# pangenome/allwave

Measured on AMD Instinct MI355X. Metric: aligned base-pairs/sec (whole node) + PAF lines/sec, all-pairs 10 kbp, higher is better.
Workload: dtype int16

## Files before the change

### allwave_amd/build.py

```python
import hashlib
import json
import os
import shutil
import subprocess
import tempfile
import time

ROOT = os.path.dirname(os.path.dirname(os.path.abspath(__file__)))
PKG = os.path.join(ROOT, "allwave_amd")
CSRC = os.path.join(PKG, "csrc")
HOST_DIR = os.path.join(CSRC, "host")
HIP_LIB = os.path.join(PKG, "liballwave_hip.so")
HOST_LIB = os.path.join(PKG, "liballwave_host.so")
CLI_BIN = os.path.join(PKG, "allwave_hip")
INFO = os.path.join(PKG, "BUILD_INFO.json")
ABI_HEADER = os.path.join(ROOT, "include", "allwave_hip.h")


def hipcc():
    for c in (os.environ.get("HIPCC"), shutil.which("hipcc"), "/opt/rocm/bin/hipcc"):
        if c and os.path.exists(c):
            return c
    raise RuntimeError("hipcc not found")


HIP_FLAGS = ["-O3", "-std=c++17", "--offload-arch=gfx950"]
HIP_FLAGS_AWV = HIP_FLAGS + ["-mllvm", "-amdgpu-sched-strategy=max-ilp"]
HIP_UNITS = (("engine.hip", HIP_FLAGS), ("kernels_awv.hip", HIP_FLAGS_AWV), ("planner.hip", HIP_FLAGS), ("orient.hip", HIP_FLAGS),
             ("verify.hip", HIP_FLAGS), ("clip.hip", HIP_FLAGS), ("split.hip", HIP_FLAGS), ("normalize.hip", HIP_FLAGS))
HIP_SOURCES = [os.path.join(CSRC, f) for f in ("engine.hip", "kernels_awv.hip", "kernels_awv.hpp", "biwfa_device.hpp", "range_span.hpp", "batch_plan.hpp", "twin_plan.hpp", "twin_base.hpp", "planner.hip",
                                               "planner_device.hpp", "orient.hip", "orient_device.hpp", "verify.hip", "verify_device.hpp", "clip.hip", "clip_device.hpp", "clip_scan.hpp", "split.hip", "split_device.hpp", "normalize.hip", "normalize_device.hpp", "wave_ops.hpp",
                                               "host_errors.hpp", "record_pass.hpp", "record_pieces.hpp")] + [ABI_HEADER]


def _host_sources():
    return [os.path.join(HOST_DIR, f) for f in sorted(os.listdir(HOST_DIR)) if f.endswith((".cpp", ".hpp", ".h"))]


_VERSIONS = {}


def _tool_version(tool):
    if tool not in _VERSIONS:
        try:
            _VERSIONS[tool] = subprocess.run([tool, "--version"], stdout=subprocess.PIPE, stderr=subprocess.STDOUT).stdout.decode(errors="replace")
        except OSError:
            _VERSIONS[tool] = "?"
    return _VERSIONS[tool]


def content_hash(sources, commands, tool):
    h = hashlib.sha256()
    for s in sorted(sources):
        h.update(os.path.relpath(s, ROOT).encode() + b"\0")
        with open(s, "rb") as f:
            h.update(f.read())
        h.update(b"\0")
    for c in commands:
        h.update(" ".join(c).encode() + b"\n")
    h.update(_tool_version(tool).encode())
    return h.hexdigest()


def _load_info():
    try:
        with open(INFO) as f:
            d = json.load(f)
        return d if isinstance(d.get("targets"), dict) else {"targets": {}}
    except (OSError, ValueError):
        return {"targets": {}}


def _record(target, digest, action):
    info = _load_info()
    info["targets"][os.path.basename(target)] = {"sha256": digest, "action": action, "when": time.strftime("%Y-%m-%dT%H:%M:%S")}
    tmp = INFO + ".%d.tmp" % os.getpid()
    with open(tmp, "w") as f:
        json.dump(info, f, indent=1)
    os.replace(tmp, INFO)


def _up_to_date(target, digest):
    return os.path.exists(target) and _load_info()["targets"].get(os.path.basename(target), {}).get("sha256") == digest


def _rel(cmd):
    return [a.replace(ROOT + os.sep, "") for a in cmd]


def build_hip(force=False, verbose=False):
    inc = ["-I" + os.path.join(ROOT, "include"), "-I" + CSRC]
    compile_cmds = [[hipcc()] + flags + ["-fPIC", "-c"] + inc + [os.path.join(CSRC, unit)] for unit, flags in HIP_UNITS]
    link_cmd = [hipcc(), "--offload-arch=gfx950", "-fPIC", "-shared"]
    digest = content_hash(HIP_SOURCES, [_rel(c) for c in compile_cmds] + [_rel(link_cmd)], hipcc())
    if not force and _up_to_date(HIP_LIB, digest):
        _record(HIP_LIB, digest, "reused (content hash of sources + flags + compiler matches)")
        return HIP_LIB
    tmp = tempfile.mkdtemp(prefix="awv_build_%d_" % os.getpid())
    try:
        objs, procs = [], []
        for (unit, _), cmd in zip(HIP_UNITS, compile_cmds):
            obj = os.path.join(tmp, unit.replace(".hip", ".o"))
            full = cmd + ["-o", obj]
            if verbose:
                print(" ".join(full))
            procs.append((full, subprocess.Popen(full)))
            objs.append(obj)
        failed = None
        for full, p in procs:
            if p.wait() != 0 and failed is None:
                failed = (p.returncode, full)
        if failed:
            raise subprocess.CalledProcessError(failed[0], failed[1])
        out = os.path.join(tmp, "liballwave_hip.so")
        full = link_cmd + ["-o", out] + objs
        if verbose:
            print(" ".join(full))
        subprocess.check_call(full)
        staged = HIP_LIB + ".%d.tmp" % os.getpid()
        shutil.copy2(out, staged)
        os.replace(staged, HIP_LIB)
    finally:
        shutil.rmtree(tmp, ignore_errors=True)
    _record(HIP_LIB, digest, "compiled")
    return HIP_LIB


def _build_one(target, sources, cmd, force, verbose, tool="g++"):
    digest = content_hash(sources, [_rel(cmd)], tool)
    if not force and _up_to_date(target, digest):
        _record(target, digest, "reused (content hash of sources + flags + compiler matches)")
        return
    tmp = target + ".%d.tmp" % os.getpid()
    full = cmd[:cmd.index("-o") + 1] + [tmp] + cmd[cmd.index("-o") + 2:]
    if verbose:
        print(" ".join(full))
    try:
        subprocess.check_call(full)
        os.replace(tmp, target)
    finally:
        if os.path.exists(tmp):
            os.remove(tmp)
    _record(target, digest, "compiled")


def build_host(force=False, verbose=False):
    if not os.path.isdir(HOST_DIR):
        return None
    srcs = _host_sources()
    cpps = [s for s in srcs if s.endswith(".cpp") and not s.endswith("main.cpp")]
    if not cpps:
        return None
    cmd = ["g++", "-O2", "-std=c++17", "-fPIC", "-shared", "-pthread", "-I" + os.path.join(ROOT, "include"), "-I" + HOST_DIR,
           "-o", HOST_LIB] + cpps + ["-L" + PKG, "-lallwave_hip", "-ldl", "-Wl,-rpath,$ORIGIN", "-Wl,-rpath-link,/opt/rocm/lib"]
    _build_one(HOST_LIB, srcs + [ABI_HEADER], cmd, force, verbose)
    cli_src = os.path.join(HOST_DIR, "main.cpp")
    if os.path.exists(cli_src):
        cmd = ["g++", "-O2", "-std=c++17", "-pthread", "-I" + os.path.join(ROOT, "include"), "-I" + HOST_DIR, "-o", CLI_BIN, cli_src,
               "-L" + PKG, "-lallwave_host", "-lallwave_hip", "-lz", "-Wl,-rpath,$ORIGIN", "-Wl,-rpath-link,/opt/rocm/lib"]
        _build_one(CLI_BIN, srcs + [ABI_HEADER], cmd, force, verbose)
    return HOST_LIB


def build_all(force=False, verbose=False):
    return build_hip(force, verbose), build_host(force, verbose)


def build_report():
    t = _load_info()["targets"]
    return {k: "%s [sha256 %s]" % (v.get("action", "?"), v.get("sha256", "")[:12]) for k, v in sorted(t.items())}


if __name__ == "__main__":
    print(build_all(force=True, verbose=True))
    print(json.dumps(build_report(), indent=1))
```

### allwave_amd/csrc/biwfa_device.hpp

```cpp


#include <hip/hip_runtime.h>
#include <stdint.h>
#include <limits.h>

#include "range_span.hpp"
#include "twin_base.hpp"

#ifndef AWV_NS
#define AWV_NS awv
#endif
#ifndef AWV_WG
#define AWV_WG 64
#endif
namespace AWV_NS {

constexpr int WG = AWV_WG;
constexpr int MAX_SCOPE = 126;
constexpr int MAX_RING = 256;
constexpr int NCOMP = 5;
constexpr int32_t OFF_NULL = INT32_MIN / 2;
constexpr int32_t NULLISH = INT32_MIN / 4;
constexpr int32_t NULL16 = -16384;
#ifdef AWV_WIDE16
constexpr bool WENC = true;
#else
constexpr bool WENC = false;
#endif
enum { C_M = 0, C_I1 = 1, C_I2 = 2, C_D1 = 3, C_D2 = 4 };
constexpr int FALLBACK_MIN_SCORE = 250;
constexpr int FALLBACK_MIN_LENGTH = 100;
constexpr int STACK_CAP = 48;
constexpr int EV_STACK_WORDS = (STACK_CAP * 32 + 3) / 4 + 16;
constexpr int EV_TWIN_WORDS = MAX_SCOPE * NCOMP;
constexpr int SUB16_MAX_LEN = 32760;
#ifndef AWV_WAVES_PER_SIMD
#define AWV_WAVES_PER_SIMD 4
#endif
constexpr int WAVES_PER_SIMD = AWV_WAVES_PER_SIMD;
constexpr int STATIC_LDS_RESERVE = 1024;
constexpr int COL_PAD = 576;

constexpr int ST_OK = 0, ST_CAPACITY = 1, ST_INTERNAL = 2, ST_MAX_STEPS = 3, ST_ABOVE_BOUND = 4;
constexpr int ST_TWIN_REDO = 64;

struct DevPenalties {
  int x, o1, e1, o2, e2, two_piece, scope;
};

struct DevResult {
  int32_t status, penalty, score;
  uint32_t cigar_len;
  uint64_t cigar_off;
  int32_t num_matches, num_mismatches, num_ins, num_del, q_end, t_end;
};

enum { STAT_CELLS = 0, STAT_EXTEND, STAT_BREAKPOINTS, STAT_BASE, STAT_OVERLAP, STAT_ALIGNED_BP, STAT_PAIRS,
       STAT_T_TOTAL, STAT_T_BI_COMPUTE, STAT_T_BI_BARRIER, STAT_T_BI_FINALIZE, STAT_T_OVERLAP, STAT_T_BASE_STEPS,
       STAT_T_BACKTRACE, STAT_T_EMIT, STAT_N_PASSES,
       STAT_T_CR_LOAD, STAT_T_CR_ALU, STAT_T_CR_EXTEND, STAT_T_CR_STORE, STAT_T_CR_REDUCE, STAT_RESTARTS, STAT_MULTI_CELLS, STAT_WIN_SINGLE, STAT_WIN_MULTI, STAT_WIN_BASE, STAT_WIN_BASE_MULTI,
       STAT_CLK_CYCLES, STAT_CLK_TICKS,
       STAT_DEEP_CELLS,
       STAT_N,
       STAT_TWIN_UNITS = STAT_N, STAT_TWIN_SHARED, STAT_TWIN_SOLO, STAT_TWIN_NONMIRROR,
       STAT_N_DEV };

#ifdef AWV_PROF
#define PROF_DRAIN() __builtin_amdgcn_s_waitcnt(0)
#define PROF_NOW() __builtin_readcyclecounter()
#define PROF_ADD(slot, t0) do { if (threadIdx.x == 0) lstats[slot] += __builtin_readcyclecounter() - (t0); } while (0)
#define PROF_INC(slot) do { if (threadIdx.x == 0) lstats[slot] += 1; } while (0)
#define PROF_ADD_L(slot, t0) do { if (threadIdx.x == 0) sh.prof[(slot) - STAT_T_CR_LOAD] += __builtin_readcyclecounter() - (t0); } while (0)
#else
#define PROF_ADD_L(slot, t0) do { (void)(t0); } while (0)
#define PROF_DRAIN() do { } while (0)
#define PROF_NOW() 0ULL
#define PROF_ADD(slot, t0) do { (void)(t0); } while (0)
#define PROF_INC(slot) do { } while (0)
#endif

struct KParams {
  const uint8_t* seq[4];
  const uint64_t* seq_off;
  const int32_t* seq_len;
  const uint32_t* seq2[2];
  const uint64_t* seq2_off;
  const uint8_t* seq2_ok;
  const int32_t* pair_q;
  const int32_t* pair_t;
  const int32_t* pair_rc;
  long long npairs;
  DevPenalties pen;
  int ring;
  int chain_max;
  int multi_T;
  int deep_passes;
  int sub16;
  int wcap;
  void* ring_mem;
  size_t ring_slot_stride;
  int lds_meta_bytes;
  int lds_seq_bytes;
  int sb_cap;
  int wb_cap;
  void* hist_mem;
  size_t hist_slot_stride;
  size_t hist_meta_offset;
  uint32_t* ev_mem;
  size_t ev_slot_stride;
  uint8_t* cigar;
  const uint64_t* cigar_off;
  DevResult* results;
  unsigned long long* work_counter;
  unsigned long long* stats;
  int score_only;
  int max_penalty;
  const int32_t* pair_max_penalty;
  const int32_t* unit_first;
  const int32_t* unit_twin;
  int twin_levels;
  int twin_base;
};

struct RowMeta { int lo, hi; };
constexpr int K_BIG = 1 << 28;
#define ROW_EMPTY RowMeta{K_BIG, -K_BIG}
struct Acc { int hull_lo[NCOMP]; int hull_hi[NCOMP]; int maxak; int oob; int reach; };
struct Task { int pb, pe, tb, te, cb, ce, score_remaining, known; };
constexpr int TM_A = 0, TM_B = 1, TM_SHARED = 2;
constexpr bool TWIN_BUILD = WG == 64 && !WENC;
constexpr int TWIN_MAGIC = 0x7477696e;
__device__ __forceinline__ int twin_comp(int c) { return c == 0 ? 0 : (c <= 2 ? c + 2 : c - 2); }
struct Breakpoint { int score, sf, sr, kf, kr, off_f, off_r, comp; };
static_assert(sizeof(Task) == 32 && sizeof(Breakpoint) == 32, "stack entry / twin record size");

__device__ __forceinline__ int s_min(int a, int b) { int r; asm("s_min_i32 %0, %1, %2" : "=s"(r) : "s"(a), "s"(b) : "scc"); return r; }
__device__ __forceinline__ int s_max(int a, int b) { int r; asm("s_max_i32 %0, %1, %2" : "=s"(r) : "s"(a), "s"(b) : "scc"); return r; }
__device__ __forceinline__ int s_add(int a, int b) { int r; asm("s_add_i32 %0, %1, %2" : "=s"(r) : "s"(a), "s"(b) : "scc"); return r; }

struct alignas(4) RowMeta16 { int16_t lo, hi; };
template <typename OffT> struct MetaTraits;
#ifdef AWV_WIDE16
template <> struct MetaTraits<int16_t> { typedef RowMeta Stored; };
#else
template <> struct MetaTraits<int16_t> { typedef RowMeta16 Stored; };
#endif
template <> struct MetaTraits<int32_t> { typedef RowMeta Stored; };
__device__ __forceinline__ RowMeta meta_load(const RowMeta16* p) {
  const RowMeta16 m = *p;
  return m.lo > m.hi ? ROW_EMPTY : RowMeta{m.lo, m.hi};
}
__device__ __forceinline__ RowMeta meta_load(const RowMeta* p) { return *p; }
__device__ __forceinline__ void meta_store(RowMeta16* p, const RowMeta& m) {
  *p = m.lo > m.hi ? RowMeta16{1, 0} : RowMeta16{(int16_t)m.lo, (int16_t)m.hi};
}
__device__ __forceinline__ void meta_store_scalar(RowMeta16* p, int lo, int hi) {
  int w;
  asm("s_pack_ll_b32_b16 %0, %1, %2\n\ts_cmp_gt_i32 %1, %2\n\ts_cselect_b32 %0, 1, %0" : "=&s"(w) : "s"(lo), "s"(hi) : "scc");
  *reinterpret_cast<int*>(p) = w;
}
__device__ __forceinline__ void meta_store_scalar(RowMeta* p, int lo, int hi) {
  int l, h;
  asm("s_cmp_gt_i32 %2, %3\n\ts_cselect_b32 %0, %4, %2\n\ts_cselect_b32 %1, %5, %3" : "=&s"(l), "=&s"(h) : "s"(lo), "s"(hi), "s"(K_BIG), "s"(-K_BIG) : "scc");
  *p = RowMeta{l, h};
}
__device__ __forceinline__ void meta_store(RowMeta* p, const RowMeta& m) { *p = m; }

template <typename OffT>
struct Lds {
  typename MetaTraits<OffT>::Stored* ring_meta;
  int* bi_A;
  int* bi_oob;
  int* firstk;
  uint32_t* seq;
  RowMeta* meta_log;
};
struct PassCtx {
  unsigned long long ring_mem;
  unsigned long long ring_bytes;
  unsigned long long P[2], T[2];
  int ring, wcap;
  int x, o1, e1, o2, e2;
  int lds_meta_bytes;
  int chain_max;
  int plen, tlen, kmin[2], wcols;
  int seq_mode, p_w0, t_w0, p_bit, t_bit;
  unsigned long long meta_log;
  int wb_cap, sb_cap, end_comp;
  unsigned long long Pw, Tw;
  int multi_T, lds_seq_bytes, pb_abs, tb_abs;
  int deep_passes;
  int max_penalty, score_cap;
};
struct PhaseResult {
  int why, sc, fmax, rmax, npass;
  int sf, sr, last_fwd;
  int deep_from;
  unsigned long long cells, deep_cells;
};
struct Shared {
  Acc acc[3][2];
  int chain_maxak[2][8];
  PassCtx pctx;
  PhaseResult pres;
  Breakpoint bp_out;
  unsigned long long ext_multi;
  unsigned int win_single, win_multi, win_base, win_base_multi;
  int ext0[2];
#ifdef AWV_PROF
  unsigned long long prof[5];
#endif
  long long cur_pair;
  int error;
  int nev;
  int bt_total;
};

typedef const __attribute__((address_space(1))) uint8_t* gseq_t;
typedef uint64_t u64_unaligned __attribute__((aligned(1)));
typedef const __attribute__((address_space(1))) uint32_t* gwords_t;
__device__ __forceinline__ gseq_t to_global(const uint8_t* p) { return (gseq_t)(uintptr_t)p; }

struct SubCtx {
  int plen, tlen;
  gseq_t P[2];
  gseq_t T[2];
  int kmin[2];
  int wcols;
  int seq_mode;
  int p_w0, t_w0;
  int p_bit, t_bit;
  gwords_t Pw, Tw;
  int pb_abs, tb_abs;
};

__device__ __forceinline__ bool row_empty(const RowMeta& m) { return m.lo > m.hi; }

__device__ __forceinline__ int uni(int x) { return __builtin_amdgcn_readfirstlane(x); }
__device__ __forceinline__ int clamp_from_m1(int x, int hi) {
  int r;
  asm("v_med3_i32 %0, %1, -1, %2" : "=v"(r) : "v"(x), "s"(hi));
  return r;
}
__device__ __forceinline__ int cold_tid() {
  int t = threadIdx.x;
  asm volatile("" : "+v"(t));
  return t;
}
__device__ __forceinline__ RowMeta uni(const RowMeta& m) { return RowMeta{uni(m.lo), uni(m.hi)}; }

__device__ __forceinline__ uint64_t ld64u(gseq_t p) {
  return *(const __attribute__((address_space(1))) u64_unaligned*)p;
}

__device__ __forceinline__ int wave_max_i32(int v) {
  v = max(v, __builtin_amdgcn_update_dpp(INT_MIN, v, 0x111, 0xf, 0xf, false));
  v = max(v, __builtin_amdgcn_update_dpp(INT_MIN, v, 0x112, 0xf, 0xf, false));
  v = max(v, __builtin_amdgcn_update_dpp(INT_MIN, v, 0x114, 0xf, 0xf, false));
  v = max(v, __builtin_amdgcn_update_dpp(INT_MIN, v, 0x118, 0xf, 0xf, false));
  v = max(v, __builtin_amdgcn_update_dpp(INT_MIN, v, 0x142, 0xa, 0xf, false));
  v = max(v, __builtin_amdgcn_update_dpp(INT_MIN, v, 0x143, 0xc, 0xf, false));
  return __builtin_amdgcn_readlane(v, 63);
}

template <typename OffT> struct OffTraits;
template <> struct OffTraits<int32_t> { static constexpr int VEC = 4; };
template <> struct OffTraits<int16_t> { static constexpr int VEC = 4; };

template <typename OffT> constexpr bool wenc_of() { return WENC && sizeof(OffT) == 2; }
template <typename OffT>
__device__ __forceinline__ int32_t off_load1(const OffT* p, int k) {
  const int32_t v = (int32_t)*p;
  if (sizeof(OffT) == 2) return v < 0 ? OFF_NULL : (wenc_of<OffT>() ? v + max(k, 0) : v);
  return v;
}
// ... 1430 lines not shown
        if (lane == 0 && t < Tn) atomicMax(&maxak_out[t], wmax);
      }
    } else {
      const int wmax = wave_max_i32(productive ? lane_maxak : 0);
      if (lane == 0) atomicMax(&maxak_out[0], wmax);
    }
  }
  if (BASE && lane == 0 && reach_mask) atomicOr(&acc.reach, (int)reach_mask);
  return cells;
}

typedef __attribute__((address_space(3))) Shared* lds_shared_ptr;
typedef __attribute__((address_space(3))) unsigned char* lds_bytes_ptr;
constexpr int MP_MARGIN = 0, MP_DISCARD = 1, MP_MET = 2, MP_ERROR = 3, MP_DEEP_MET = 4, MP_BOUND = 5;
template <bool P2, typename OffT, int E1, int E2>
__device__ __attribute__((noinline)) void deep_phase(unsigned sh_addr, unsigned dyn_addr, int s0_v, int fmax_v, int rmax_v, int Tn_v, int pass_v,
                                                     int far_npass_v, unsigned far_cells_lo, unsigned far_cells_hi);
#ifndef AWV_RESTART_ATTEMPTS
#define AWV_RESTART_ATTEMPTS 3
#endif
#ifndef AWV_MARGIN_BASE
#define AWV_MARGIN_BASE 256
#endif
#ifndef AWV_MARGIN_MUL4
#define AWV_MARGIN_MUL4 6
#endif
constexpr int MARGIN_BASE = AWV_MARGIN_BASE, MARGIN_MUL4 = AWV_MARGIN_MUL4;
template <bool P2, typename OffT, int E1, int E2, bool CHAIN>
__device__ __attribute__((noinline)) void multi_phase(unsigned sh_addr, unsigned dyn_addr, int s0_v, int fmax_v, int rmax_v, int Tn_v, int pass_v, int deep_v) {
  Shared& sh = *(Shared*)__builtin_assume_aligned((Shared*)(lds_shared_ptr)(uintptr_t)uni((int)sh_addr), 8);
  unsigned char* dyn_smem = (unsigned char*)__builtin_assume_aligned((unsigned char*)(lds_bytes_ptr)(uintptr_t)uni((int)dyn_addr), 16);
  const int Tn = uni(Tn_v);
  int sc = uni(s0_v);
  int fmax = uni(fmax_v), rmax = uni(rmax_v), pass = uni(pass_v);
  const PassCtx& pc = sh.pctx;
  KParams kp{};
  kp.ring = uni(pc.ring);
  kp.wcap = uni(pc.wcap);
  kp.pen.x = uni(pc.x);
  kp.pen.o1 = uni(pc.o1);
  kp.pen.e1 = uni(pc.e1);
  kp.pen.o2 = uni(pc.o2);
  kp.pen.e2 = uni(pc.e2);
  kp.pen.two_piece = P2 ? 1 : 0;
  kp.pen.scope = max(kp.pen.x, max(kp.pen.o1 + kp.pen.e1, P2 ? kp.pen.o2 + kp.pen.e2 : 0)) + 1;
  kp.lds_meta_bytes = uni(pc.lds_meta_bytes);
  auto uni64 = [](unsigned long long v) { return ((unsigned long long)(unsigned)uni((int)(v >> 32)) << 32) | (unsigned)uni((int)v); };
  SubCtx cx;
  cx.plen = uni(pc.plen);
  cx.tlen = uni(pc.tlen);
  cx.kmin[0] = uni(pc.kmin[0]);
  cx.kmin[1] = uni(pc.kmin[1]);
  cx.wcols = uni(pc.wcols);
  cx.seq_mode = uni(pc.seq_mode);
  cx.p_w0 = uni(pc.p_w0);
  cx.t_w0 = uni(pc.t_w0);
  cx.p_bit = uni(pc.p_bit);
  cx.t_bit = uni(pc.t_bit);
  cx.P[0] = (gseq_t)(uintptr_t)uni64(pc.P[0]);
  cx.P[1] = (gseq_t)(uintptr_t)uni64(pc.P[1]);
  cx.T[0] = (gseq_t)(uintptr_t)uni64(pc.T[0]);
  cx.T[1] = (gseq_t)(uintptr_t)uni64(pc.T[1]);
  cx.Pw = nullptr;
  cx.Tw = nullptr;
  cx.pb_abs = cx.tb_abs = 0;
  Lds<OffT> lds;
  typedef typename MetaTraits<OffT>::Stored MetaStored;
  lds.ring_meta = reinterpret_cast<MetaStored*>(dyn_smem);
  lds.bi_A = reinterpret_cast<int*>(lds.ring_meta + 2 * NCOMP * kp.ring);
  lds.bi_oob = lds.bi_A + 2 * kp.ring;
  lds.firstk = lds.bi_oob + 2 * kp.ring;
  lds.seq = reinterpret_cast<uint32_t*>(dyn_smem + kp.lds_meta_bytes);
  lds.meta_log = nullptr;
  const rsrc_t rs = make_rsrc((void*)(uintptr_t)uni64(pc.ring_mem), (size_t)uni64(pc.ring_bytes));
  const int rmask = kp.ring - 1;
  const int max_antidiagonal = cx.plen + cx.tlen - 1;
  const int arun_start = fmax + rmax;
  int arun0 = fmax, arun1 = rmax;
  int nsteps = 0, npass = 0, why = MP_MARGIN;
  unsigned long long cells = 0;
  unsigned ext_iters = 0;
  const bool lds_chain = CHAIN && sizeof(OffT) == 4 && cx.seq_mode != 1 &&
                         uni(pc.lds_seq_bytes) >= (WG / 64) * TMAX32 * 64 * 16;
  const int margin_shift = (uni(deep_v) >> 8) & 3;
  const bool long_reads = (uni(deep_v) & 0x400) != 0;
  const int chain_cap = CHAIN ? min(max(uni(pc.chain_max), 1), sizeof(OffT) == 2 ? CHAIN_MAX : (lds_chain ? 3 : CHAIN_MAX32)) : 1;
  for (;;) {
    if (sc >= uni(pc.score_cap)) { why = MP_BOUND; break; }
    const int grow = nsteps > 0 ? (arun0 + arun1 - arun_start) / nsteps : 0;
    int nh = 0;
    for (int c = chain_cap; c >= 1; --c) {
      const int T = c > 1 ? TMAX * c : Tn;
      const int mul4 = (sizeof(OffT) == 2 && !long_reads) ? MARGIN_MUL4 : MARGIN_MUL4 + 2;
      if (arun0 + arun1 < max_antidiagonal - ((MARGIN_BASE + mul4 * (kp.pen.scope + T) * max(grow, 8) / 4) << margin_shift)) { nh = c; break; }
    }
    if (nh == 0) { why = MP_MARGIN; break; }
    const int T = nh > 1 ? TMAX * nh : Tn;
    const int aslot = pass % 3;
    int nc0 = 0, nc1 = 0;
#pragma nounroll
    for (int dir = 0; dir < 2; ++dir) {
      MultiPlan mp;
      const unsigned long long tpl = PROF_NOW();
      plan_multi<P2, OffT, E1, E2, false>(kp, lds, cx, dir, sc, T, nh, mp);
      mp.lds_chain = lds_chain ? 1 : 0;
      PROF_ADD_L(STAT_T_CR_REDUCE, tpl);
      Acc& acc = dir ? sh.acc[aslot][1] : sh.acc[aslot][0];
      const int nc = compute_rows_multi<P2, OffT, E1, E2, false, CHAIN>(kp, sh, lds, cx, rs, dir, sc, mp, acc, dir ? sh.chain_maxak[1] : sh.chain_maxak[0], ext_iters);
      if (dir) nc1 = nc; else nc0 = nc;
    }
    __syncthreads();
    if (uni(sh.error)) { why = MP_ERROR; break; }
    if (uni(sh.acc[aslot][0].oob) != 0 || uni(sh.acc[aslot][1].oob) != 0) { why = MP_DISCARD; break; }
    cells += (unsigned long long)(nc0 + nc1);
    const int P0 = uni(sh.chain_maxak[0][0]), P1 = uni(sh.chain_maxak[1][0]);
    arun0 = max(arun0, P0);
    arun1 = max(arun1, P1);
    fmax = max(fmax, P0);
    rmax = max(rmax, P1);
    const bool met = fmax + rmax >= max_antidiagonal;
    __syncthreads();
    if (threadIdx.x < 16) sh.chain_maxak[threadIdx.x >> 3][threadIdx.x & 7] = 0;
    if (threadIdx.x == 0) { acc_reset(sh.acc[(pass + 2) % 3][0]); acc_reset(sh.acc[(pass + 2) % 3][1]); }
    __syncthreads();
    ++pass;
    ++npass;
    nsteps += T;
    sc += T;
    if (met) { why = MP_MET; break; }
  }
  __syncthreads();
  if (threadIdx.x == 0) {
    PhaseResult& pr = sh.pres;
    pr.why = why;
    pr.sc = sc;
    pr.sf = pr.sr = sc;
    pr.last_fwd = 0;
    pr.deep_from = sc;
    pr.fmax = fmax;
    pr.rmax = rmax;
    pr.npass = npass;
    pr.cells = cells;
    pr.deep_cells = 0;
#pragma unroll
    for (int i = 0; i < 3; ++i) { acc_reset(sh.acc[i][0]); acc_reset(sh.acc[i][1]); }
  }
  if (threadIdx.x < 16) sh.chain_maxak[threadIdx.x >> 3][threadIdx.x & 7] = 0;
  atomicAdd(&sh.ext_multi, (unsigned long long)ext_iters);
  __syncthreads();
  if ((uni(deep_v) & 1) != 0 && why == MP_MARGIN)
    deep_phase<P2, OffT, E1, E2>(sh_addr, dyn_addr, sc, fmax, rmax, Tn, pass, npass, (unsigned)cells, (unsigned)(cells >> 32));
}

template <bool P2, typename OffT, int E1, int E2>
__device__ __attribute__((noinline)) void deep_phase(unsigned sh_addr, unsigned dyn_addr, int s0_v, int fmax_v, int rmax_v, int Tn_v, int pass_v,
                                                     int far_npass_v, unsigned far_cells_lo, unsigned far_cells_hi) {
  Shared& sh = *(Shared*)__builtin_assume_aligned((Shared*)(lds_shared_ptr)(uintptr_t)uni((int)sh_addr), 8);
  unsigned char* dyn_smem = (unsigned char*)__builtin_assume_aligned((unsigned char*)(lds_bytes_ptr)(uintptr_t)uni((int)dyn_addr), 16);
  const int Tn = uni(Tn_v);
  int sc = uni(s0_v);
  int fmax = uni(fmax_v), rmax = uni(rmax_v), pass = uni(pass_v);
  const PassCtx& pc = sh.pctx;
  KParams kp{};
  kp.ring = uni(pc.ring);
  kp.wcap = uni(pc.wcap);
  kp.pen.x = uni(pc.x);
  kp.pen.o1 = uni(pc.o1);
  kp.pen.e1 = uni(pc.e1);
  kp.pen.o2 = uni(pc.o2);
  kp.pen.e2 = uni(pc.e2);
  kp.pen.two_piece = P2 ? 1 : 0;
  kp.pen.scope = max(kp.pen.x, max(kp.pen.o1 + kp.pen.e1, P2 ? kp.pen.o2 + kp.pen.e2 : 0)) + 1;
  kp.lds_meta_bytes = uni(pc.lds_meta_bytes);
  auto uni64 = [](unsigned long long v) { return ((unsigned long long)(unsigned)uni((int)(v >> 32)) << 32) | (unsigned)uni((int)v); };
  SubCtx cx;
  cx.plen = uni(pc.plen);
  cx.tlen = uni(pc.tlen);
  cx.kmin[0] = uni(pc.kmin[0]);
  cx.kmin[1] = uni(pc.kmin[1]);
  cx.wcols = uni(pc.wcols);
  cx.seq_mode = uni(pc.seq_mode);
  cx.p_w0 = uni(pc.p_w0);
  cx.t_w0 = uni(pc.t_w0);
  cx.p_bit = uni(pc.p_bit);
  cx.t_bit = uni(pc.t_bit);
  cx.P[0] = (gseq_t)(uintptr_t)uni64(pc.P[0]);
  cx.P[1] = (gseq_t)(uintptr_t)uni64(pc.P[1]);
  cx.T[0] = (gseq_t)(uintptr_t)uni64(pc.T[0]);
  cx.T[1] = (gseq_t)(uintptr_t)uni64(pc.T[1]);
  cx.Pw = nullptr;
  cx.Tw = nullptr;
  cx.pb_abs = cx.tb_abs = 0;
  Lds<OffT> lds;
  typedef typename MetaTraits<OffT>::Stored MetaStored;
  lds.ring_meta = reinterpret_cast<MetaStored*>(dyn_smem);
  lds.bi_A = reinterpret_cast<int*>(lds.ring_meta + 2 * NCOMP * kp.ring);
  lds.bi_oob = lds.bi_A + 2 * kp.ring;
  lds.firstk = lds.bi_oob + 2 * kp.ring;
  lds.seq = reinterpret_cast<uint32_t*>(dyn_smem + kp.lds_meta_bytes);
  lds.meta_log = nullptr;
  const rsrc_t rs = make_rsrc((void*)(uintptr_t)uni64(pc.ring_mem), (size_t)uni64(pc.ring_bytes));
  const int rmask = kp.ring - 1;
  const int max_antidiagonal = cx.plen + cx.tlen - 1;
  int sf = sc, sr = sc, last_fwd = 0;
  const int deep_from = sc, far_npass = uni(far_npass_v);
  const unsigned long long far_cells = ((unsigned long long)(unsigned)uni((int)far_cells_hi) << 32) | (unsigned)uni((int)far_cells_lo);
  int npass = 0, why = MP_DISCARD;
  unsigned long long cells = 0;
  unsigned ext_iters = 0;
  for (;;) {
    if (sc >= uni(pc.score_cap)) { why = MP_BOUND; break; }
    const int aslot = pass % 3;
    int nc0 = 0, nc1 = 0;
#pragma nounroll
    for (int dir = 0; dir < 2; ++dir) {
      MultiPlan mp;
      const unsigned long long tpl = PROF_NOW();
      plan_multi<P2, OffT, E1, E2, false>(kp, lds, cx, dir, sc, Tn, 1, mp);
      PROF_ADD_L(STAT_T_CR_REDUCE, tpl);
      Acc& acc = dir ? sh.acc[aslot][1] : sh.acc[aslot][0];
      const int nc = compute_rows_multi<P2, OffT, E1, E2, false, false, true>(kp, sh, lds, cx, rs, dir, sc, mp, acc, dir ? sh.chain_maxak[1] : sh.chain_maxak[0], ext_iters);
      if (dir) nc1 = nc; else nc0 = nc;
    }
    __syncthreads();
    if (uni(sh.error)) { why = MP_ERROR; break; }
    if (uni(sh.acc[aslot][0].oob) != 0 || uni(sh.acc[aslot][1].oob) != 0) { why = MP_DISCARD; break; }
    cells += (unsigned long long)(nc0 + nc1);
    bool met = false;
    for (int t = 0; t < Tn; ++t) {
      const int slot = (sc + 1 + t) & rmask;
      const int A0 = uni(sh.chain_maxak[0][t]), A1 = uni(sh.chain_maxak[1][t]);
      lds.bi_A[slot] = A0;
      lds.bi_A[kp.ring + slot] = A1;
      lds.bi_oob[slot] = 0;
      lds.bi_oob[kp.ring + slot] = 0;
      if (!met) {
        ++sf;
        fmax = max(fmax, A0);
        last_fwd = 1;
        if (fmax + rmax >= max_antidiagonal) met = true;
        else {
          ++sr;
          rmax = max(rmax, A1);
          last_fwd = 0;
          if (fmax + rmax >= max_antidiagonal) met = true;
        }
      }
    }
    __syncthreads();
    if (threadIdx.x < 16) sh.chain_maxak[threadIdx.x >> 3][threadIdx.x & 7] = 0;
    if (threadIdx.x == 0) { acc_reset(sh.acc[(pass + 2) % 3][0]); acc_reset(sh.acc[(pass + 2) % 3][1]); }
    __syncthreads();
    ++pass;
    ++npass;
    sc += Tn;
    if (met) { why = MP_DEEP_MET; break; }
  }
  __syncthreads();
  if (threadIdx.x == 0) {
    PhaseResult& pr = sh.pres;
    pr.why = why;
    pr.sc = sc;
    pr.sf = sf;
    pr.sr = sr;
    pr.last_fwd = last_fwd;
    pr.deep_from = deep_from;
    pr.fmax = fmax;
    pr.rmax = rmax;
    pr.npass = far_npass + npass;
    pr.cells = far_cells + cells;
    pr.deep_cells = cells;
#pragma unroll
    for (int i = 0; i < 3; ++i) { acc_reset(sh.acc[i][0]); acc_reset(sh.acc[i][1]); }
  }
  if (threadIdx.x < 16) sh.chain_maxak[threadIdx.x >> 3][threadIdx.x & 7] = 0;
  atomicAdd(&sh.ext_multi, (unsigned long long)ext_iters);
  __syncthreads();
}

template <bool P2, typename OffT, int E1, int E2>
__device__ __attribute__((noinline)) void base_phase(unsigned sh_addr, unsigned dyn_addr, int s0_v, int Tn_v, int pass_v) {
  Shared& sh = *(Shared*)__builtin_assume_aligned((Shared*)(lds_shared_ptr)(uintptr_t)uni((int)sh_addr), 8);
  unsigned char* dyn_smem = (unsigned char*)__builtin_assume_aligned((unsigned char*)(lds_bytes_ptr)(uintptr_t)uni((int)dyn_addr), 16);
  const int Tn = uni(Tn_v);
  int sc = uni(s0_v), pass = uni(pass_v);
  const PassCtx& pc = sh.pctx;
  KParams kp{};
  kp.ring = uni(pc.ring);
  kp.wb_cap = uni(pc.wb_cap);
  kp.sb_cap = uni(pc.sb_cap);
  kp.pen.x = uni(pc.x);
  kp.pen.o1 = uni(pc.o1);
  kp.pen.e1 = uni(pc.e1);
  kp.pen.o2 = uni(pc.o2);
  kp.pen.e2 = uni(pc.e2);
  kp.pen.two_piece = P2 ? 1 : 0;
  kp.pen.scope = max(kp.pen.x, max(kp.pen.o1 + kp.pen.e1, P2 ? kp.pen.o2 + kp.pen.e2 : 0)) + 1;
  kp.lds_meta_bytes = uni(pc.lds_meta_bytes);
  auto uni64 = [](unsigned long long v) { return ((unsigned long long)(unsigned)uni((int)(v >> 32)) << 32) | (unsigned)uni((int)v); };
  SubCtx cx;
  cx.plen = uni(pc.plen);
  cx.tlen = uni(pc.tlen);
  cx.kmin[0] = uni(pc.kmin[0]);
  cx.kmin[1] = cx.kmin[0];
  cx.wcols = uni(pc.wcols);
  cx.seq_mode = uni(pc.seq_mode);
// ... 1008 lines not shown
  bp.score = INT_MAX;
  unsigned ext_iters = 0;
  unsigned long long cells = 0, multi_cells = 0, deep_cells = 0;
  int pass = 0;
  const long long max_steps = ((long long)pn.o1 + pn.o2 + 2LL * (pn.e1 + pn.e2) + pn.x) * ((long long)plen + tlen + 4) + 1024;
  long long steps = 0;
  int rc = BP_OK;
  if (kp.max_penalty != INT_MAX) bp.score = kp.max_penalty + 1;
  const int gap_opening = P2 ? max(pn.o1, pn.o2) : pn.o1;
  bool last_fwd = false;
  const bool known_optimum = known_score != INT_MAX;
  bool dirty[2] = {false, false};
  const bool force_single = (attempt & 0xff) >= AWV_RESTART_ATTEMPTS - 1;
  const int deep_arg = kp.deep_passes | ((attempt & 0xff) == 1 && !force_single ? 0x200 : 0) | ((attempt & 0x100) ? 0x400 : 0);
  const int multi_T = (!force_single && plen + tlen > AWV_MIN_PASS_LEN) ? kp.multi_T : 0;
  bool deep_on = multi_T == 0;
  int deep_since[2] = {deep_on ? 0 : INT_MAX, deep_on ? 0 : INT_MAX};
  auto deep_ok = [&](int d0, int s0, int d1, int s1) {
    const int lo_need = max(s1 - (pn.scope - 1), 1);
    return (s0 == 0 || deep_since[d0] <= s0) && (s1 == 0 || deep_since[d1] <= lo_need);
  };
  int phase = 1;
  for (;;) {
    if (phase == 1 && fmax + rmax >= max_antidiagonal) phase = 2;
    {
      Acc* a = sh.acc[pass % 3];
      int plo[2] = {1, 1}, phi[2] = {0, 0};
      bool need[2];
      const unsigned long long tp0 = PROF_NOW();
      if (!deep_on && (dirty[0] || dirty[1])) {
        deep_on = true;
        deep_since[0] = comp[0] + 1;
        deep_since[1] = comp[1] + 1;
      }
      if (!deep_on && phase == 1 && comp[0] == sc[0] && comp[1] == sc[1] && sc[0] == sc[1]) {
        if (P2) multi_phase<P2, OffT, 2, 1, P2>(sh_addr, dyn_addr, sc[0], fmax, rmax, multi_T, pass, deep_arg);
        else if (pn.e1 == 1) multi_phase<P2, OffT, 1, 1, false>(sh_addr, dyn_addr, sc[0], fmax, rmax, multi_T, pass, deep_arg);
        else multi_phase<P2, OffT, 2, 1, false>(sh_addr, dyn_addr, sc[0], fmax, rmax, multi_T, pass, deep_arg);
        PROF_ADD(STAT_T_BI_COMPUTE, tp0);
        const int why = uni(sh.pres.why);
        if (why == MP_ERROR) { rc = uni(sh.error); break; }
        if (why == MP_MET) { rc = BP_RESTART; break; }
        steps += (long long)(uni(sh.pres.sc) - sc[0]);
        comp[0] = comp[1] = uni(sh.pres.sc);
        sc[0] = uni(sh.pres.sf);
        sc[1] = uni(sh.pres.sr);
        last_fwd = uni(sh.pres.last_fwd) != 0;
        fmax = uni(sh.pres.fmax);
        rmax = uni(sh.pres.rmax);
        pass += uni(sh.pres.npass);
        {
          const unsigned long long c = ((unsigned long long)(unsigned)uni((int)(sh.pres.cells >> 32)) << 32) | (unsigned)uni((int)sh.pres.cells);
          const unsigned long long dc = ((unsigned long long)(unsigned)uni((int)(sh.pres.deep_cells >> 32)) << 32) | (unsigned)uni((int)sh.pres.deep_cells);
          cells += c;
          multi_cells += c;
          deep_cells += dc;
        }
        deep_on = true;
        deep_since[0] = deep_since[1] = uni(sh.pres.deep_from) + 1;
        __syncthreads();
        continue;
      } else {
#pragma unroll
      for (int dir = 0; dir < 2; ++dir) {
        need[dir] = comp[dir] == sc[dir];
        if (need[dir]) {
          StepPlan pl;
          plan_step<P2, false, OffT>(kp, lds, dir, sc[dir] + 1, pl);
          cells += compute_row<P2, false, OffT>(kp, sh, lds, cx, ring_rs, dir, sc[dir] + 1, pl, dirty[dir], a[dir], ext_iters);
          plo[dir] = pl.lo;
          phi[dir] = pl.hi;
        }
      }
#ifdef AWV_DIAG
      if (tid == 0) {
        const int zone = (dirty[0] || dirty[1]) ? 4 : multi_T == 0 ? 0 : phase == 2 ? 3 : (sc[0] + 1 - (pn.scope - 1) >= 1) ? 2 : 1;
        unsigned nw = 0;
        if (need[0] && plo[0] <= phi[0]) nw += (unsigned)((phi[0] - plo[0] + 4) / 248 + 1);
        if (need[1] && plo[1] <= phi[1]) nw += (unsigned)((phi[1] - plo[1] + 4) / 248 + 1);
        lstats[STAT_T_CR_LOAD + zone] += nw;
      }
#endif
      if (need[0] || need[1]) {
        PROF_ADD(STAT_T_BI_COMPUTE, tp0);
        PROF_INC(STAT_N_PASSES);
        const unsigned long long tp1 = PROF_NOW();
        __syncthreads();
        PROF_ADD(STAT_T_BI_BARRIER, tp1);
        const unsigned long long tp2 = PROF_NOW();
        if (uni(sh.error)) { rc = uni(sh.error); break; }
        const bool trim0 = need[0] && uni(a[0].oob) != 0, trim1 = need[1] && uni(a[1].oob) != 0;
        dirty[0] = dirty[0] || trim0;
        dirty[1] = dirty[1] || trim1;
        if (trim0 || trim1) {
          if (trim0) trim_pass_fn<P2, false, OffT>(sh_addr, 0, sc[0] + 1, plo[0], phi[0], pass % 3);
          if (trim1) trim_pass_fn<P2, false, OffT>(sh_addr, 1, sc[1] + 1, plo[1], phi[1], pass % 3);
          __syncthreads();
        }
        if (need[0]) { finalize_row<false, OffT>(kp, lds, cx, 0, sc[0] + 1, a[0], trim0); comp[0] = sc[0] + 1; }
        if (need[1]) { finalize_row<false, OffT>(kp, lds, cx, 1, sc[1] + 1, a[1], trim1); comp[1] = sc[1] + 1; }
        if (tid == 0) { acc_reset(sh.acc[(pass + 2) % 3][0]); acc_reset(sh.acc[(pass + 2) % 3][1]); }
        ++pass;
        PROF_ADD(STAT_T_BI_FINALIZE, tp2);
      }
      }
    }
    if (phase == 1) {
      ++sc[0];
      fmax = max(fmax, uni(lds.bi_A[0 * kp.ring + (sc[0] & rmask)]));
      last_fwd = true;
      if (fmax + rmax >= max_antidiagonal) { phase = 2; continue; }
      ++sc[1];
      rmax = max(rmax, uni(lds.bi_A[1 * kp.ring + (sc[1] & rmask)]));
      last_fwd = false;
      if (sc[1] >= uni(sh.pctx.score_cap)) { rc = BP_ABOVE_BOUND; break; }
    } else {
      if (last_fwd) {
        const int min_sr = (sc[1] > pn.scope - 1) ? sc[1] - (pn.scope - 1) : 0;
        if (sc[0] + min_sr - gap_opening >= bp.score) break;
        if (!deep_ok(0, sc[0], 1, sc[1])) { rc = BP_RESTART; break; }
        const unsigned long long to0 = PROF_NOW();
        bialign_overlap<P2, OffT>(kp, sh, lds, cx, ring_mem, ring_rs, 0, sc[0], sc[1], true, bp, lstats);
        PROF_ADD(STAT_T_OVERLAP, to0);
        if (known_optimum && bp.score == known_score) break;
        ++sc[1];
      }
      const int min_sf = (sc[0] > pn.scope - 1) ? sc[0] - (pn.scope - 1) : 0;
      if (min_sf + sc[1] - gap_opening >= bp.score) break;
      if (!deep_ok(1, sc[1], 0, sc[0])) { rc = BP_RESTART; break; }
      const unsigned long long to1 = PROF_NOW();
      bialign_overlap<P2, OffT>(kp, sh, lds, cx, ring_mem, ring_rs, 1, sc[1], sc[0], false, bp, lstats);
      PROF_ADD(STAT_T_OVERLAP, to1);
      if (known_optimum && bp.score == known_score) break;
      ++sc[0];
      last_fwd = true;
    }
    if (++steps > max_steps) { rc = ST_MAX_STEPS; break; }
  }
  if (tid == 0) {
    lstats[STAT_CELLS] += cells;
    lstats[STAT_MULTI_CELLS] += multi_cells;
    lstats[STAT_DEEP_CELLS] += deep_cells;
    lstats[STAT_BREAKPOINTS] += 1;
  }
  atomicAdd(&lstats[STAT_EXTEND], (unsigned long long)ext_iters);
  if (tid == 0) lstats[STAT_EXTEND] += sh.ext_multi;
  if (rc == BP_OK && bp.score > uni(sh.pctx.max_penalty)) rc = BP_ABOVE_BOUND;
  __syncthreads();
  if (rc == BP_OK && bp.score == INT_MAX) rc = ST_INTERNAL;
  return rc;
}

template <bool P2, typename OffT>
__device__ __attribute__((noinline)) int find_breakpoint_fn(unsigned sh_addr, unsigned dyn_addr, unsigned lstats_addr, int cb_v, int ce_v,
                                                            int score_remaining_v, int known_v, int attempt_v) {
  Shared& sh = *(Shared*)__builtin_assume_aligned((Shared*)(__attribute__((address_space(3))) Shared*)(uintptr_t)uni((int)sh_addr), 8);
  unsigned char* dyn_smem = (unsigned char*)__builtin_assume_aligned((unsigned char*)(__attribute__((address_space(3))) unsigned char*)(uintptr_t)uni((int)dyn_addr), 16);
  unsigned long long* lstats = (unsigned long long*)__builtin_assume_aligned((unsigned long long*)(__attribute__((address_space(3))) unsigned long long*)(uintptr_t)uni((int)lstats_addr), 8);
  const int cb = uni(cb_v), ce = uni(ce_v), score_remaining = uni(score_remaining_v), known = uni(known_v);
  const int attempt = uni(attempt_v);
  const PassCtx& pc = sh.pctx;
  auto uni64 = [](unsigned long long v) { return ((unsigned long long)(unsigned)uni((int)(v >> 32)) << 32) | (unsigned)uni((int)v); };
  KParams kp{};
  kp.ring = uni(pc.ring);
  kp.wcap = uni(pc.wcap);
  kp.pen.x = uni(pc.x);
  kp.pen.o1 = uni(pc.o1);
  kp.pen.e1 = uni(pc.e1);
  kp.pen.o2 = uni(pc.o2);
  kp.pen.e2 = uni(pc.e2);
  kp.pen.two_piece = P2 ? 1 : 0;
  kp.pen.scope = max(kp.pen.x, max(kp.pen.o1 + kp.pen.e1, P2 ? kp.pen.o2 + kp.pen.e2 : 0)) + 1;
  kp.lds_meta_bytes = uni(pc.lds_meta_bytes);
  kp.lds_seq_bytes = uni(pc.lds_seq_bytes);
  kp.chain_max = uni(pc.chain_max);
  kp.multi_T = uni(pc.multi_T);
  kp.deep_passes = uni(pc.deep_passes);
  kp.max_penalty = score_remaining == INT_MAX ? uni(pc.max_penalty) : INT_MAX;
  kp.ring_slot_stride = (size_t)uni64(pc.ring_bytes);
  SubCtx cx;
  cx.plen = uni(pc.plen);
  cx.tlen = uni(pc.tlen);
  cx.kmin[0] = cx.kmin[1] = 0;
  cx.wcols = 0;
  cx.seq_mode = uni(pc.seq_mode);
  cx.p_w0 = uni(pc.p_w0);
  cx.t_w0 = uni(pc.t_w0);
  cx.p_bit = uni(pc.p_bit);
  cx.t_bit = uni(pc.t_bit);
  cx.P[0] = (gseq_t)(uintptr_t)uni64(pc.P[0]);
  cx.P[1] = (gseq_t)(uintptr_t)uni64(pc.P[1]);
  cx.T[0] = (gseq_t)(uintptr_t)uni64(pc.T[0]);
  cx.T[1] = (gseq_t)(uintptr_t)uni64(pc.T[1]);
  cx.Pw = (gwords_t)(uintptr_t)uni64(pc.Pw);
  cx.Tw = (gwords_t)(uintptr_t)uni64(pc.Tw);
  cx.pb_abs = uni(pc.pb_abs);
  cx.tb_abs = uni(pc.tb_abs);
  Lds<OffT> lds;
  typedef typename MetaTraits<OffT>::Stored MetaStored;
  lds.ring_meta = reinterpret_cast<MetaStored*>(dyn_smem);
  lds.bi_A = reinterpret_cast<int*>(lds.ring_meta + 2 * NCOMP * kp.ring);
  lds.bi_oob = lds.bi_A + 2 * kp.ring;
  lds.firstk = lds.bi_oob + 2 * kp.ring;
  lds.seq = reinterpret_cast<uint32_t*>(dyn_smem + kp.lds_meta_bytes);
  lds.meta_log = nullptr;
  void* ring_mem = (void*)(__attribute__((address_space(1))) char*)(uintptr_t)uni64(pc.ring_mem);
  const rsrc_t ring_rs = make_rsrc(ring_mem, kp.ring_slot_stride);
  __syncthreads();
  Breakpoint bp;
  const int rc = find_breakpoint<P2, OffT>(kp, sh, lds, cx, ring_mem, ring_rs, cb, ce, score_remaining, known, attempt, bp, lstats);
  if (threadIdx.x == 0) sh.bp_out = bp;
  __syncthreads();
  return rc;
}

template <bool P2, typename OffT, typename... PairSpan>
__global__ __launch_bounds__(WG, WAVES_PER_SIMD) void biwfa_align_kernel(KParams kp, PairSpan... pair_span_arg) {
  constexpr bool RANGES = sizeof...(PairSpan) > 0;
  static_assert(sizeof...(PairSpan) <= 1, "one optional argument: const awvr::Span*");
  __shared__ Shared sh;
  __shared__ unsigned long long lstats[STAT_N];
  static_assert(sizeof(Shared) + sizeof(unsigned long long) * STAT_N <= STATIC_LDS_RESERVE, "static LDS reserve");
  extern __shared__ __attribute__((aligned(16))) unsigned char dyn_smem[];
  Lds<OffT> lds;
  typedef typename MetaTraits<OffT>::Stored MetaStored;
  lds.ring_meta = reinterpret_cast<MetaStored*>(dyn_smem);
  lds.bi_A = reinterpret_cast<int*>(lds.ring_meta + 2 * NCOMP * kp.ring);
  lds.bi_oob = lds.bi_A + 2 * kp.ring;
  lds.firstk = lds.bi_oob + 2 * kp.ring;
  lds.seq = reinterpret_cast<uint32_t*>(dyn_smem + kp.lds_meta_bytes);
  const int tid = cold_tid();
  const DevPenalties& pn = kp.pen;
  void* ring_mem = (char*)kp.ring_mem + (size_t)blockIdx.x * kp.ring_slot_stride;
  void* hist = (char*)kp.hist_mem + (size_t)blockIdx.x * kp.hist_slot_stride;
  uint32_t* events = kp.ev_mem + (size_t)blockIdx.x * kp.ev_slot_stride;
  Task* const stack = reinterpret_cast<Task*>(events + kp.wcap);
  const rsrc_t hist_rs = make_rsrc(hist, kp.hist_slot_stride);
  lds.meta_log = reinterpret_cast<RowMeta*>((char*)hist + kp.hist_meta_offset);
  if (tid < STAT_N) lstats[tid] = 0;
#ifdef AWV_PROF
  if (tid < 5) sh.prof[tid] = 0;
#endif
  const unsigned long long clk_c0 = __builtin_amdgcn_s_memtime(), clk_r0 = __builtin_amdgcn_s_memrealtime();
  if (tid < 16) sh.chain_maxak[tid >> 3][tid & 7] = 0;
  __syncthreads();
  constexpr bool TWINS = TWIN_BUILD && !RANGES && sizeof(OffT) == 2;
  if constexpr (TWINS) {
  for (;;) {
    if (tid == 0) {
      sh.cur_pair = (long long)atomicAdd(kp.work_counter, 1ULL);
      sh.win_single = sh.win_multi = sh.win_base = sh.win_base_multi = 0;
    }
    __syncthreads();
    const long long unit = ((long long)uni((int)(sh.cur_pair >> 32)) << 32) | (unsigned)uni((int)sh.cur_pair);
    if (unit >= kp.npairs) break;
    long long pair = unit, pair_b = -1;
    if constexpr (TWINS) {
      if (kp.unit_first) {
        pair = uni(kp.unit_first[unit]);
        pair_b = uni(kp.unit_twin[unit]);
      }
    }
    const int qi = kp.pair_q[pair], ti = kp.pair_t[pair];
    const int qv = kp.pair_rc[pair] ? 2 : 0;
    const uint64_t qoff = kp.seq_off[qi], toff = kp.seq_off[ti];
    int plenT = kp.seq_len[qi], tlenT = kp.seq_len[ti];
    const uint8_t* Pf = kp.seq[qv] + qoff;
    const uint8_t* Pr = kp.seq[qv + 1] + qoff;
    const uint8_t* Tf = kp.seq[0] + toff;
    const uint8_t* Tr = kp.seq[1] + toff;
    const int qok = (kp.seq2_ok[qi] >> (qv ? 1 : 0)) & 1, tok = kp.seq2_ok[ti] & 1;
    gwords_t Pw = nullptr, Tw = nullptr;
    if (qok && tok && kp.lds_seq_bytes > 0) {
      Pw = (gwords_t)(uintptr_t)(kp.seq2[qv ? 1 : 0] + kp.seq2_off[qi]);
      Tw = (gwords_t)(uintptr_t)(kp.seq2[0] + kp.seq2_off[ti]);
    }
    int tw_shared = 0, tw_solo = 0, tw_nonmirror = 0;
    int run_mode = TWINS && pair_b >= 0 ? TM_SHARED : TM_A;
    int todo = 0;
    for (;;) {
    const unsigned long long tt0 = PROF_NOW();
    int cur = TM_A;
    Emit em, em_o;
    em.cig = kp.score_only ? nullptr : kp.cigar + kp.cigar_off[pair];
    em.n = 0;
    em.cnt[0] = em.cnt[1] = em.cnt[2] = em.cnt[3] = 0;
    em_o = em;
    if (pair_b >= 0 && !kp.score_only) em_o.cig = kp.cigar + kp.cigar_off[pair_b];
    int status = ST_OK;
    int penalty = -1, penalty_o = -1;
    bool top = true, top_o = true;
    auto face = [&](int o) {
      if (cur == o) return;
      cur = o;
      { const uint8_t* x = Pf; Pf = Tf; Tf = x; }
      { const uint8_t* x = Pr; Pr = Tr; Tr = x; }
      { const gwords_t x = Pw; Pw = Tw; Tw = x; }
      { const int x = plenT; plenT = tlenT; tlenT = x; }
      { const Emit x = em; em = em_o; em_o = x; }
      { const int x = penalty; penalty = penalty_o; penalty_o = x; }
      { const bool x = top; top = top_o; top_o = x; }
    };
    if (TWINS && run_mode == TM_B) face(TM_B);
    int sp = 0;
    if constexpr (RANGES) {
      if (tid == 0) {
        const awvr::Span top = (pair_span_arg, ...)[pair];
        const bool min_length = max(top.pe - top.pb, top.te - top.tb) <= FALLBACK_MIN_LENGTH;
        stack[0] = Task{top.pb, top.pe, top.tb, top.te, C_M, C_M, min_length ? 0 : INT_MAX, INT_MAX};
        sh.error = 0;
      }
    } else if (tid == 0) {
      const bool min_length = max(plenT, tlenT) <= FALLBACK_MIN_LENGTH;
      stack[0] = Task{0, plenT, 0, tlenT, C_M | (run_mode << 8), C_M, min_length ? 0 : INT_MAX, INT_MAX};
      sh.error = 0;
    }
    sp = 1;
    __syncthreads();
    while (sp > 0 && status == ST_OK) {
      Task t = stack[sp - 1];
      t.pb = uni(t.pb); t.pe = uni(t.pe); t.tb = uni(t.tb); t.te = uni(t.te);
      t.cb = uni(t.cb); t.ce = uni(t.ce); t.score_remaining = uni(t.score_remaining); t.known = uni(t.known);
      --sp;
      __syncthreads();
      const int mode = TWINS ? (t.cb >> 8) & 3 : TM_A, depth = TWINS ? t.cb >> 16 : 0;
      if (TWINS) {
        t.cb &= 0xff;
        face(mode == TM_B ? TM_B : TM_A);
      }
      const int plen = t.pe - t.pb, tlen = t.te - t.tb;
      bool split = mode == TM_SHARED && (tlen == 0 || plen == 0 || t.score_remaining <= FALLBACK_MIN_SCORE);
      Breakpoint bp, bq;
      bool do_base = false;
      SubCtx cx;
      if (!split) {
      if (tlen == 0) {
        emit_run(em, 'D', plen);
        if (top) penalty = plen > 0 ? min(pn.o1 + plen * pn.e1, P2 ? pn.o2 + plen * pn.e2 : INT_MAX) : 0;
        top = false;
        continue;
      } else if (plen == 0) {
        emit_run(em, 'I', tlen);
        if (top) penalty = min(pn.o1 + tlen * pn.e1, P2 ? pn.o2 + tlen * pn.e2 : INT_MAX);
        top = false;
        continue;
      }
      cx.plen = plen;
      cx.tlen = tlen;
      cx.P[0] = to_global(Pf + t.pb);
      cx.T[0] = to_global(Tf + t.tb);
      cx.P[1] = to_global(Pr + (plenT - t.pe));
      cx.T[1] = to_global(Tr + (tlenT - t.te));
      cx.kmin[0] = cx.kmin[1] = 0;
      cx.wcols = 0;
      cx.Pw = Pw;
      cx.Tw = Tw;
      cx.pb_abs = t.pb;
      cx.tb_abs = t.tb;
      stage_sequences<OffT>(kp, lds, cx);
      do_base = t.score_remaining <= FALLBACK_MIN_SCORE;
      if (!do_base) {
        int rc = BP_OK;
        for (int attempt = 0; attempt < AWV_RESTART_ATTEMPTS; ++attempt) {
          if (tid == 0) {
            PassCtx& pc = sh.pctx;
            pc.ring_mem = (unsigned long long)(uintptr_t)ring_mem;
            pc.ring_bytes = (unsigned long long)kp.ring_slot_stride;
            pc.P[0] = (unsigned long long)(uintptr_t)cx.P[0];
            pc.P[1] = (unsigned long long)(uintptr_t)cx.P[1];
            pc.T[0] = (unsigned long long)(uintptr_t)cx.T[0];
            pc.T[1] = (unsigned long long)(uintptr_t)cx.T[1];
            pc.Pw = (unsigned long long)(uintptr_t)cx.Pw;
            pc.Tw = (unsigned long long)(uintptr_t)cx.Tw;
            pc.ring = kp.ring;
            pc.wcap = kp.wcap;
            pc.x = pn.x; pc.o1 = pn.o1; pc.e1 = pn.e1; pc.o2 = pn.o2; pc.e2 = pn.e2;
            pc.lds_meta_bytes = kp.lds_meta_bytes;
            pc.lds_seq_bytes = kp.lds_seq_bytes;
            pc.chain_max = kp.chain_max;
            pc.multi_T = kp.multi_T;
            pc.deep_passes = kp.deep_passes;
            pc.max_penalty = kp.pair_max_penalty ? kp.pair_max_penalty[pair] : kp.max_penalty;
            pc.plen = plen; pc.tlen = tlen;
            pc.seq_mode = cx.seq_mode; pc.p_w0 = cx.p_w0; pc.t_w0 = cx.t_w0; pc.p_bit = cx.p_bit; pc.t_bit = cx.t_bit;
            pc.pb_abs = cx.pb_abs; pc.tb_abs = cx.tb_abs;
            const unsigned long long tab = (unsigned long long)(uintptr_t)(events + kp.wcap + EV_STACK_WORDS);
            sh.bp_out.comp = mode == TM_SHARED && !kp.score_only ? TWIN_MAGIC : 0;
            sh.bp_out.off_f = (int)(unsigned)tab;
            sh.bp_out.off_r = (int)(unsigned)(tab >> 32);
            if (mode == TM_SHARED)
              reinterpret_cast<Breakpoint*>(dyn_smem + kp.lds_meta_bytes - sizeof(Breakpoint))->score = INT_MAX;
          }
          __syncthreads();
          if constexpr (sizeof(OffT) == 4 && !WENC) {
            if (kp.sub16 != 0 && max(plen, tlen) < SUB16_MAX_LEN)
              rc = uni(find_breakpoint_fn<P2, int16_t>((unsigned)(uintptr_t)&sh, (unsigned)(uintptr_t)lds.ring_meta, (unsigned)(uintptr_t)lstats,
                                                       t.cb, t.ce, t.score_remaining, t.known, attempt | 0x100));
            else
              rc = uni(find_breakpoint_fn<P2, OffT>((unsigned)(uintptr_t)&sh, (unsigned)(uintptr_t)lds.ring_meta, (unsigned)(uintptr_t)lstats,
                                                    t.cb, t.ce, t.score_remaining, t.known, attempt));
          } else {
            rc = uni(find_breakpoint_fn<P2, OffT>((unsigned)(uintptr_t)&sh, (unsigned)(uintptr_t)lds.ring_meta, (unsigned)(uintptr_t)lstats,
                                                  t.cb, t.ce, t.score_remaining, t.known, attempt));
          }
          if (rc == BP_OK) {
            bp.score = uni(sh.bp_out.score); bp.sf = uni(sh.bp_out.sf); bp.sr = uni(sh.bp_out.sr); bp.kf = uni(sh.bp_out.kf);
            bp.kr = uni(sh.bp_out.kr); bp.off_f = uni(sh.bp_out.off_f); bp.off_r = uni(sh.bp_out.off_r); bp.comp = uni(sh.bp_out.comp);
            if (mode == TM_SHARED && !kp.score_only) {
              const Breakpoint* rec = reinterpret_cast<const Breakpoint*>(dyn_smem + kp.lds_meta_bytes - sizeof(Breakpoint));
              bq.score = uni(rec->score); bq.sf = uni(rec->sf); bq.sr = uni(rec->sr); bq.kf = uni(rec->kf);
              bq.off_f = uni(rec->off_f); bq.comp = uni(rec->comp);
            }
          }
          if (rc != BP_RESTART) break;
          if (tid == 0) lstats[STAT_RESTARTS] += 1;
        }
        if (TWINS && pair_b >= 0 && run_mode == TM_SHARED) {
          if (mode == TM_SHARED) ++tw_shared;
          else ++tw_solo;
        }
        if (rc == BP_END_REACHED) {
          if (mode == TM_SHARED) split = true;
          else do_base = true;
        }
        else if (rc == BP_ABOVE_BOUND) { status = ST_ABOVE_BOUND; break; }
        else if (rc != BP_OK) { status = rc; break; }
      }
      }
      bool shared_base = false;
      if (split && kp.twin_base != 0) {
        if (tlen == 0 || plen == 0) {
          const int n = max(plen, tlen);
          const int pen_gap = n > 0 ? min(pn.o1 + n * pn.e1, P2 ? pn.o2 + n * pn.e2 : INT_MAX) : 0;
          emit_run(em, tlen == 0 ? 'D' : 'I', n);
          emit_run(em_o, plen == 0 ? 'D' : 'I', n);
          if (top) penalty = pen_gap;
          if (top_o) penalty_o = pen_gap;
          top = top_o = false;
          continue;
        }
        if (t.score_remaining <= FALLBACK_MIN_SCORE) {
          cx.plen = plen;
          cx.tlen = tlen;
          cx.P[0] = to_global(Pf + t.pb);
          cx.T[0] = to_global(Tf + t.tb);
          cx.P[1] = to_global(Pr + (plenT - t.pe));
          cx.T[1] = to_global(Tr + (tlenT - t.te));
          cx.kmin[0] = cx.kmin[1] = 0;
          cx.wcols = 0;
          cx.Pw = Pw;
          cx.Tw = Tw;
          cx.pb_abs = t.pb;
          cx.tb_abs = t.tb;
          stage_sequences<OffT>(kp, lds, cx);
        }
        split = false;
        do_base = shared_base = true;
      }
      if (split) {
        if (sp + 2 > STACK_CAP) { status = ST_TWIN_REDO; break; }
        if (tid == 0) {
          stack[sp] = Task{t.tb, t.te, t.pb, t.pe, twin_comp(t.cb) | (TM_B << 8), twin_comp(t.ce), t.score_remaining, t.known};
          stack[sp + 1] = Task{t.pb, t.pe, t.tb, t.te, t.cb | (TM_A << 8), t.ce, t.score_remaining, t.known};
        }
        sp += 2;
        __syncthreads();
        continue;
      }
      if (do_base) {
        int pen_b = 0;
        const int rc = base_align_twin<P2, OffT>(kp, sh, lds, cx, hist, hist_rs, events, t.cb, t.ce, em, pen_b, lstats, em_o, shared_base && !kp.score_only);
        if (rc != ST_OK) { status = shared_base ? ST_TWIN_REDO : rc; break; }
        if (top) penalty = pen_b;
        top = false;
        if (shared_base) {
          if (top_o) penalty_o = pen_b;
          top_o = false;
        }
        continue;
      }
      if (kp.score_only) {
        penalty = bp.score;
        if (mode == TM_SHARED) penalty_o = bp.score;
        break;
      }
      const int bh = bp.off_f, bv = bp.off_f - bp.kf;
      if (mode != TM_SHARED) {
        if (bh < 0 || bh > tlen || bv < 0 || bv > plen || sp + 2 > STACK_CAP) { status = ST_INTERNAL; break; }
        if (tid == 0) {
          const int open_c = bp.comp == C_M ? 0 : ((bp.comp == C_I1 || bp.comp == C_D1) ? kp.pen.o1 : kp.pen.o2);
          stack[sp] = Task{t.pb + bv, t.pe, t.tb + bh, t.te, bp.comp | (mode << 8), t.ce, bp.sr, bp.sr - open_c};
          stack[sp + 1] = Task{t.pb, t.pb + bv, t.tb, t.tb + bh, t.cb | (mode << 8), bp.comp, bp.sf, bp.sf - open_c};
        }
        sp += 2;
      } else {
        const int qh = bq.off_f, qv2 = bq.off_f - bq.kf;
        if (bq.score != bp.score || bq.comp < 0 || bq.comp >= NCOMP || (!P2 && (bq.comp == C_I2 || bq.comp == C_D2)) || bh < 0 || bh > tlen || bv < 0 || bv > plen || qh < 0 || qh > plen || qv2 < 0 || qv2 > tlen ||
            sp + 4 > STACK_CAP) { status = ST_TWIN_REDO; break; }
        const bool mirror = bq.kf == -bp.kf && qh == bv && bq.comp == twin_comp(bp.comp) && bq.sf == bp.sf && bq.sr == bp.sr;
        if (!mirror) ++tw_nonmirror;
        const int open_c = bp.comp == C_M ? 0 : ((bp.comp == C_I1 || bp.comp == C_D1) ? kp.pen.o1 : kp.pen.o2);
        if (mirror && depth + 1 < kp.twin_levels) {
          if (tid == 0) {
            const int tag = (TM_SHARED << 8) | ((depth + 1) << 16);
            stack[sp] = Task{t.pb + bv, t.pe, t.tb + bh, t.te, bp.comp | tag, t.ce, bp.sr, bp.sr - open_c};
            stack[sp + 1] = Task{t.pb, t.pb + bv, t.tb, t.tb + bh, t.cb | tag, bp.comp, bp.sf, bp.sf - open_c};
          }
          sp += 2;
        } else {
          if (tid == 0) {
            const int open_q = bq.comp == C_M ? 0 : ((bq.comp == C_I1 || bq.comp == C_D1) ? kp.pen.o1 : kp.pen.o2);
            const int cbq = twin_comp(t.cb), ceq = twin_comp(t.ce);
            stack[sp] = Task{t.pb + bv, t.pe, t.tb + bh, t.te, bp.comp | (TM_A << 8), t.ce, bp.sr, bp.sr - open_c};
            stack[sp + 1] = Task{t.tb + qv2, t.te, t.pb + qh, t.pe, bq.comp | (TM_B << 8), ceq, bq.sr, bq.sr - open_q};
            stack[sp + 2] = Task{t.pb, t.pb + bv, t.tb, t.tb + bh, t.cb | (TM_A << 8), bp.comp, bp.sf, bp.sf - open_c};
            stack[sp + 3] = Task{t.tb, t.tb + qv2, t.pb, t.pb + qh, cbq | (TM_B << 8), bq.comp, bq.sf, bq.sf - open_q};
          }
          sp += 4;
        }
        if (top_o) penalty_o = bp.score;
        top_o = false;
      }
      if (top) penalty = bp.score;
      top = false;
      __syncthreads();
    }
    const int failed_in = cur;
    if (TWINS) face(TM_A);
    bool write_a = run_mode == TM_A, write_b = run_mode == TM_B;
    if (TWINS && run_mode == TM_SHARED) {
      if (status == ST_OK) write_a = write_b = true;
      else if (status == ST_TWIN_REDO) todo = 3;
      else if (failed_in == TM_B) { write_b = true; todo = 1; }
      else { write_a = true; todo = 2; }
    }
    const int pair_bound = kp.pair_max_penalty ? kp.pair_max_penalty[pair] : kp.max_penalty;
    if (status == ST_OK && penalty > pair_bound) {
      status = ST_ABOVE_BOUND;
      em.cnt[0] = em.cnt[1] = em.cnt[2] = em.cnt[3] = 0;
    }
    if (tid == 0) {
      auto record = [&](long long pi, const Emit& e, int pen, int qlen) {
        DevResult r;
        r.status = status;
        r.penalty = status == ST_OK ? pen : status == ST_ABOVE_BOUND ? pair_bound + 1 : 0;
        r.score = -r.penalty;
        r.cigar_len = status == ST_OK && !kp.score_only ? (uint32_t)e.n : 0u;
        r.cigar_off = kp.score_only ? 0 : kp.cigar_off[pi];
        r.num_matches = e.cnt[0];
        r.num_mismatches = e.cnt[1];
        r.num_ins = e.cnt[2];
        r.num_del = e.cnt[3];
        r.q_end = e.cnt[0] + e.cnt[1] + e.cnt[3];
        r.t_end = e.cnt[0] + e.cnt[1] + e.cnt[2];
        kp.results[pi] = r;
        if (status == ST_OK) {
          lstats[STAT_ALIGNED_BP] += (unsigned long long)qlen;
          lstats[STAT_PAIRS] += 1;
        }
      };
      if constexpr (RANGES) {
        record(pair, em, penalty, (pair_span_arg, ...)[pair].pe - (pair_span_arg, ...)[pair].pb);
      } else {
        if (write_a) record(pair, em, penalty, plenT);
        if (TWINS && write_b) record(pair_b, em_o, penalty_o, tlenT);
      }
      PROF_ADD(STAT_T_TOTAL, tt0);
      lstats[STAT_WIN_SINGLE] += sh.win_single; lstats[STAT_WIN_MULTI] += sh.win_multi; lstats[STAT_WIN_BASE] += sh.win_base; lstats[STAT_WIN_BASE_MULTI] += sh.win_base_multi;
      sh.win_single = sh.win_multi = sh.win_base = sh.win_base_multi = 0;
    }
    __syncthreads();
    if (!TWINS || !todo) break;
    run_mode = (todo & 1) ? TM_A : TM_B;
    todo &= ~(1 << run_mode);
    }
    if (TWINS && pair_b >= 0 && tid == 0) {
      atomicAdd(&kp.stats[STAT_TWIN_UNITS], 1ULL);
      atomicAdd(&kp.stats[STAT_TWIN_SHARED], (unsigned long long)tw_shared);
      atomicAdd(&kp.stats[STAT_TWIN_SOLO], (unsigned long long)tw_solo);
      atomicAdd(&kp.stats[STAT_TWIN_NONMIRROR], (unsigned long long)tw_nonmirror);
    }
  }
  } else {
  for (;;) {
    if (tid == 0) {
      sh.cur_pair = (long long)atomicAdd(kp.work_counter, 1ULL);
      sh.error = 0;
      sh.win_single = sh.win_multi = sh.win_base = sh.win_base_multi = 0;
    }
    __syncthreads();
    const long long pair = ((long long)uni((int)(sh.cur_pair >> 32)) << 32) | (unsigned)uni((int)sh.cur_pair);
    if (pair >= kp.npairs) break;
    const int qi = kp.pair_q[pair], ti = kp.pair_t[pair];
    const int qv = kp.pair_rc[pair] ? 2 : 0;
    const uint64_t qoff = kp.seq_off[qi], toff = kp.seq_off[ti];
    const int plenT = kp.seq_len[qi], tlenT = kp.seq_len[ti];
    const uint8_t* Pf = kp.seq[qv] + qoff;
    const uint8_t* Pr = kp.seq[qv + 1] + qoff;
    const uint8_t* Tf = kp.seq[0] + toff;
    const uint8_t* Tr = kp.seq[1] + toff;
    const int qok = (kp.seq2_ok[qi] >> (qv ? 1 : 0)) & 1, tok = kp.seq2_ok[ti] & 1;
    gwords_t Pw = nullptr, Tw = nullptr;
    if (qok && tok && kp.lds_seq_bytes > 0) {
      Pw = (gwords_t)(uintptr_t)(kp.seq2[qv ? 1 : 0] + kp.seq2_off[qi]);
      Tw = (gwords_t)(uintptr_t)(kp.seq2[0] + kp.seq2_off[ti]);
    }
    const unsigned long long tt0 = PROF_NOW();
    Emit em;
    em.cig = kp.score_only ? nullptr : kp.cigar + kp.cigar_off[pair];
    em.n = 0;
    em.cnt[0] = em.cnt[1] = em.cnt[2] = em.cnt[3] = 0;
    int status = ST_OK;
    int penalty = -1;
    int sp = 0;
    if constexpr (RANGES) {
      if (tid == 0) {
        const awvr::Span top = (pair_span_arg, ...)[pair];
        const bool min_length = max(top.pe - top.pb, top.te - top.tb) <= FALLBACK_MIN_LENGTH;
        stack[0] = Task{top.pb, top.pe, top.tb, top.te, C_M, C_M, min_length ? 0 : INT_MAX, INT_MAX};
      }
    } else if (tid == 0) {
      const bool min_length = max(plenT, tlenT) <= FALLBACK_MIN_LENGTH;
      stack[0] = Task{0, plenT, 0, tlenT, C_M, C_M, min_length ? 0 : INT_MAX, INT_MAX};
    }
    sp = 1;
    __syncthreads();
    bool top = true;
    while (sp > 0 && status == ST_OK) {
      Task t = stack[sp - 1];
      t.pb = uni(t.pb); t.pe = uni(t.pe); t.tb = uni(t.tb); t.te = uni(t.te);
      t.cb = uni(t.cb); t.ce = uni(t.ce); t.score_remaining = uni(t.score_remaining); t.known = uni(t.known);
      --sp;
      __syncthreads();
      const int plen = t.pe - t.pb, tlen = t.te - t.tb;
      if (tlen == 0) {
        emit_run(em, 'D', plen);
        if (top) penalty = plen > 0 ? min(pn.o1 + plen * pn.e1, P2 ? pn.o2 + plen * pn.e2 : INT_MAX) : 0;
        top = false;
        continue;
      } else if (plen == 0) {
        emit_run(em, 'I', tlen);
        if (top) penalty = min(pn.o1 + tlen * pn.e1, P2 ? pn.o2 + tlen * pn.e2 : INT_MAX);
        top = false;
        continue;
      }
      SubCtx cx;
      cx.plen = plen;
      cx.tlen = tlen;
      cx.P[0] = to_global(Pf + t.pb);
      cx.T[0] = to_global(Tf + t.tb);
      cx.P[1] = to_global(Pr + (plenT - t.pe));
      cx.T[1] = to_global(Tr + (tlenT - t.te));
      cx.kmin[0] = cx.kmin[1] = 0;
      cx.wcols = 0;
      cx.Pw = Pw;
      cx.Tw = Tw;
      cx.pb_abs = t.pb;
      cx.tb_abs = t.tb;
      stage_sequences<OffT>(kp, lds, cx);
      bool do_base = t.score_remaining <= FALLBACK_MIN_SCORE;
      Breakpoint bp;
      if (!do_base) {
        int rc = BP_OK;
        for (int attempt = 0; attempt < AWV_RESTART_ATTEMPTS; ++attempt) {
          if (tid == 0) {
            PassCtx& pc = sh.pctx;
            pc.ring_mem = (unsigned long long)(uintptr_t)ring_mem;
            pc.ring_bytes = (unsigned long long)kp.ring_slot_stride;
            pc.P[0] = (unsigned long long)(uintptr_t)cx.P[0];
            pc.P[1] = (unsigned long long)(uintptr_t)cx.P[1];
            pc.T[0] = (unsigned long long)(uintptr_t)cx.T[0];
            pc.T[1] = (unsigned long long)(uintptr_t)cx.T[1];
            pc.Pw = (unsigned long long)(uintptr_t)cx.Pw;
            pc.Tw = (unsigned long long)(uintptr_t)cx.Tw;
            pc.ring = kp.ring;
            pc.wcap = kp.wcap;
            pc.x = pn.x; pc.o1 = pn.o1; pc.e1 = pn.e1; pc.o2 = pn.o2; pc.e2 = pn.e2;
            pc.lds_meta_bytes = kp.lds_meta_bytes;
            pc.lds_seq_bytes = kp.lds_seq_bytes;
            pc.chain_max = kp.chain_max;
            pc.multi_T = kp.multi_T;
            pc.deep_passes = kp.deep_passes;
            pc.max_penalty = kp.pair_max_penalty ? kp.pair_max_penalty[pair] : kp.max_penalty;
            pc.plen = plen; pc.tlen = tlen;
            pc.seq_mode = cx.seq_mode; pc.p_w0 = cx.p_w0; pc.t_w0 = cx.t_w0; pc.p_bit = cx.p_bit; pc.t_bit = cx.t_bit;
            pc.pb_abs = cx.pb_abs; pc.tb_abs = cx.tb_abs;
          }
          __syncthreads();
          if constexpr (sizeof(OffT) == 4 && !WENC) {
            if (kp.sub16 != 0 && max(plen, tlen) < SUB16_MAX_LEN)
              rc = uni(find_breakpoint_fn<P2, int16_t>((unsigned)(uintptr_t)&sh, (unsigned)(uintptr_t)lds.ring_meta, (unsigned)(uintptr_t)lstats,
                                                       t.cb, t.ce, t.score_remaining, t.known, attempt | 0x100));
            else
              rc = uni(find_breakpoint_fn<P2, OffT>((unsigned)(uintptr_t)&sh, (unsigned)(uintptr_t)lds.ring_meta, (unsigned)(uintptr_t)lstats,
                                                    t.cb, t.ce, t.score_remaining, t.known, attempt));
          } else {
            rc = uni(find_breakpoint_fn<P2, OffT>((unsigned)(uintptr_t)&sh, (unsigned)(uintptr_t)lds.ring_meta, (unsigned)(uintptr_t)lstats,
                                                  t.cb, t.ce, t.score_remaining, t.known, attempt));
          }
          if (rc == BP_OK) {
            bp.score = uni(sh.bp_out.score); bp.sf = uni(sh.bp_out.sf); bp.sr = uni(sh.bp_out.sr); bp.kf = uni(sh.bp_out.kf);
            bp.kr = uni(sh.bp_out.kr); bp.off_f = uni(sh.bp_out.off_f); bp.off_r = uni(sh.bp_out.off_r); bp.comp = uni(sh.bp_out.comp);
          }
          if (rc != BP_RESTART) break;
          if (tid == 0) lstats[STAT_RESTARTS] += 1;
        }
        if (rc == BP_END_REACHED) do_base = true;
        else if (rc == BP_ABOVE_BOUND) { status = ST_ABOVE_BOUND; break; }
        else if (rc != BP_OK) { status = rc; break; }
      }
      if (do_base) {
        int pen_b = 0;
        const int rc = base_align<P2, OffT>(kp, sh, lds, cx, hist, hist_rs, events, t.cb, t.ce, em, pen_b, lstats);
        if (rc != ST_OK) { status = rc; break; }
        if (top) penalty = pen_b;
        top = false;
        continue;
      }
      if (kp.score_only) {
        penalty = bp.score;
        break;
      }
      const int bh = bp.off_f, bv = bp.off_f - bp.kf;
      if (bh < 0 || bh > tlen || bv < 0 || bv > plen || sp + 2 > STACK_CAP) { status = ST_INTERNAL; break; }
      if (tid == 0) {
        const int open_c = bp.comp == C_M ? 0 : ((bp.comp == C_I1 || bp.comp == C_D1) ? kp.pen.o1 : kp.pen.o2);
        stack[sp] = Task{t.pb + bv, t.pe, t.tb + bh, t.te, bp.comp, t.ce, bp.sr, bp.sr - open_c};
        stack[sp + 1] = Task{t.pb, t.pb + bv, t.tb, t.tb + bh, t.cb, bp.comp, bp.sf, bp.sf - open_c};
      }
      sp += 2;
      if (top) penalty = bp.score;
      top = false;
      __syncthreads();
    }
// ... 45 lines not shown
```

### allwave_amd/csrc/engine.hip

```cpp
#include "allwave_hip.h"
#include "host_errors.hpp"
#include "planner_device.hpp"
#include "verify_device.hpp"
#include "clip_device.hpp"
#include "split_device.hpp"
#include "normalize_device.hpp"
#include "kernels_awv.hpp"
#define AWV_NS awv
#define AWV_WG 64
#include "biwfa_device.hpp"
#undef AWV_NS
#undef AWV_WG
#define AWV_NS awvw
#define AWV_WG 256
#include "biwfa_device.hpp"
#undef AWV_NS
#undef AWV_WG
#define AWV_NS awvx
#define AWV_WG 1024
#include "biwfa_device.hpp"
#undef AWV_NS
#undef AWV_WG
#define AWV_WIDE16 1
#define AWV_NS awvw_m
#define AWV_WG 256
#include "biwfa_device.hpp"
#undef AWV_NS
#undef AWV_WG
#define AWV_NS awvx_m
#define AWV_WG 1024
#include "biwfa_device.hpp"
#undef AWV_NS
#undef AWV_WG
#undef AWV_WIDE16

#include <algorithm>
#include <chrono>
#include <climits>
#include <cmath>
#include <cstdio>
#include <cstdlib>
#include <cstring>
#include <exception>
#include <string>
#include <thread>
#include <vector>

#include "batch_plan.hpp"
#include "twin_plan.hpp"

namespace {
const awvb::Limits LIMITS = {awv::TMAX, awv::TMAX32, awv::CHAIN_MAX, awv::MAX_RING, awv::MAX_SCOPE, awv::NCOMP, awv::COL_PAD,
                             awv::FALLBACK_MIN_SCORE, awv::FALLBACK_MIN_LENGTH, awv::WAVES_PER_SIMD, awv::STATIC_LDS_RESERVE,
                             (size_t)awv::EV_STACK_WORDS, (size_t)awv::EV_TWIN_WORDS, sizeof(awv::RowMeta), sizeof(awv::RowMeta16),
                             sizeof(awv::Breakpoint)};
static_assert(awv::EV_STACK_WORDS == (awv::STACK_CAP * sizeof(awv::Task) + 3) / 4 + 16, "DFS stack words");

thread_local std::string g_last_error;

int fail(int code, const std::string& msg) {
  g_last_error = msg;
  return code;
}

template <typename T>
struct DevBuf {
  T* p = nullptr;
  size_t cap = 0;
  int reserve(size_t n) {
    if (n <= cap) return AWV_OK;
    if (p) (void)hipFree(p);
    p = nullptr;
    cap = 0;
    size_t want = n + std::min<size_t>(n / 8, (size_t)64 << 20) + 64;
    hipError_t e = hipMalloc((void**)&p, want * sizeof(T));
    if (e != hipSuccess) {
      want = n;
      e = hipMalloc((void**)&p, want * sizeof(T));
    }
    if (e != hipSuccess) {
      p = nullptr;
      return fail(AWV_ERR_OOM, std::string("hipMalloc ") + std::to_string(want * sizeof(T)) + " bytes: " + hipGetErrorString(e));
    }
    cap = want;
    return AWV_OK;
  }
  void release() {
    if (p) (void)hipFree(p);
    p = nullptr;
    cap = 0;
  }
  void adopt(T* q, size_t n) {
    release();
    p = q;
    cap = n;
  }
  size_t bytes() const { return cap * sizeof(T); }
};

struct SeqSet {
  int32_t n = 0;
  std::vector<uint64_t> off;
  std::vector<int32_t> len;
  DevBuf<uint8_t> d_seq[4];
  DevBuf<uint64_t> d_off;
  DevBuf<int32_t> d_len;
  DevBuf<uint32_t> d_seq2[2];
  DevBuf<uint64_t> d_off2;
  DevBuf<uint8_t> d_ok2;
  size_t total = 0;
  void release() {
    for (auto& b : d_seq) b.release();
    for (auto& b : d_seq2) b.release();
    d_off2.release();
    d_ok2.release();
    d_off.release();
    d_len.release();
    n = 0;
  }
};

inline uint8_t rc_base(uint8_t b) {
  switch (b) {
    case 'A': case 'a': return 'T';
    case 'T': case 't': return 'A';
    case 'C': case 'c': return 'G';
    case 'G': case 'g': return 'C';
    default: return 'N';
  }
}

}

struct awv_engine {
  awv_engine_config cfg{};
  int device = 0;
  int num_cus = 0;
  int wall_clock_khz = 100000;
  hipStream_t stream = nullptr;
  hipEvent_t ev0 = nullptr, ev1 = nullptr;
  SeqSet seqs;
  DevBuf<uint8_t> ring_mem, hist_mem;
  DevBuf<uint32_t> ev_mem;
  DevBuf<int32_t> d_pair_q, d_pair_t, d_pair_rc;
  DevBuf<int32_t> d_pair_bound;
  DevBuf<int32_t> d_unit_first, d_unit_twin;
  uint64_t twin_stats[4] = {0, 0, 0, 0};
  DevBuf<awvr::Span> d_pair_span;
  DevBuf<uint64_t> d_cigar_off;
  DevBuf<awv::DevResult> d_results;
  DevBuf<uint8_t> d_cigar;
  DevBuf<unsigned long long> d_counters;
  std::vector<uint8_t> h_cigar;
  struct HostStage {
    std::vector<int32_t> hq, ht, hrc, hbound, hufirst, hutwin;
    std::vector<uint64_t> hoff;
    std::vector<awvr::Span> hspan;
    std::vector<awv_result> tres;
  } stage;
  awv_stats stats{};
  awp::PlanState* plan = nullptr;
  awvf::State* verify = nullptr;
  awvc::State* clip = nullptr;
  awvs::State* split = nullptr;
  awvn::State* normalize = nullptr;
  int32_t norm_mode = AWV_NORM_OFF;
};

namespace {

int upload_seqset(awv_engine* e, SeqSet& s, int32_t n, const uint8_t* bytes, const uint64_t* offsets) {
  if (n < 0 || (n > 0 && (!bytes || !offsets))) return fail(AWV_ERR_ARG, "set_sequences: null input");
  s.n = 0;
  s.off.assign((size_t)n + 1, 0);
  s.len.assign((size_t)n, 0);
  uint64_t run = 0;
  for (int i = 0; i < n; ++i) {
    if (offsets[i + 1] < offsets[i]) return fail(AWV_ERR_ARG, "set_sequences: offsets not monotone");
    const uint64_t l = offsets[i + 1] - offsets[i];
    if (l > (uint64_t)(INT32_MAX / 4)) return fail(AWV_ERR_ARG, "set_sequences: sequence too long");
    s.off[i] = run;
    s.len[i] = (int32_t)l;
    run += l + awp::SEQ_PAD_BYTES;
  }
  s.off[n] = run;
  s.total = run + 64;
  std::vector<uint8_t> h[4];
  for (auto& v : h) v.assign(s.total, 0);
  for (int i = 0; i < n; ++i) {
    const uint8_t* src = bytes + offsets[i];
    const size_t l = (size_t)s.len[i];
    uint8_t* f = h[0].data() + s.off[i];
    uint8_t* r = h[1].data() + s.off[i];
    uint8_t* c = h[2].data() + s.off[i];
    uint8_t* cr = h[3].data() + s.off[i];
    for (size_t j = 0; j < l; ++j) {
      const uint8_t b = src[j];
      f[j] = b;
      r[l - 1 - j] = b;
      const uint8_t cb = rc_base(b);
      c[l - 1 - j] = cb;
      cr[j] = cb;
    }
  }
  std::vector<uint64_t> off2((size_t)n + 1, 2);
  std::vector<uint8_t> ok2((size_t)std::max(n, 1), 0);
  for (int i = 0; i < n; ++i) off2[i + 1] = off2[i] + ((size_t)s.len[i] + 15) / 16 + 1;
  std::vector<uint32_t> h2[2];
  for (auto& v : h2) v.assign(off2[n] + 4, 0u);
  auto code = [](uint8_t b) -> int { return b == 'A' ? 0 : b == 'C' ? 1 : b == 'G' ? 2 : b == 'T' ? 3 : -1; };
  for (int i = 0; i < n; ++i) {
    for (int v = 0; v < 2; ++v) {
      const uint8_t* src = h[v ? 2 : 0].data() + s.off[i];
      uint32_t* dst = h2[v].data() + off2[i];
      bool ok = true;
      for (size_t j = 0; j < (size_t)s.len[i]; ++j) {
        const int c = code(src[j]);
        if (c < 0) { ok = false; break; }
        dst[j >> 4] |= (uint32_t)c << (2 * (j & 15));
      }
      if (ok) ok2[i] |= (uint8_t)(1 << v);
    }
  }
  AWV_TRY(hipSetDevice(e->device));
  for (int v = 0; v < 2; ++v) {
    if (int rc = s.d_seq2[v].reserve(h2[v].size())) return rc;
    AWV_TRY(hipMemcpyAsync(s.d_seq2[v].p, h2[v].data(), h2[v].size() * sizeof(uint32_t), hipMemcpyHostToDevice, e->stream));
  }
  if (int rc = s.d_off2.reserve((size_t)n + 1)) return rc;
  if (int rc = s.d_ok2.reserve(ok2.size())) return rc;
  AWV_TRY(hipMemcpyAsync(s.d_off2.p, off2.data(), ((size_t)n + 1) * sizeof(uint64_t), hipMemcpyHostToDevice, e->stream));
  AWV_TRY(hipMemcpyAsync(s.d_ok2.p, ok2.data(), ok2.size(), hipMemcpyHostToDevice, e->stream));
  for (int v = 0; v < 4; ++v) {
    if (int rc = s.d_seq[v].reserve(s.total)) return rc;
    AWV_TRY(hipMemcpyAsync(s.d_seq[v].p, h[v].data(), s.total, hipMemcpyHostToDevice, e->stream));
  }
  if (int rc = s.d_off.reserve((size_t)n + 1)) return rc;
  if (int rc = s.d_len.reserve((size_t)std::max(n, 1))) return rc;
  AWV_TRY(hipMemcpyAsync(s.d_off.p, s.off.data(), ((size_t)n + 1) * sizeof(uint64_t), hipMemcpyHostToDevice, e->stream));
  if (n > 0) AWV_TRY(hipMemcpyAsync(s.d_len.p, s.len.data(), (size_t)n * sizeof(int32_t), hipMemcpyHostToDevice, e->stream));
  AWV_TRY(hipStreamSynchronize(e->stream));
  s.n = n;
  return AWV_OK;
}

int check_penalty_signs(const awv_penalties* p) {
  std::string msg;
  const int rc = awvb::check_signs(p, msg);
  return rc == AWV_OK ? rc : fail(rc, msg);
}

__global__ __launch_bounds__(64, 4) void arena_probe_kernel(unsigned char* arena, size_t slot_stride, int row_bytes, int steps, int width_cols,
                                                             unsigned long long* sink) {
  const int lane = threadIdx.x;
  awv::rsrc_t rs = __builtin_amdgcn_make_buffer_rsrc(arena + (size_t)blockIdx.x * slot_stride, 0, (int)std::min<size_t>(slot_stride, 0x7FFFFFFF), 0x00020000);
  auto off = [&](int dir, int comp, int score) { return ((dir * 5 + comp) * 32 + (score & 31)) * row_bytes; };
  typedef unsigned int u32x2 __attribute__((ext_vector_type(2)));
  unsigned acc = 0;
  for (int s = 32; s < 32 + steps; ++s) {
    for (int dir = 0; dir < 2; ++dir) {
      const int lo = 1024 + (s & 7) * 4;
      for (int cb = lo; cb < lo + width_cols; cb += 248) {
        const int voff = (cb + lane * 4) * 2;
        const u32x2 a = __builtin_amdgcn_raw_buffer_load_b64(rs, voff, off(dir, 0, s - 5), 0);
        const u32x2 b = __builtin_amdgcn_raw_buffer_load_b64(rs, voff, off(dir, 0, s - 10), 0);
        const u32x2 c = __builtin_amdgcn_raw_buffer_load_b64(rs, voff, off(dir, 0, s - 25), 0);
        const u32x2 d = __builtin_amdgcn_raw_buffer_load_b64(rs, voff, off(dir, 1, s - 2), 2);
        const u32x2 f = __builtin_amdgcn_raw_buffer_load_b64(rs, voff, off(dir, 3, s - 2), 2);
        const u32x2 g = __builtin_amdgcn_raw_buffer_load_b64(rs, voff, off(dir, 2, s - 1), 2);
        const u32x2 h = __builtin_amdgcn_raw_buffer_load_b64(rs, voff, off(dir, 4, s - 1), 2);
        const u32x2 m = a + b + c;
        acc += m[0] ^ m[1];
        __builtin_amdgcn_raw_buffer_store_b64(b + d, rs, voff, off(dir, 1, s), 0);
        __builtin_amdgcn_raw_buffer_store_b64(b + f, rs, voff, off(dir, 3, s), 0);
        __builtin_amdgcn_raw_buffer_store_b64(c + g, rs, voff, off(dir, 2, s), 0);
        __builtin_amdgcn_raw_buffer_store_b64(c + h, rs, voff, off(dir, 4, s), 0);
        __builtin_amdgcn_raw_buffer_store_b64(m, rs, voff, off(dir, 0, s), 0);
      }
    }
  }
  if (acc == 0x12345678u) sink[0] = acc;
}

struct SplitOut {
  int64_t min_score;
  const uint64_t* seg_first;
  awv_split_index* iout;
  awv_clip_result* sout;
};
struct AlignRequest {
  const awv_pair* pairs = nullptr;
  int64_t npairs = 0;
  awv_result* out = nullptr;
  awv_sink sink = nullptr;
  void* user = nullptr;
  bool score_only = false;
  int max_penalty = INT_MAX;
  const int32_t* pair_bound = nullptr;
  awv_verify_result* vout = nullptr;
  const awvr::Span* spans = nullptr;
  awv_clip_result* cout = nullptr;
  int32_t match_bonus = 0;
  const SplitOut* split = nullptr;
};

struct SinkRunner {
  std::thread th;
  int rc = 0;
  std::vector<awv_result> res;
  std::vector<uint8_t> cig;
  int wait() {
    if (th.joinable()) th.join();
    const int r = rc;
    rc = 0;
    return r;
  }
  ~SinkRunner() { if (th.joinable()) th.join(); }
};

struct AlignCall {
  awv_engine* e;
  SeqSet& s;
  const awv_penalties* pen;
  const AlignRequest& rq;
  awvb::PenaltyPlan pp;
  awvb::Config cfg;
  int32_t norm = AWV_NORM_OFF;
  bool twin_ok = false;
  int64_t max_batch = 0;
  uint64_t max_arena = 0;
  bool inline_sink = false, timing = false;
  int force_sixteen_len = INT_MAX;
  std::chrono::steady_clock::time_point t0 = std::chrono::steady_clock::now();
  int64_t first = 0, n = 0;
  uint64_t arena = 0;
  std::vector<awvb::Entry> entries;
  std::vector<awv_result> hres;
  double kernel_ms = 0, h2d_ms = 0, d2h_ms = 0;
  unsigned long long stat_tot[awv::STAT_N_DEV] = {0};
  uint64_t launches = 0;
  SinkRunner runner;
  bool want_cigar() const { return rq.sink && !rq.score_only && !(e->cfg.flags & AWV_F_KEEP_ON_DEVICE); }
  void lap(const char* what) const {
    if (timing) fprintf(stderr, "[awv] %-22s %.3f s\n", what, std::chrono::duration<double>(std::chrono::steady_clock::now() - t0).count());
  }
};

void read_knobs(AlignCall& c) {
#ifdef AWV_DEBUG_KNOBS
  if (const char* env = getenv("AWV_MAX_ARENA_MB")) c.max_arena = std::max<uint64_t>(1, (uint64_t)atoll(env)) << 20;
  c.inline_sink = getenv("AWV_INLINE_SINK") != nullptr;
  c.timing = getenv("AWV_TIMING") != nullptr;
  if (const char* env = getenv("AWV_FORCE_SIXTEEN")) c.force_sixteen_len = atoi(env);
#else
  (void)c;
#endif
}

int timer_wait(AlignCall& c, double& acc) {
  float ms = 0;
  AWV_TRY(hipEventSynchronize(c.e->ev1));
  AWV_TRY(hipEventElapsedTime(&ms, c.e->ev0, c.e->ev1));
  acc += ms;
  return AWV_OK;
}
int timer_stop(AlignCall& c, double& acc) {
  AWV_TRY(hipEventRecord(c.e->ev1, c.e->stream));
  return timer_wait(c, acc);
}

bool carve_and_order(AlignCall& c) {
  const AlignRequest& rq = c.rq;
  const awvb::Carve cv = awvb::carve_batch(
      [&](int64_t gi, int32_t& ql, int32_t& tl) {
        if (rq.spans) {
          ql = rq.spans[gi].pe - rq.spans[gi].pb;
          tl = rq.spans[gi].te - rq.spans[gi].tb;
        } else {
          ql = c.s.len[rq.pairs[gi].q_idx];
          tl = c.s.len[rq.pairs[gi].t_idx];
        }
      },
      c.first, rq.npairs, c.max_batch, c.max_arena, rq.score_only, c.entries);
  c.n = cv.n;
  c.arena = cv.arena;
  for (awvb::Entry& en : c.entries) {
    const awv_pair& p = rq.pairs[c.first + en.batch_index];
    en.q = p.q_idx;
    en.t = p.t_idx;
    en.rc = p.q_revcomp ? 1 : 0;
  }
  return awvb::order_by_cost(c.entries);
}

int reserve_batch_buffers(AlignCall& c) {
  awv_engine* e = c.e;
  const size_t n = (size_t)c.n;
  if (int rc = e->d_pair_q.reserve(n)) return rc;
  if (int rc = e->d_pair_t.reserve(n)) return rc;
  if (int rc = e->d_pair_rc.reserve(n)) return rc;
  if (int rc = e->d_cigar_off.reserve(n)) return rc;
  if (int rc = e->d_results.reserve(n)) return rc;
  if (int rc = e->d_cigar.reserve((size_t)c.arena + 64)) return rc;
  if (int rc = e->d_counters.reserve(1 + awv::STAT_N_DEV)) return rc;
  static_assert(sizeof(awv_result) == sizeof(awv::DevResult), "result layout");
  c.hres.assign(n, awv_result{});
  return AWV_OK;
}

void drop_beyond_span(AlignCall& c, std::vector<awvb::Entry>& ge, int width) {
  const long long span = awvb::capacity_span(LIMITS, awvb::wc_2g(LIMITS, c.pp.ring, width));
  size_t k = 0;
  for (size_t i = 0; i < ge.size(); ++i) {
    const awvb::Entry en = ge[i];
    if (awvb::beyond_span(en.ql, en.tl, span)) {
      awv_result r{};
      r.status = AWV_ST_CAPACITY;
      r.cigar_off = en.off;
      c.hres[(size_t)en.batch_index] = r;
      continue;
    }
    ge[k++] = en;
  }
  ge.resize(k);
}

int choose_ring_arena(AlignCall& c, const awvb::RowPlan& rp, int wc, int nslots) {
  awv_engine* e = c.e;
  const size_t ring_stride = rp.ring_stride(wc);
  const size_t want = ring_stride * (size_t)nslots + ((size_t)64 << 20);
  size_t free_b = 0, total_b = 0;
  e->ring_mem.release();
  (void)hipMemGetInfo(&free_b, &total_b);
  int ncand = (e->cfg.flags & AWV_F_NO_ARENA_PROBE) ? 1 : 4;
  while (ncand > 1 && (size_t)ncand * want > free_b / 10 * 8) --ncand;
  const bool probe_ok = ncand > 1 && want >= ((size_t)1 << 30) && rp.esz == 2 && ring_stride >= (size_t)2 * 5 * 32 * 4096 &&
                        (size_t)wc * rp.esz >= 4096;
  if (!probe_ok) ncand = 1;
  uint8_t* cand[4] = {nullptr, nullptr, nullptr, nullptr};
  float cms[4] = {0, 0, 0, 0};
  int best = -1;
  for (int k = 0; k < ncand; ++k) {
    if (hipMalloc((void**)&cand[k], want) != hipSuccess) { cand[k] = nullptr; (void)hipGetLastError(); break; }
    if (ncand == 1) { best = 0; break; }
    float tbest = 1e30f;
    hipError_t perr = hipSuccess;
    for (int rep = 0; rep < 2 && perr == hipSuccess; ++rep) {
      float pms = 0;
      if ((perr = hipEventRecord(e->ev0, e->stream)) != hipSuccess) break;
      hipLaunchKernelGGL(arena_probe_kernel, dim3(nslots), dim3(64), 0, e->stream, cand[k], ring_stride, (int)((size_t)wc * rp.esz), 24,
                         std::min(1400, wc - 2048), e->d_counters.p);
      if ((perr = hipEventRecord(e->ev1, e->stream)) != hipSuccess) break;
      if ((perr = hipEventSynchronize(e->ev1)) != hipSuccess) break;
      if ((perr = hipEventElapsedTime(&pms, e->ev0, e->ev1)) != hipSuccess) break;
      tbest = std::min(tbest, pms);
    }
    if (perr != hipSuccess) {
      for (int j = 0; j < 4; ++j)
        if (cand[j]) (void)hipFree(cand[j]);
      return fail(AWV_ERR_HIP, std::string("ring arena probe: ") + hipGetErrorString(perr));
    }
    cms[k] = tbest;
    if (best < 0 || tbest < cms[best]) best = k;
    if (c.timing) fprintf(stderr, "[awv] ring arena candidate %d at %p: %.2f ms\n", k, (void*)cand[k], tbest);
  }
  if (best < 0) return fail(AWV_ERR_OOM, "hipMalloc " + std::to_string(want) + " bytes for the ring arena failed");
  for (int k = 0; k < 4; ++k)
    if (k != best && cand[k]) (void)hipFree(cand[k]);
  e->ring_mem.adopt(cand[best], want);
  return AWV_OK;
}

int ensure_arenas(AlignCall& c, const awvb::RowPlan& rp, int wc, int nslots) {
  awv_engine* e = c.e;
  if (rp.ring_stride(wc) * nslots > e->ring_mem.cap)
    if (int rc = choose_ring_arena(c, rp, wc, nslots)) return rc;
  if (int rc = e->hist_mem.reserve(rp.hist_stride * nslots)) return rc;
  if (int rc = e->ev_mem.reserve(rp.ev_stride(wc) * nslots)) return rc;
  return AWV_OK;
}

int upload_twin_units(AlignCall& c, const std::vector<awvb::Entry>& ge, int64_t& nunits) {
  awv_engine* e = c.e;
  awv_engine::HostStage& st = e->stage;
  const awvt::TwinPlan tp = awvt::plan_twins(st.hq.data(), st.ht.data(), st.hrc.data(), ge.size());
  std::vector<size_t> uo(tp.first.size());
  for (size_t u = 0; u < uo.size(); ++u) uo[u] = u;
  auto ucost = [&](size_t u) {
    const awvb::Entry& en = ge[(size_t)tp.first[u]];
    const uint64_t cost = awvb::pair_cost(en.ql, en.tl);
    return tp.twin[u] >= 0 ? 2 * cost : cost;
  };
  std::stable_sort(uo.begin(), uo.end(), [&](size_t a, size_t b) { return ucost(a) > ucost(b); });
  st.hufirst.resize(uo.size());
  st.hutwin.resize(uo.size());
  for (size_t u = 0; u < uo.size(); ++u) {
    st.hufirst[u] = tp.first[uo[u]];
    st.hutwin[u] = tp.twin[uo[u]];
  }
  nunits = (int64_t)uo.size();
  if (int rc = e->d_unit_first.reserve((size_t)nunits)) return rc;
  if (int rc = e->d_unit_twin.reserve((size_t)nunits)) return rc;
  AWV_TRY(hipMemcpyAsync(e->d_unit_first.p, st.hufirst.data(), (size_t)nunits * 4, hipMemcpyHostToDevice, e->stream));
  AWV_TRY(hipMemcpyAsync(e->d_unit_twin.p, st.hutwin.data(), (size_t)nunits * 4, hipMemcpyHostToDevice, e->stream));
  return AWV_OK;
}

int upload_group(AlignCall& c, const std::vector<awvb::Entry>& ge, const awvb::RowPlan& rp, int64_t& nunits) {
  awv_engine* e = c.e;
  awv_engine::HostStage& st = e->stage;
  const AlignRequest& rq = c.rq;
  const size_t m = ge.size();
  st.hq.resize(m); st.ht.resize(m); st.hrc.resize(m); st.hoff.resize(m);
  for (size_t i = 0; i < m; ++i) {
    st.hq[i] = ge[i].q; st.ht[i] = ge[i].t; st.hrc[i] = ge[i].rc; st.hoff[i] = ge[i].off;
  }
  AWV_TRY(hipEventRecord(e->ev0, e->stream));
  AWV_TRY(hipMemcpyAsync(e->d_pair_q.p, st.hq.data(), m * 4, hipMemcpyHostToDevice, e->stream));
  AWV_TRY(hipMemcpyAsync(e->d_pair_t.p, st.ht.data(), m * 4, hipMemcpyHostToDevice, e->stream));
  AWV_TRY(hipMemcpyAsync(e->d_pair_rc.p, st.hrc.data(), m * 4, hipMemcpyHostToDevice, e->stream));
  AWV_TRY(hipMemcpyAsync(e->d_cigar_off.p, st.hoff.data(), m * 8, hipMemcpyHostToDevice, e->stream));
  if (rq.pair_bound) {
    st.hbound.resize(m);
    for (size_t i = 0; i < m; ++i) st.hbound[i] = rq.pair_bound[c.first + ge[i].batch_index];
    if (int rc = e->d_pair_bound.reserve(m)) return rc;
    AWV_TRY(hipMemcpyAsync(e->d_pair_bound.p, st.hbound.data(), m * 4, hipMemcpyHostToDevice, e->stream));
  }
  if (rq.spans) {
    st.hspan.resize(m);
    for (size_t i = 0; i < m; ++i) st.hspan[i] = rq.spans[c.first + ge[i].batch_index];
    if (int rc = e->d_pair_span.reserve(m)) return rc;
    AWV_TRY(hipMemcpyAsync(e->d_pair_span.p, st.hspan.data(), m * sizeof(awvr::Span), hipMemcpyHostToDevice, e->stream));
  }
  nunits = (int64_t)m;
  if (rp.twin_here)
    if (int rc = upload_twin_units(c, ge, nunits)) return rc;
  AWV_TRY(hipMemsetAsync(e->d_counters.p, 0, (1 + awv::STAT_N_DEV) * sizeof(unsigned long long), e->stream));
  return timer_stop(c, c.h2d_ms);
}

awv::KParams fill_kparams(const AlignCall& c, const awvb::RowPlan& rp, int wc, int64_t nunits) {
  const awv_engine* e = c.e;
  const SeqSet& s = c.s;
  const bool narrow = rp.width != 1;
  awv::KParams kp{};
  for (int v = 0; v < 4; ++v) kp.seq[v] = s.d_seq[v].p;
  kp.seq_off = s.d_off.p;
  kp.seq_len = s.d_len.p;
  kp.seq2[0] = s.d_seq2[0].p;
  kp.seq2[1] = s.d_seq2[1].p;
  kp.seq2_off = s.d_off2.p;
  kp.seq2_ok = s.d_ok2.p;
  kp.pair_q = e->d_pair_q.p;
  kp.pair_t = e->d_pair_t.p;
  kp.pair_rc = e->d_pair_rc.p;
  kp.npairs = nunits;
  kp.unit_first = rp.twin_here ? e->d_unit_first.p : nullptr;
  kp.unit_twin = rp.twin_here ? e->d_unit_twin.p : nullptr;
  kp.twin_levels = (e->cfg.flags & AWV_F_TWIN_TOP_ONLY) ? 1 : INT_MAX;
  kp.twin_base = (e->cfg.flags & AWV_F_NO_TWIN_BASE) ? 0 : 1;
  kp.pen = awv::DevPenalties{c.pp.x, c.pp.o1, c.pp.e1, c.pp.o2, c.pp.e2, c.pp.two_piece, c.pp.scope};
  kp.ring = c.pp.ring;
  kp.multi_T = narrow ? c.pp.multi_T : (std::min(c.pp.multi_T, awv::TMAX32) >= 2 ? std::min(c.pp.multi_T, awv::TMAX32) : 0);
  kp.deep_passes = (kp.multi_T > 0 && !(e->cfg.flags & AWV_F_NO_DEEP)) ? 1 : 0;
  kp.sub16 = (e->cfg.flags & AWV_F_FORCE_INT32) ? 0 : 1;
  kp.chain_max = narrow ? c.pp.chain_max : (awv::TMAX32 == awv::TMAX ? std::min(c.pp.chain_max, 3) : 1);
  kp.wcap = wc;
  kp.ring_mem = e->ring_mem.p;
  kp.ring_slot_stride = rp.ring_stride(wc);
  kp.lds_meta_bytes = (int)rp.lds_meta;
  kp.lds_seq_bytes = (int)rp.lds_seq;
  kp.sb_cap = c.pp.sb_cap;
  kp.wb_cap = c.pp.wb_cap;
  kp.hist_mem = e->hist_mem.p;
  kp.hist_slot_stride = rp.hist_stride;
  kp.hist_meta_offset = rp.hist_rows;
  kp.ev_mem = e->ev_mem.p;
  kp.ev_slot_stride = rp.ev_stride(wc);
  kp.cigar = e->d_cigar.p;
  kp.cigar_off = e->d_cigar_off.p;
  kp.results = e->d_results.p;
  kp.work_counter = e->d_counters.p;
  kp.stats = e->d_counters.p + 1;
  kp.score_only = c.rq.score_only ? 1 : 0;
  kp.max_penalty = c.rq.max_penalty;
  kp.pair_max_penalty = c.rq.pair_bound ? e->d_pair_bound.p : nullptr;
  return kp;
}

struct LaunchShape {
  unsigned grid;
  int wg;
  size_t dyn_lds;
  hipStream_t stream;
  bool two_piece, narrow;
  const awvr::Span* d_span;
};
#define AWV_KERNELS_OF(NS)                                                                   \
  struct NS##_kernels {                                                                      \
    typedef NS::KParams KParams;                                                             \
    static constexpr bool only16 = NS::WENC;                                                 \
    template <bool P2, typename OffT, typename... S>                                         \
    static auto kernel() { return &NS::biwfa_align_kernel<P2, OffT, S...>; }                \
  }
AWV_KERNELS_OF(awvw);
AWV_KERNELS_OF(awvx);
AWV_KERNELS_OF(awvw_m);
AWV_KERNELS_OF(awvx_m);
#undef AWV_KERNELS_OF
template <typename K, typename KP, typename... PairSpan>
int launch_kernel(K kern, const LaunchShape& l, const KP& kparams, PairSpan... pair_span) {
  AWV_TRY(hipFuncSetAttribute((const void*)kern, hipFuncAttributeMaxDynamicSharedMemorySize, (int)l.dyn_lds));
  hipLaunchKernelGGL(kern, dim3(l.grid), dim3(l.wg), l.dyn_lds, l.stream, kparams, pair_span...);
  return AWV_OK;
}
template <typename NS, bool P2, typename OffT>
int launch_ranged(const LaunchShape& l, const typename NS::KParams& k) {
  if (l.d_span) return launch_kernel(NS::template kernel<P2, OffT, const awvr::Span*>(), l, k, l.d_span);
  return launch_kernel(NS::template kernel<P2, OffT>(), l, k);
}
template <typename NS, bool P2>
int launch_rows(const LaunchShape& l, const typename NS::KParams& k) {
  if constexpr (NS::only16) return launch_ranged<NS, P2, int16_t>(l, k);
  else return l.narrow ? launch_ranged<NS, P2, int16_t>(l, k) : launch_ranged<NS, P2, int32_t>(l, k);
}
template <typename NS>
int launch_flavour(const LaunchShape& l, const awv::KParams& kp) {
  static_assert(sizeof(typename NS::KParams) == sizeof(awv::KParams), "same parameter block for every workgroup size");
  typename NS::KParams k;
  std::memcpy(&k, &kp, sizeof(k));
  return l.two_piece ? launch_rows<NS, true>(l, k) : launch_rows<NS, false>(l, k);
}

int launch_group(AlignCall& c, const awvb::RowPlan& rp, const awv::KParams& kp, int nslots) {
  awv_engine* e = c.e;
  const LaunchShape l{(unsigned)nslots, rp.wg, rp.dyn_lds, e->stream, kp.pen.two_piece != 0, rp.width != 1, c.rq.spans ? e->d_pair_span.p : nullptr};
  AWV_TRY(hipEventRecord(e->ev0, e->stream));
  if (rp.waves == 1) AWV_TRY((hipError_t)awv_launch_one_wave(l.two_piece, l.narrow ? 1 : 0, l.d_span, l.grid, l.dyn_lds, l.stream, &kp));
  else if (int rc = rp.width == 2 ? (rp.waves == 4 ? launch_flavour<awvw_m_kernels>(l, kp) : launch_flavour<awvx_m_kernels>(l, kp))
                                  : (rp.waves == 4 ? launch_flavour<awvw_kernels>(l, kp) : launch_flavour<awvx_kernels>(l, kp)))
    return rc;
  AWV_TRY(hipGetLastError());
  AWV_TRY(hipEventRecord(e->ev1, e->stream));
  if (c.want_cigar() && e->h_cigar.size() < (size_t)c.arena + 64) e->h_cigar.resize((size_t)c.arena + 64);
  if (int rc = timer_wait(c, c.kernel_ms)) return rc;
  ++c.launches;
  c.lap("kernel done");
  return AWV_OK;
}

int read_back(AlignCall& c, const std::vector<awvb::Entry>& ge) {
  awv_engine* e = c.e;
  awv_engine::HostStage& st = e->stage;
  const size_t m = ge.size();
  st.tres.resize(m);
  AWV_TRY(hipEventRecord(e->ev0, e->stream));
  AWV_TRY(hipMemcpyAsync(st.tres.data(), e->d_results.p, m * sizeof(awv_result), hipMemcpyDeviceToHost, e->stream));
  unsigned long long hstat[1 + awv::STAT_N_DEV];
  AWV_TRY(hipMemcpyAsync(hstat, e->d_counters.p, sizeof(hstat), hipMemcpyDeviceToHost, e->stream));
  if (int rc = timer_stop(c, c.d2h_ms)) return rc;
  for (int i = 0; i < awv::STAT_N_DEV; ++i) c.stat_tot[i] += hstat[1 + i];
  for (size_t i = 0; i < m; ++i) c.hres[(size_t)ge[i].batch_index] = st.tres[i];
  return AWV_OK;
}

void select_reruns(const AlignCall& c, std::vector<awvb::Entry>& ge, bool wider_rows_left) {
  const awv_engine::HostStage& st = c.e->stage;
  size_t k = 0;
  if (wider_rows_left && !(c.e->cfg.flags & AWV_F_NO_RERUN))
    for (size_t i = 0; i < ge.size(); ++i)
      if (st.tres[i].status == AWV_ST_CAPACITY) ge[k++] = ge[i];
  ge.resize(k);
}

int run_group(AlignCall& c, std::vector<awvb::Entry>& ge, const awvb::RowPlan& rp) {
  for (int wc = rp.wcap; !ge.empty(); wc = rp.next_wc(wc)) {
    const int nslots = rp.slots(wc, (int64_t)ge.size());
    if (int rc = ensure_arenas(c, rp, wc, nslots)) return rc;
    c.lap("arenas reserved");
    if (c.timing) fprintf(stderr, "[awv] ring arena %p (%zu MiB), hist %p, cigar %p\n", (void*)c.e->ring_mem.p, c.e->ring_mem.bytes() >> 20, (void*)c.e->hist_mem.p, (void*)c.e->d_cigar.p);
    int64_t nunits = 0;
    if (int rc = upload_group(c, ge, rp, nunits)) return rc;
    if (int rc = launch_group(c, rp, fill_kparams(c, rp, wc, nunits), nslots)) return rc;
    if (int rc = read_back(c, ge)) return rc;
    select_reruns(c, ge, wc < rp.wc_last);
  }
  return AWV_OK;
}

int run_groups(AlignCall& c, bool skewed) {
  const awvb::GroupPlan gp = awvb::assign_groups(LIMITS, c.cfg, c.entries, skewed, c.force_sixteen_len);
  std::vector<awvb::Entry> ge[awvb::NG];
  for (int g = 0; g < awvb::NG; ++g) ge[g].reserve(gp.count[g]);
  for (size_t i = 0; i < c.entries.size(); ++i) ge[gp.group[i]].push_back(c.entries[i]);
  awvb::RowPlan rp[awvb::NG];
  for (int k = 0; k < awvb::NG; ++k) {
    const int g = gp.demand_order[k];
    drop_beyond_span(c, ge[g], awvb::width_of(g));
    if (ge[g].empty()) continue;
    rp[g] = awvb::plan_rows(LIMITS, c.cfg, c.pp, ge[g], awvb::waves_of(g), awvb::width_of(g), c.twin_ok);
    if (int rc = ensure_arenas(c, rp[g], rp[g].wcap, rp[g].slots(rp[g].wcap, (int64_t)ge[g].size()))) return rc;
  }
  for (int g = awvb::NG - 1; g >= 0; --g)
    if (int rc = run_group(c, ge[g], rp[g])) return rc;
  return AWV_OK;
}

int run_record_steps(AlignCall& c) {
  awv_engine* e = c.e;
  const AlignRequest& rq = c.rq;
  const SeqSet& s = c.s;
  const int64_t first = c.first, n = c.n;
  const uint64_t arena = c.arena;
  std::vector<awv_result>& hres = c.hres;
  if (c.norm != AWV_NORM_OFF) {
    const awvn::SeqView sv{s.n, s.d_seq[0].p, s.d_seq[2].p, s.d_off.p, s.d_len.p};
    if (int rc = awvn::normalize_batch(e, sv, c.norm, rq.pairs + first, n, hres.data(), e->d_cigar.p, arena, rq.spans ? rq.spans + first : nullptr)) return rc;
    c.lap("batch normalized");
  }
  if (rq.vout) {
    if (int rc = awvf::verify_batch(e, c.pen, rq.pairs + first, n, hres.data(), e->d_cigar.p, arena, rq.vout + first, rq.spans ? rq.spans + first : nullptr)) return rc;
    c.lap("batch verified");
  }
  if (rq.cout) {
    if (int rc = awvc::clip_batch(e, c.pen, rq.match_bonus, n, hres.data(), e->d_cigar.p, arena, rq.cout + first)) return rc;
    c.lap("batch clipped");
  }
  if (rq.split) {
    if (int rc = awvs::split_batch(e, c.pen, rq.match_bonus, rq.split->min_score, n, hres.data(), e->d_cigar.p, arena, rq.split->seg_first + first,
                                   rq.split->iout + first, rq.split->sout)) return rc;
    c.lap("batch split");
  }
  return AWV_OK;
}

int copy_cigars_back(AlignCall& c) {
  awv_engine* e = c.e;
  if (c.want_cigar()) {
    e->h_cigar.resize((size_t)c.arena + 64);
    c.lap("host cigar buffer");
    AWV_TRY(hipEventRecord(e->ev0, e->stream));
    AWV_TRY(hipMemcpyAsync(e->h_cigar.data(), e->d_cigar.p, (size_t)c.arena, hipMemcpyDeviceToHost, e->stream));
    if (int rc = timer_stop(c, c.d2h_ms)) return rc;
  }
  c.lap("cigars on host");
  return AWV_OK;
}

int deliver(AlignCall& c) {
  const AlignRequest& rq = c.rq;
  if (rq.out) std::memcpy(rq.out + c.first, c.hres.data(), (size_t)c.n * sizeof(awv_result));
  if (!rq.sink) return AWV_OK;
  const bool want_cigar = c.want_cigar();
  const awv_sink sink = rq.sink;
  void* const user = rq.user;
  if (const int prc = c.runner.wait()) return fail(AWV_ERR_SINK, "sink callback returned " + std::to_string(prc));
  if (c.first + c.n >= rq.npairs || c.inline_sink) {
    const int rc = sink(user, c.first, c.n, c.hres.data(), want_cigar ? c.e->h_cigar.data() : nullptr);
    if (rc != 0) return fail(AWV_ERR_SINK, "sink callback returned " + std::to_string(rc));
    c.lap("sink returned");
    return AWV_OK;
  }
  c.runner.res.swap(c.hres);
  c.runner.cig.swap(c.e->h_cigar);
  const awv_result* rp = c.runner.res.data();
  const uint8_t* cp = want_cigar ? c.runner.cig.data() : nullptr;
  const int64_t f0 = c.first, n0 = c.n;
  SinkRunner* rn = &c.runner;
  try {
    c.runner.th = std::thread([rn, sink, user, f0, n0, rp, cp]() { rn->rc = sink(user, f0, n0, rp, cp); });
    c.lap("sink handed off");
  } catch (const std::exception&) {
    const int rc = sink(user, f0, n0, rp, cp);
    if (rc != 0) return fail(AWV_ERR_SINK, "sink callback returned " + std::to_string(rc));
  }
  return AWV_OK;
}

void publish_stats(AlignCall& c) {
  using namespace awv;
  awv_engine* e = c.e;
  const unsigned long long* stat_tot = c.stat_tot;
  e->stats.kernel_ms = c.kernel_ms;
  e->stats.h2d_ms = c.h2d_ms;
  e->stats.d2h_ms = c.d2h_ms;
  e->stats.launches = c.launches;
  e->stats.cell_steps = stat_tot[STAT_CELLS];
  e->stats.extend_steps = stat_tot[STAT_EXTEND];
  e->stats.n_breakpoints = stat_tot[STAT_BREAKPOINTS];
  e->stats.n_base = stat_tot[STAT_BASE];
  e->stats.overlap_scans = stat_tot[STAT_OVERLAP];
  e->stats.aligned_bp = stat_tot[STAT_ALIGNED_BP];
  e->stats.pairs_completed = stat_tot[STAT_PAIRS];
  e->stats.scratch_bytes = e->ring_mem.bytes() + e->hist_mem.bytes() + e->ev_mem.bytes();
  for (int i = 0; i < 14; ++i) e->stats.prof[i] = stat_tot[STAT_T_TOTAL + i];
  e->stats.restarts = stat_tot[STAT_RESTARTS];
  e->stats.multi_cell_steps = stat_tot[STAT_MULTI_CELLS];
  e->stats.windows[0] = stat_tot[STAT_WIN_SINGLE];
  e->stats.windows[1] = stat_tot[STAT_WIN_MULTI];
  e->stats.windows[2] = stat_tot[STAT_WIN_BASE];
  e->stats.windows[3] = stat_tot[STAT_WIN_BASE_MULTI];
  e->stats.clock_cycles = stat_tot[STAT_CLK_CYCLES];
  e->stats.clock_ticks = stat_tot[STAT_CLK_TICKS];
  e->stats.clock_tick_khz = (uint64_t)e->wall_clock_khz;
  e->stats.deep_cell_steps = stat_tot[STAT_DEEP_CELLS];
  for (int i = 0; i < 4; ++i) e->twin_stats[i] = stat_tot[STAT_TWIN_UNITS + i];
}

int align_core(awv_engine* e, SeqSet& s, const awv_penalties* pen, const AlignRequest& rq) {
  if (rq.npairs < 0 || (rq.npairs > 0 && !rq.pairs)) return fail(AWV_ERR_ARG, "align_pairs: null pairs");
  AlignCall c{e, s, pen, rq};
  c.pp = awvb::plan_penalties(LIMITS, pen, e->cfg.flags);
  if (c.pp.code != AWV_OK && !c.pp.late) return fail(c.pp.code, c.pp.message);
  AWV_TRY(hipSetDevice(e->device));
  e->stats = awv_stats{};
  for (uint64_t& v : e->twin_stats) v = 0;
  c.norm = rq.score_only ? AWV_NORM_OFF : e->norm_mode;
  if (c.norm != AWV_NORM_OFF) awvn::stats_reset(e->normalize);
  if (rq.npairs == 0) return AWV_OK;
  for (int64_t i = 0; i < rq.npairs; ++i) {
    if (rq.pairs[i].q_idx < 0 || rq.pairs[i].q_idx >= s.n || rq.pairs[i].t_idx < 0 || rq.pairs[i].t_idx >= s.n)
      return fail(AWV_ERR_ARG, "align_pairs: sequence index out of range");
  }
  if (c.pp.code != AWV_OK) return fail(c.pp.code, c.pp.message);
  c.cfg = awvb::Config{e->cfg.flags, e->num_cus, e->cfg.workgroups, (int64_t)e->cfg.max_scratch_bytes, e->cfg.first_row_cols};
  c.max_batch = e->cfg.max_batch_pairs > 0 ? e->cfg.max_batch_pairs : (int64_t)1 << 20;
  c.max_arena = e->cfg.max_arena_bytes > 0 ? (uint64_t)e->cfg.max_arena_bytes : (uint64_t)8 << 30;
  c.twin_ok = rq.max_penalty == INT_MAX && !rq.pair_bound && !rq.spans && !rq.cout && !(e->cfg.flags & (AWV_F_NO_TWIN | AWV_F_NO_RERUN));
  read_knobs(c);
  for (; c.first < rq.npairs; c.first += c.n) {
    const bool skewed = carve_and_order(c);
    if (int rc = reserve_batch_buffers(c)) return rc;
    if (int rc = run_groups(c, skewed)) return rc;
    c.lap("results on host");
    if (int rc = run_record_steps(c)) return rc;
    if (int rc = copy_cigars_back(c)) return rc;
    if (int rc = deliver(c)) return rc;
  }
  publish_stats(c);
  return AWV_OK;
}

int require_sequences(const awv_engine* e, int64_t n, const char* who) {
  if (e->seqs.n == 0 && n > 0) return fail(AWV_ERR_STATE, std::string(who) + " before set_sequences");
  return AWV_OK;
}
int32_t norm_bound(int32_t b) { return b < 0 || b >= (1 << 30) ? INT_MAX : b; }
const int32_t* normalized_bounds(const int32_t* bounds, int64_t n, std::vector<int32_t>& store) {
  if (!bounds || n <= 0) return nullptr;
  store.resize((size_t)n);
  for (int64_t i = 0; i < n; ++i) store[(size_t)i] = norm_bound(bounds[i]);
  return store.data();
}
AlignRequest full_request(const awv_pair* pairs, int64_t npairs, awv_result* out, awv_sink sink, void* user) {
  AlignRequest rq;
  rq.pairs = pairs;
  rq.npairs = npairs;
  rq.out = out;
  rq.sink = sink;
  rq.user = user;
  return rq;
}

}

extern "C" {

int awv_abi_version(void) { return AWV_ABI_VERSION; }

const char* awv_last_error(void) { return g_last_error.c_str(); }

int awv_engine_create(const awv_engine_config* cfg, awv_engine** out) {
  if (!out) return fail(AWV_ERR_ARG, "engine_create: null out");
  *out = nullptr;
  int ndev = 0;
  hipError_t err = hipGetDeviceCount(&ndev);
  if (err != hipSuccess || ndev <= 0)
    return fail(AWV_ERR_NO_DEVICE, std::string("no HIP device available (") + hipGetErrorString(err) +
                                       "): liballwave_hip has no CPU fallback");
  awv_engine* e = new awv_engine();
  if (cfg) e->cfg = *cfg;
  e->device = e->cfg.device;
  if (e->device < 0 || e->device >= ndev) {
    delete e;
    return fail(AWV_ERR_ARG, "engine_create: device ordinal out of range");
  }
  auto bail = [&](hipError_t he, const char* what) {
    std::string m = std::string(what) + ": " + hipGetErrorString(he);
    awv_engine_destroy(e);
    return fail(AWV_ERR_HIP, m);
  };
  hipError_t he;
  if ((he = hipSetDevice(e->device)) != hipSuccess) return bail(he, "hipSetDevice");
  hipDeviceProp_t prop;
  if ((he = hipGetDeviceProperties(&prop, e->device)) != hipSuccess) return bail(he, "hipGetDeviceProperties");
  e->num_cus = prop.multiProcessorCount;
  {
    int khz = 0;
    if (hipDeviceGetAttribute(&khz, hipDeviceAttributeWallClockRate, e->device) == hipSuccess && khz > 0) e->wall_clock_khz = khz;
    else (void)hipGetLastError();
  }
  if ((he = hipStreamCreateWithFlags(&e->stream, hipStreamNonBlocking)) != hipSuccess) return bail(he, "hipStreamCreate");
  if ((he = hipEventCreate(&e->ev0)) != hipSuccess) return bail(he, "hipEventCreate");
  if ((he = hipEventCreate(&e->ev1)) != hipSuccess) return bail(he, "hipEventCreate");
  *out = e;
  return AWV_OK;
}

void awv_engine_destroy(awv_engine* e) {
  if (!e) return;
  (void)hipSetDevice(e->device);
  awp::plan_state_release(e->plan);
  e->plan = nullptr;
  awvf::state_release(e->verify);
  e->verify = nullptr;
  awvc::state_release(e->clip);
  e->clip = nullptr;
  awvs::state_release(e->split);
  e->split = nullptr;
  awvn::state_release(e->normalize);
  e->normalize = nullptr;
  e->seqs.release();
  e->ring_mem.release();
  e->hist_mem.release();
  e->ev_mem.release();
  e->d_pair_q.release();
  e->d_pair_t.release();
  e->d_pair_rc.release();
  e->d_pair_bound.release();
  e->d_pair_span.release();
  e->d_cigar_off.release();
  e->d_results.release();
  e->d_cigar.release();
  e->d_counters.release();
  if (e->ev0) (void)hipEventDestroy(e->ev0);
  if (e->ev1) (void)hipEventDestroy(e->ev1);
  if (e->stream) (void)hipStreamDestroy(e->stream);
  delete e;
}

int awv_engine_set_sequences(awv_engine* e, int32_t n, const uint8_t* concat_bytes, const uint64_t* offsets) {
  if (!e) return fail(AWV_ERR_ARG, "null engine");
  awp::plan_state_release(e->plan);
  e->plan = nullptr;
  AWV_GUARDED(return upload_seqset(e, e->seqs, n, concat_bytes, offsets);)
}

int awv_align_pairs(awv_engine* e, const awv_penalties* pen, const awv_pair* pairs, int64_t npairs, awv_result* out,
                    awv_sink sink, void* user) {
  if (!e) return fail(AWV_ERR_ARG, "null engine");
  if (int rc = require_sequences(e, npairs, "align_pairs")) return rc;
  AWV_GUARDED(return align_core(e, e->seqs, pen, full_request(pairs, npairs, out, sink, user));)
}

int awv_align_pairs_verified(awv_engine* e, const awv_penalties* pen, const awv_pair* pairs, int64_t npairs, awv_result* out,
                             awv_verify_result* vout, awv_sink sink, void* user) {
  if (!e) return fail(AWV_ERR_ARG, "null engine");
  if (!vout) return fail(AWV_ERR_ARG, "align_pairs_verified: null vout");
  if (int rc = require_sequences(e, npairs, "align_pairs")) return rc;
  awvf::stats_reset(e->verify);
  AlignRequest rq = full_request(pairs, npairs, out, sink, user);
  rq.vout = vout;
  AWV_GUARDED(return align_core(e, e->seqs, pen, rq);)
}

namespace {
int score_core(awv_engine* e, const awv_penalties* pen, AlignRequest rq, awv_score_result* out) {
  if (!e) return awv_internal_null_engine();
  if (!out) return fail(AWV_ERR_ARG, "score_pairs: null out");
  if (rq.npairs < 0) return fail(AWV_ERR_ARG, "score_pairs: npairs < 0");
  if (int rc = require_sequences(e, rq.npairs, "score_pairs")) return rc;
  AWV_GUARDED(
    std::vector<awv_result> res((size_t)rq.npairs);
    std::vector<int32_t> pb;
    rq.out = res.data();
    rq.score_only = true;
    rq.max_penalty = norm_bound(rq.max_penalty);
    rq.pair_bound = normalized_bounds(rq.pair_bound, rq.npairs, pb);
    const int rc = align_core(e, e->seqs, pen, rq);
    if (rc != AWV_OK) return rc;
    for (int64_t i = 0; i < rq.npairs; ++i) {
      out[i].status = res[(size_t)i].status;
      out[i].penalty = res[(size_t)i].penalty;
    }
    return AWV_OK;
  )
}
}

int awv_score_pairs(awv_engine* e, const awv_penalties* pen, const awv_pair* pairs, int64_t npairs, int32_t max_penalty,
                    awv_score_result* out) {
  AlignRequest rq = full_request(pairs, npairs, nullptr, nullptr, nullptr);
  rq.max_penalty = max_penalty;
  return score_core(e, pen, rq, out);
}

int awv_score_pairs_bounded(awv_engine* e, const awv_penalties* pen, const awv_pair* pairs, int64_t npairs,
                            const int32_t* max_penalty, awv_score_result* out) {
  if (e && npairs > 0 && !max_penalty) return fail(AWV_ERR_ARG, "score_pairs_bounded: null max_penalty");
  AlignRequest rq = full_request(pairs, npairs, nullptr, nullptr, nullptr);
  rq.max_penalty = -1;
  rq.pair_bound = max_penalty;
  return score_core(e, pen, rq, out);
}

namespace {
int split_ranges(const SeqSet& s, const awv_range_pair* ranges, int64_t n, std::vector<awv_pair>& pairs, std::vector<awvr::Span>& spans,
                 const char* who) {
  pairs.resize((size_t)n);
  spans.resize((size_t)n);
  for (int64_t i = 0; i < n; ++i)
    if (!awvr::split_range(s.len.data(), s.n, ranges[i], pairs[(size_t)i], spans[(size_t)i]))
      return fail(AWV_ERR_ARG, std::string(who) + ": range " + std::to_string(i) + " names a sequence index or an interval out of range");
  return AWV_OK;
}
int check_split_args(int32_t match_bonus, const SplitOut& sp, int64_t n) {
  if (match_bonus < 1 || match_bonus > AWV_CLIP_MAX_BONUS) return fail(AWV_ERR_ARG, "align_split: match_bonus must be in [1, 32767]");
  if (sp.min_score < 1) return fail(AWV_ERR_ARG, "align_split: min_score must be >= 1");
  if (!sp.seg_first || (n > 0 && !sp.iout)) return fail(AWV_ERR_ARG, "align_split: null seg_first or iout");
  for (int64_t i = 0; i < n; ++i)
    if (sp.seg_first[i + 1] < sp.seg_first[i]) return fail(AWV_ERR_ARG, "align_split: seg_first must ascend");
  if (n > 0 && sp.seg_first[n] > sp.seg_first[0] && !sp.sout) return fail(AWV_ERR_ARG, "align_split: null sout");
  return AWV_OK;
}
int check_split_slots(const SplitOut& sp, int64_t i, int32_t match_bonus, int64_t shorter) {
  if (sp.seg_first[i + 1] - sp.seg_first[i] < (uint64_t)awvs::slots(match_bonus, sp.min_score, shorter))
    return fail(AWV_ERR_ARG, "align_split: entry " + std::to_string(i) + " owns fewer slots than awv_split_slots(a, min_score, min(plen, tlen))");
  return AWV_OK;
}
int align_ranges_core(awv_engine* e, const awv_penalties* pen, const awv_range_pair* ranges, int64_t n, AlignRequest rq) {
  if (n < 0 || (n > 0 && !ranges)) return fail(AWV_ERR_ARG, "align_ranges: null ranges");
  if (int rc = require_sequences(e, n, "align_ranges")) return rc;
  std::vector<awv_pair> pairs;
  std::vector<awvr::Span> spans;
  if (int rc = split_ranges(e->seqs, ranges, n, pairs, spans, "align_ranges")) return rc;
  if (rq.vout) awvf::stats_reset(e->verify);
  if (n == 0) return align_core(e, e->seqs, pen, full_request(nullptr, 0, rq.out, rq.sink, rq.user));
  if (rq.split)
    for (int64_t i = 0; i < n; ++i) {
      const awvr::Span& sp = spans[(size_t)i];
      if (int rc = check_split_slots(*rq.split, i, rq.match_bonus, std::min(sp.pe - sp.pb, sp.te - sp.tb))) return rc;
    }
  std::vector<int32_t> pb;
  rq.pairs = pairs.data();
  rq.npairs = n;
  rq.spans = spans.data();
  rq.pair_bound = normalized_bounds(rq.pair_bound, n, pb);
  return align_core(e, e->seqs, pen, rq);
}
int check_clip_args(const awv_clip_result* cout, int32_t match_bonus) {
  if (!cout) return fail(AWV_ERR_ARG, "align_clipped: null cout");
  if (match_bonus < 1 || match_bonus > AWV_CLIP_MAX_BONUS) return fail(AWV_ERR_ARG, "align_clipped: match_bonus must be in [1, 32767]");
  return AWV_OK;
}
}

int awv_align_pairs_clipped(awv_engine* e, const awv_penalties* pen, const awv_pair* pairs, int64_t npairs, const int32_t* max_penalty,
                            int32_t match_bonus, awv_result* out, awv_verify_result* vout, awv_clip_result* cout, awv_sink sink, void* user) {
  if (!e) return fail(AWV_ERR_ARG, "null engine");
  if (int rc = check_clip_args(cout, match_bonus)) return rc;
  if (int rc = require_sequences(e, npairs, "align_pairs")) return rc;
  if (vout) awvf::stats_reset(e->verify);
  awvc::stats_reset(e->clip);
  AWV_GUARDED(
    std::vector<int32_t> pb;
    AlignRequest rq = full_request(pairs, npairs, out, sink, user);
    rq.pair_bound = normalized_bounds(max_penalty, npairs, pb);
    rq.vout = vout;
    rq.cout = cout;
    rq.match_bonus = match_bonus;
    return align_core(e, e->seqs, pen, rq);
  )
}

int awv_align_ranges_clipped(awv_engine* e, const awv_penalties* pen, const awv_range_pair* ranges, int64_t n, const int32_t* max_penalty,
                             int32_t match_bonus, awv_result* out, awv_verify_result* vout, awv_clip_result* cout, awv_sink sink, void* user) {
  if (!e) return fail(AWV_ERR_ARG, "null engine");
  if (int rc = check_clip_args(cout, match_bonus)) return rc;
// ... 223 lines not shown
```

### allwave_amd/ffi.py

```python
import ctypes as C
import os

import numpy as np

_HERE = os.path.dirname(os.path.abspath(__file__))
LIB_PATH = os.environ.get("AWV_HIP_LIB") or os.path.join(_HERE, "liballwave_hip.so")

AWV_OK = 0
AWV_ERR_NO_DEVICE = -1
AWV_ERR_ARG = -3
AWV_ERR_STATE = -6
AWV_ERR_SINK = -7
AWV_ST_COMPLETED = 0
AWV_ST_CAPACITY = 1
AWV_ST_ABOVE_BOUND = 4
AWV_F_KEEP_ON_DEVICE = 1
AWV_F_FORCE_INT32 = 2
AWV_F_NO_PACKED_SEQ = 4
AWV_F_ONE_WAVE = 8
AWV_F_FOUR_WAVES = 16
AWV_F_NO_ARENA_PROBE = 32
AWV_F_SINGLE_STEP = 64
AWV_F_NO_CHAIN = 128
AWV_F_NO_WIDE16 = 256
AWV_F_NO_DEEP = 512
AWV_F_NO_RERUN = 1024
AWV_F_NO_TWIN = 2048
AWV_F_TWIN_TOP_ONLY = 4096
AWV_F_NO_TWIN_BASE = 8192
AWV_ORIENT_FORWARD = 0
AWV_ORIENT_REVERSE = 1
AWV_ORIENT_UNDECIDED = 2
AWV_ORIENT_BY_BOUND = 0
AWV_ORIENT_BY_EDITS = 1
AWV_ORIENT_FULL = 1
AWV_ORIENT_SKIP_RATIO = 8
AWV_ORIENT_NO_EDITS = 2 ** 64 - 1
AWV_ORIENT_HI_NONE = 2 ** 31 - 1
AWV_VF_OK = 0
AWV_VF_SKIPPED = 1
AWV_VF_BAD_OP = 2
AWV_VF_OVERRUN = 3
AWV_VF_M_DIFFERS = 4
AWV_VF_X_EQUAL = 5
AWV_VF_SHORT = 6
AWV_VF_COUNTS = 7
AWV_VF_PENALTY = 8
AWV_CL_OK = 0
AWV_CL_SKIPPED = 1
AWV_CL_EMPTY = 2
AWV_CL_BAD_OP = 3
AWV_CLIP_MAX_BONUS = 32767
AWV_NORM_OFF = 0
AWV_NORM_LEFT = 1
AWV_NORM_RIGHT = 2
AWV_NM_OK = 0
AWV_NM_SKIPPED = 1
AWV_NM_BAD_OP = 2
AWV_NM_LENGTHS = 3
AWV_SK_CANONICAL = 0
AWV_SK_FORWARD = 1
AWV_SK_REVCOMP = 2

EXPORTS = ("awv_abi_version", "awv_last_error", "awv_engine_create", "awv_engine_destroy",
           "awv_engine_set_sequences", "awv_align_pairs", "awv_align_one", "awv_score_pairs", "awv_engine_stats",
           "awv_score_pairs_bounded", "awv_orient_pairs", "awv_orient_decide", "awv_orient_settling_bound",
           "awv_sketch", "awv_sketch_copy", "awv_sketch_pair_counts", "awv_sketch_rows", "awv_sketch_knn", "awv_keep_pairs",
           "awv_align_pairs_verified", "awv_verify_cigars", "awv_verify_one_host", "awv_engine_verify_stats",
           "awv_align_ranges", "awv_align_ranges_verified", "awv_score_ranges", "awv_verify_ranges",
           "awv_align_pairs_bounded", "awv_align_ranges_bounded", "awv_divergence_bound",
           "awv_clip_one_host", "awv_clip_cigars", "awv_align_pairs_clipped", "awv_align_ranges_clipped", "awv_engine_clip_stats",
           "awv_twin_stats",
           "awv_split_slots", "awv_split_layout_pairs", "awv_split_layout_ranges", "awv_split_one_host", "awv_split_cigars",
           "awv_align_pairs_split", "awv_align_ranges_split", "awv_engine_split_stats",
           "awv_normalize_one_host", "awv_normalize_cigars", "awv_normalize_ranges", "awv_engine_set_normalize",
           "awv_engine_normalize_stats")


class EngineConfig(C.Structure):
    _fields_ = [("device", C.c_int32), ("workgroups", C.c_int32), ("max_batch_pairs", C.c_int64),
                ("max_arena_bytes", C.c_int64), ("flags", C.c_int32), ("first_row_cols", C.c_int32),
                ("max_scratch_bytes", C.c_int64)]


class Penalties(C.Structure):
    _fields_ = [(n, C.c_int32) for n in
                ("match", "mismatch", "gap_open1", "gap_ext1", "gap_open2", "gap_ext2", "two_piece")]

    @classmethod
    def from_scores(cls, scores):
        s = [int(v) for v in scores]
        if len(s) == 6:
            return cls(s[0], s[1], s[2], s[3], s[4], s[5], 1)
        if len(s) == 4:
            return cls(s[0], s[1], s[2], s[3], 0, 0, 0)
        raise ValueError("Invalid number of scores: %d. Expected 4 or 6 values." % len(s))


class Stats(C.Structure):
    _fields_ = [("kernel_ms", C.c_double), ("h2d_ms", C.c_double), ("d2h_ms", C.c_double),
                ("launches", C.c_uint64), ("cell_steps", C.c_uint64), ("extend_steps", C.c_uint64),
                ("n_breakpoints", C.c_uint64), ("n_base", C.c_uint64), ("overlap_scans", C.c_uint64),
                ("aligned_bp", C.c_uint64), ("pairs_completed", C.c_uint64), ("scratch_bytes", C.c_uint64),
                ("prof", C.c_uint64 * 14), ("restarts", C.c_uint64), ("multi_cell_steps", C.c_uint64), ("windows", C.c_uint64 * 4),
                ("clock_cycles", C.c_uint64), ("clock_ticks", C.c_uint64), ("clock_tick_khz", C.c_uint64),
                ("deep_cell_steps", C.c_uint64)]


class VerifyStats(C.Structure):
    _fields_ = [("kernel_ms", C.c_double), ("pairs", C.c_uint64), ("failed", C.c_uint64), ("columns", C.c_uint64)]


class ClipStats(C.Structure):
    _fields_ = [("kernel_ms", C.c_double), ("pairs", C.c_uint64), ("empty", C.c_uint64), ("columns", C.c_uint64)]


class SplitStats(C.Structure):
    _fields_ = [("kernel_ms", C.c_double), ("pairs", C.c_uint64), ("segments", C.c_uint64), ("empty", C.c_uint64), ("columns", C.c_uint64),
                ("columns_scanned", C.c_uint64)]


class NormStats(C.Structure):
    _fields_ = [("kernel_ms", C.c_double), ("pairs", C.c_uint64), ("records_moved", C.c_uint64), ("runs", C.c_uint64),
                ("runs_moved", C.c_uint64), ("columns_moved", C.c_uint64), ("columns", C.c_uint64)]


PAIR_DTYPE = np.dtype([("q_idx", "<i4"), ("t_idx", "<i4"), ("q_revcomp", "<i4")])
RANGE_DTYPE = np.dtype([("q_idx", "<i4"), ("t_idx", "<i4"), ("q_revcomp", "<i4"), ("q_beg", "<i4"), ("q_end", "<i4"),
                        ("t_beg", "<i4"), ("t_end", "<i4")])
RESULT_DTYPE = np.dtype([("status", "<i4"), ("penalty", "<i4"), ("score", "<i4"), ("cigar_len", "<u4"),
                         ("cigar_off", "<u8"), ("num_matches", "<i4"), ("num_mismatches", "<i4"),
                         ("num_ins", "<i4"), ("num_del", "<i4"), ("q_end", "<i4"), ("t_end", "<i4")])
VERIFY_DTYPE = np.dtype([("code", "<i4"), ("reserved", "<i4"), ("column", "<i8"), ("penalty", "<i8")])
CLIP_DTYPE = np.dtype([("code", "<i4"), ("reserved", "<i4"), ("score", "<i8"), ("col_beg", "<u4"), ("col_end", "<u4"),
                       ("q_skip", "<i4"), ("t_skip", "<i4"), ("num_matches", "<i4"), ("num_mismatches", "<i4"),
                       ("num_ins", "<i4"), ("num_del", "<i4"), ("penalty", "<i4"), ("reserved2", "<i4")])
SPLIT_INDEX_DTYPE = np.dtype([("code", "<i4"), ("count", "<i4"), ("column", "<i8")])
NORM_DTYPE = np.dtype([("code", "<i4"), ("runs_moved", "<i4"), ("columns_moved", "<i8"), ("max_shift", "<i4"), ("reserved", "<i4")])
SCORE_DTYPE = np.dtype([("status", "<i4"), ("penalty", "<i4")])

ORIENT_DTYPE = np.dtype([("is_reverse", "<i4"), ("how", "<i4"), ("lo_f", "<i4"), ("hi_f", "<i4"), ("lo_r", "<i4"), ("hi_r", "<i4"),
                         ("edits_f", "<u8"), ("edits_r", "<u8"), ("rounds", "<i4"), ("reserved", "<i4")])

SINK_FN = C.CFUNCTYPE(C.c_int, C.c_void_p, C.c_int64, C.c_int64, C.c_void_p, C.c_void_p)

_LIB = None


def load():
    global _LIB
    if _LIB is None:
        if not os.path.exists(LIB_PATH):
            raise RuntimeError("%s is missing: run `python -c 'import __graft_entry__ as g; g.build()'`" % LIB_PATH)
        L = C.CDLL(LIB_PATH)
        L.awv_abi_version.restype = C.c_int
        L.awv_last_error.restype = C.c_char_p
        L.awv_engine_create.argtypes = [C.POINTER(EngineConfig), C.POINTER(C.c_void_p)]
        L.awv_engine_destroy.argtypes = [C.c_void_p]
        L.awv_engine_destroy.restype = None
        L.awv_engine_set_sequences.argtypes = [C.c_void_p, C.c_int32, C.c_void_p, C.c_void_p]
        L.awv_align_pairs.argtypes = [C.c_void_p, C.POINTER(Penalties), C.c_void_p, C.c_int64, C.c_void_p,
                                      SINK_FN, C.c_void_p]
        L.awv_align_one.argtypes = [C.c_void_p, C.POINTER(Penalties), C.c_char_p, C.c_int32, C.c_char_p, C.c_int32,
                                    C.c_void_p, C.c_void_p, C.c_size_t]
        L.awv_score_pairs.argtypes = [C.c_void_p, C.POINTER(Penalties), C.c_void_p, C.c_int64, C.c_int32, C.c_void_p]
        L.awv_engine_stats.argtypes = [C.c_void_p, C.POINTER(Stats)]
        L.awv_twin_stats.argtypes = [C.c_void_p, C.POINTER(C.c_uint64 * 4)]
        L.awv_score_pairs_bounded.argtypes = [C.c_void_p, C.POINTER(Penalties), C.c_void_p, C.c_int64, C.c_void_p, C.c_void_p]
        L.awv_orient_pairs.argtypes = [C.c_void_p, C.POINTER(Penalties), C.c_void_p, C.c_int64, C.c_int32, C.c_void_p]
        L.awv_orient_decide.argtypes = [C.POINTER(Penalties), C.c_int32, C.c_int32, C.c_int32, C.c_int32]
        L.awv_orient_settling_bound.argtypes = [C.POINTER(Penalties), C.c_int32, C.c_int32]
        L.awv_orient_settling_bound.restype = C.c_int32
        L.awv_align_pairs_verified.argtypes = [C.c_void_p, C.POINTER(Penalties), C.c_void_p, C.c_int64, C.c_void_p, C.c_void_p,
                                               SINK_FN, C.c_void_p]
        L.awv_verify_cigars.argtypes = [C.c_void_p, C.POINTER(Penalties), C.c_void_p, C.c_int64, C.c_void_p, C.c_void_p, C.c_uint64,
                                        C.c_void_p]
        L.awv_verify_one_host.argtypes = [C.POINTER(Penalties), C.c_char_p, C.c_int32, C.c_char_p, C.c_int32, C.c_char_p, C.c_int64,
                                          C.c_void_p, C.c_void_p]
        L.awv_engine_verify_stats.argtypes = [C.c_void_p, C.POINTER(VerifyStats)]
        L.awv_align_ranges.argtypes = L.awv_align_pairs.argtypes
        L.awv_align_ranges_verified.argtypes = L.awv_align_pairs_verified.argtypes
        L.awv_score_ranges.argtypes = L.awv_score_pairs_bounded.argtypes
# ... 481 lines not shown
```

### include/allwave_hip.h

```cpp
#ifndef ALLWAVE_HIP_H
#define ALLWAVE_HIP_H

#include <stddef.h>
#include <stdint.h>

#ifdef __cplusplus
extern "C" {
#endif

#define AWV_ABI_VERSION 3

#define AWV_OK 0
#define AWV_ERR_NO_DEVICE (-1)
#define AWV_ERR_HIP (-2)
#define AWV_ERR_ARG (-3)
#define AWV_ERR_PENALTIES (-4)
#define AWV_ERR_OOM (-5)
#define AWV_ERR_STATE (-6)
#define AWV_ERR_SINK (-7)

#define AWV_ST_COMPLETED 0
#define AWV_ST_CAPACITY 1
#define AWV_ST_INTERNAL 2
#define AWV_ST_MAX_STEPS 3
#define AWV_ST_ABOVE_BOUND 4

typedef struct awv_engine awv_engine;

typedef struct {
  int32_t device;
  int32_t workgroups;
  int64_t max_batch_pairs;
  int64_t max_arena_bytes;
  int32_t flags;
  int32_t first_row_cols;
  int64_t max_scratch_bytes;
} awv_engine_config;

#define AWV_F_KEEP_ON_DEVICE 1
#define AWV_F_NO_ARENA_PROBE 32
#define AWV_F_NO_RERUN 1024
#define AWV_F_FORCE_INT32 2
#define AWV_F_NO_WIDE16 256
#define AWV_F_NO_PACKED_SEQ 4
#define AWV_F_ONE_WAVE 8
#define AWV_F_FOUR_WAVES 16
#define AWV_F_NO_CHAIN 128
#define AWV_F_NO_DEEP 512
#define AWV_F_SINGLE_STEP 64
#define AWV_F_NO_TWIN 2048
#define AWV_F_TWIN_TOP_ONLY 4096
#define AWV_F_NO_TWIN_BASE 8192

typedef struct {
  int32_t match;
  int32_t mismatch;
  int32_t gap_open1;
  int32_t gap_ext1;
  int32_t gap_open2;
  int32_t gap_ext2;
  int32_t two_piece;
} awv_penalties;

typedef struct {
  int32_t q_idx;
  int32_t t_idx;
  int32_t q_revcomp;
} awv_pair;

typedef struct {
  int32_t status;
  int32_t penalty;
  int32_t score;
  uint32_t cigar_len;
  uint64_t cigar_off;
  int32_t num_matches;
  int32_t num_mismatches;
  int32_t num_ins;
  int32_t num_del;
  int32_t q_end;
  int32_t t_end;
} awv_result;

typedef int (*awv_sink)(void* user, int64_t first, int64_t n, const awv_result* results,
                        const uint8_t* cigar_arena);

typedef struct {
  double kernel_ms;
  double h2d_ms, d2h_ms;
  uint64_t launches;
  uint64_t cell_steps;
  uint64_t extend_steps;
  uint64_t n_breakpoints;
  uint64_t n_base;
  uint64_t overlap_scans;
  uint64_t aligned_bp;
  uint64_t pairs_completed;
  uint64_t scratch_bytes;
  uint64_t prof[14];
  uint64_t restarts;
  uint64_t multi_cell_steps;
  uint64_t windows[4];
  uint64_t clock_cycles, clock_ticks;
  uint64_t clock_tick_khz;
  uint64_t deep_cell_steps;
} awv_stats;

int awv_abi_version(void);
const char* awv_last_error(void);

int awv_engine_create(const awv_engine_config* cfg, awv_engine** out);
void awv_engine_destroy(awv_engine* e);

int awv_engine_set_sequences(awv_engine* e, int32_t n, const uint8_t* concat_bytes,
                             const uint64_t* offsets);

int awv_align_pairs(awv_engine* e, const awv_penalties* pen, const awv_pair* pairs, int64_t npairs,
                    awv_result* out, awv_sink sink, void* user);

int awv_align_one(awv_engine* e, const awv_penalties* pen, const uint8_t* pattern, int32_t plen,
                  const uint8_t* text, int32_t tlen, awv_result* result, uint8_t* cigar_buf,
                  size_t cigar_cap);

typedef struct {
  int32_t status;
  int32_t penalty;
} awv_score_result;
int awv_score_pairs(awv_engine* e, const awv_penalties* pen, const awv_pair* pairs, int64_t npairs,
                    int32_t max_penalty , awv_score_result* out );

int awv_score_pairs_bounded(awv_engine* e, const awv_penalties* pen, const awv_pair* pairs, int64_t npairs,
                            const int32_t* max_penalty , awv_score_result* out );

#define AWV_ORIENT_FORWARD 0
#define AWV_ORIENT_REVERSE 1
#define AWV_ORIENT_UNDECIDED 2
#define AWV_ORIENT_SKIP_RATIO 8
#define AWV_ORIENT_BY_BOUND 0
#define AWV_ORIENT_BY_EDITS 1
#define AWV_ORIENT_FULL 1
#define AWV_ORIENT_NO_EDITS UINT64_MAX

typedef struct {
  int32_t is_reverse;
  int32_t how;
  int32_t lo_f, hi_f;
  int32_t lo_r, hi_r;
  uint64_t edits_f;
  uint64_t edits_r;
  int32_t rounds;
  int32_t reserved;
} awv_orient_result;

int awv_orient_pairs(awv_engine* e, const awv_penalties* pen, const awv_pair* pairs, int64_t npairs, int32_t flags,
                     awv_orient_result* out );
int awv_orient_decide(const awv_penalties* pen, int32_t lo_f, int32_t hi_f, int32_t lo_r, int32_t hi_r);
int32_t awv_orient_settling_bound(const awv_penalties* pen, int32_t known_is_reverse, int32_t penalty);

int awv_engine_stats(const awv_engine* e, awv_stats* out);
int awv_twin_stats(const awv_engine* e, uint64_t out[4]);

#define AWV_VF_OK 0
#define AWV_VF_SKIPPED 1
#define AWV_VF_BAD_OP 2
#define AWV_VF_OVERRUN 3
#define AWV_VF_M_DIFFERS 4
#define AWV_VF_X_EQUAL 5
#define AWV_VF_SHORT 6
#define AWV_VF_COUNTS 7
#define AWV_VF_PENALTY 8

typedef struct {
  int32_t code;
  int32_t reserved;
  int64_t column;
  int64_t penalty;
} awv_verify_result;

typedef struct {
  double kernel_ms;
  uint64_t pairs;
  uint64_t failed;
  uint64_t columns;
} awv_verify_stats;

int awv_align_pairs_verified(awv_engine* e, const awv_penalties* pen, const awv_pair* pairs, int64_t npairs, awv_result* out,
                             awv_verify_result* vout , awv_sink sink, void* user);
int awv_verify_cigars(awv_engine* e, const awv_penalties* pen, const awv_pair* pairs, int64_t npairs, const awv_result* results,
                      const uint8_t* cigar_arena, uint64_t arena_bytes, awv_verify_result* vout );
int awv_verify_one_host(const awv_penalties* pen, const uint8_t* pattern, int32_t plen, const uint8_t* text, int32_t tlen,
                        const uint8_t* cigar, int64_t n, const awv_result* claimed, awv_verify_result* out);
int awv_engine_verify_stats(const awv_engine* e, awv_verify_stats* out);

typedef struct {
  int32_t q_idx, t_idx, q_revcomp;
  int32_t q_beg, q_end;
  int32_t t_beg, t_end;
} awv_range_pair;

int awv_align_ranges(awv_engine* e, const awv_penalties* pen, const awv_range_pair* ranges, int64_t n, awv_result* out,
                     awv_sink sink, void* user);
int awv_align_ranges_verified(awv_engine* e, const awv_penalties* pen, const awv_range_pair* ranges, int64_t n, awv_result* out,
                              awv_verify_result* vout , awv_sink sink, void* user);
int awv_score_ranges(awv_engine* e, const awv_penalties* pen, const awv_range_pair* ranges, int64_t n,
                     const int32_t* max_penalty , awv_score_result* out );
// ... 137 lines not shown
```

Baseline: 759.4 million.

## Archive wavefront rows across passes and reuse them for repeated alignments

Adds per-workgroup row archives in global memory that record ring rows, metadata and per-pass bounding boxes during a recording pass. Later coverage passes over the same pair (forward or reverse) can skip recomputing archived score passes and hand archived rows back into the ring. The goal is to avoid redundant wavefront extension work between repeated BiWFA passes, at the cost of extra device memory, extra global copies and added branching in the multi-phase loop.

Measured after the change: 782.1 million, median of 6. +3.0%, better.

```diff
diff --git a/allwave_amd/build.py b/allwave_amd/build.py
--- a/allwave_amd/build.py
+++ b/allwave_amd/build.py
@@ -28,7 +28,7 @@
 HIP_FLAGS_AWV = HIP_FLAGS + ["-mllvm", "-amdgpu-sched-strategy=max-ilp"]
 HIP_UNITS = (("engine.hip", HIP_FLAGS), ("kernels_awv.hip", HIP_FLAGS_AWV), ("planner.hip", HIP_FLAGS), ("orient.hip", HIP_FLAGS),
              ("verify.hip", HIP_FLAGS), ("clip.hip", HIP_FLAGS), ("split.hip", HIP_FLAGS), ("normalize.hip", HIP_FLAGS))
-HIP_SOURCES = [os.path.join(CSRC, f) for f in ("engine.hip", "kernels_awv.hip", "kernels_awv.hpp", "biwfa_device.hpp", "range_span.hpp", "batch_plan.hpp", "twin_plan.hpp", "twin_base.hpp", "planner.hip",
+HIP_SOURCES = [os.path.join(CSRC, f) for f in ("engine.hip", "kernels_awv.hip", "kernels_awv.hpp", "biwfa_device.hpp", "range_span.hpp", "batch_plan.hpp", "twin_plan.hpp", "twin_base.hpp", "row_reuse.hpp", "planner.hip",
                                                "planner_device.hpp", "orient.hip", "orient_device.hpp", "verify.hip", "verify_device.hpp", "clip.hip", "clip_device.hpp", "clip_scan.hpp", "split.hip", "split_device.hpp", "normalize.hip", "normalize_device.hpp", "wave_ops.hpp",
                                                "host_errors.hpp", "record_pass.hpp", "record_pieces.hpp")] + [ABI_HEADER]
 
diff --git a/allwave_amd/csrc/biwfa_device.hpp b/allwave_amd/csrc/biwfa_device.hpp
--- a/allwave_amd/csrc/biwfa_device.hpp
+++ b/allwave_amd/csrc/biwfa_device.hpp
@@ -6,6 +6,7 @@
 
 #include "range_span.hpp"
 #include "twin_base.hpp"
+#include "row_reuse.hpp"
 
 #ifndef AWV_NS
 #define AWV_NS awv
@@ -63,6 +64,7 @@
        STAT_DEEP_CELLS,
        STAT_N,
        STAT_TWIN_UNITS = STAT_N, STAT_TWIN_SHARED, STAT_TWIN_SOLO, STAT_TWIN_NONMIRROR,
+       STAT_REUSE_CELLS, STAT_REUSE_SEARCHES,
        STAT_N_DEV };
 
 #ifdef AWV_PROF
@@ -121,6 +123,7 @@
   int twin_levels;
   int twin_base;
 };
+constexpr int RR_DESC_WORDS = 4;
 
 struct RowMeta { int lo, hi; };
 constexpr int K_BIG = 1 << 28;
@@ -1857,6 +1860,383 @@
     deep_phase<P2, OffT, E1, E2>(sh_addr, dyn_addr, sc, fmax, rmax, Tn, pass, npass, (unsigned)cells, (unsigned)(cells >> 32));
 }
 
+constexpr int RR_RECORD = 0x1000, RR_FWD = 0x2000, RR_REV = 0x4000;
+enum { RRS_ARCH_LO = 0, RRS_ARCH_HI, RRS_PASSES, RRS_T, RRS_NID,
+       RRS_PART,
+       RRS_COV,
+       RRS_N,
+       RRS_KMIN,
+       RRS_BOX,
+       RRS_SKIP = RRS_BOX + 4,
+       RRS_MAXAK,
+       RRS_CELLS,
+       RRS_WORDS };
+static_assert(RRS_WORDS == 16, "the kernel asks for scope * NCOMP >= RRS_WORDS words of Lds::firstk");
+typedef __attribute__((address_space(1))) unsigned char* garch_t;
+
+template <typename OffT>
+struct RrEnv {
+  typedef typename MetaTraits<OffT>::Stored MetaStored;
+  Shared* sh;
+  KParams kp;
+  int plen, tlen, kmin[2], wcols;
+  MetaStored* ring_meta;
+  int* st;
+  garch_t ring, arch;
+  awvrr::Layout al;
+  __device__ __forceinline__ __attribute__((address_space(1))) int* word(size_t byte_off) const { return (__attribute__((address_space(1))) int*)(arch + byte_off); }
+  __device__ __forceinline__ int load(size_t byte_off) const { return uni(__hip_atomic_load((int*)word(byte_off), __ATOMIC_RELAXED, __HIP_MEMORY_SCOPE_AGENT)); }
+  __device__ __forceinline__ garch_t ring_row(int dir, int comp, int score) const { return ring + (unsigned)row_off<false, OffT>(kp, dir, comp, score); }
+};
+template <bool P2, typename OffT>
+__device__ __forceinline__ RrEnv<OffT> rr_env(unsigned sh_addr, unsigned dyn_addr) {
+  static_assert(WG == 64 && sizeof(OffT) == 2 && !wenc_of<OffT>(), "row archives: one wave per workgroup, 16-bit text offsets");
+  RrEnv<OffT> e;
+  e.sh = (Shared*)__builtin_assume_aligned((Shared*)(lds_shared_ptr)(uintptr_t)uni((int)sh_addr), 8);
+  unsigned char* dyn_smem = (unsigned char*)__builtin_assume_aligned((unsigned char*)(lds_bytes_ptr)(uintptr_t)uni((int)dyn_addr), 16);
+  const PassCtx& pc = e.sh->pctx;
+  auto uni64 = [](unsigned long long v) { return ((unsigned long long)(unsigned)uni((int)(v >> 32)) << 32) | (unsigned)uni((int)v); };
+  e.kp = KParams{};
+  e.kp.ring = uni(pc.ring);
+  e.kp.wcap = uni(pc.wcap);
+  e.kp.pen.x = uni(pc.x);
+  e.kp.pen.o1 = uni(pc.o1);
+  e.kp.pen.e1 = uni(pc.e1);
+  e.kp.pen.o2 = uni(pc.o2);
+  e.kp.pen.e2 = uni(pc.e2);
+  e.kp.pen.two_piece = P2 ? 1 : 0;
+  e.kp.pen.scope = max(e.kp.pen.x, max(e.kp.pen.o1 + e.kp.pen.e1, P2 ? e.kp.pen.o2 + e.kp.pen.e2 : 0)) + 1;
+  e.plen = uni(pc.plen);
+  e.tlen = uni(pc.tlen);
+  e.kmin[0] = uni(pc.kmin[0]);
+  e.kmin[1] = uni(pc.kmin[1]);
+  e.wcols = uni(pc.wcols);
+  e.ring_meta = reinterpret_cast<typename RrEnv<OffT>::MetaStored*>(dyn_smem);
+  e.st = reinterpret_cast<int*>(e.ring_meta + 2 * NCOMP * e.kp.ring) + 4 * e.kp.ring;
+  e.ring = (garch_t)(uintptr_t)uni64(pc.ring_mem);
+  e.arch = (garch_t)(uintptr_t)(((unsigned long long)(unsigned)uni(e.st[RRS_ARCH_HI]) << 32) | (unsigned)uni(e.st[RRS_ARCH_LO]));
+  e.al = awvrr::make_layout(uni(e.st[RRS_PASSES]), uni(e.st[RRS_T]), uni(e.st[RRS_NID]));
+  return e;
+}
+
+template <bool P2, typename OffT, int E1, int E2>
+__device__ __attribute__((noinline)) void rr_begin(unsigned sh_addr, unsigned dyn_addr, int s0_v, int t_full_v) {
+  constexpr int NID = 2 * E1 + (P2 ? 2 * E2 : 0);
+  const RrEnv<OffT> e = rr_env<P2, OffT>(sh_addr, dyn_addr);
+  const int part = uni(e.st[RRS_PART]);
+  const bool usable = e.arch != nullptr && uni(s0_v) == 0 && e.al.passes > 0 && e.al.nid == NID && e.al.T == uni(t_full_v);
+  const bool rec = usable && (part & RR_RECORD) != 0;
+  int cov = !usable || rec ? -1 : (part & RR_FWD) ? 0 : (part & RR_REV) ? 1 : -1;
+  int n = 0, kmin = 0;
+  if (rec && threadIdx.x == 0) {
+    *e.word(awvrr::H_KMIN0 * 4) = e.kmin[0];
+    *e.word(awvrr::H_KMIN1 * 4) = e.kmin[1];
+  }
+  if (cov >= 0) {
+    n = e.load(awvrr::H_NPASS * 4);
+    kmin = e.load((cov ? awvrr::H_KMIN1 : awvrr::H_KMIN0) * 4);
+    if (n <= 0) cov = -1;
+  }
+  if (threadIdx.x == 0) {
+    e.st[RRS_PART] = rec ? 1 : 0;
+    e.st[RRS_COV] = cov;
+    e.st[RRS_N] = n;
+    e.st[RRS_KMIN] = kmin;
+    e.st[RRS_BOX] = e.st[RRS_BOX + 1] = e.st[RRS_BOX + 2] = e.st[RRS_BOX + 3] = 0;
+    e.st[RRS_SKIP] = -1;
+    e.st[RRS_MAXAK] = e.st[RRS_CELLS] = 0;
+  }
+  __syncthreads();
+}
+
+template <bool P2, typename OffT, int E1, int E2>
+__device__ __forceinline__ void rr_hand_over(const RrEnv<OffT>& e, int dirc, int sc) {
+  constexpr int NID = 2 * E1 + (P2 ? 2 * E2 : 0);
+  const awvrr::Layout& al = e.al;
+  const int kminC = dirc ? e.kmin[1] : e.kmin[0], kminA = uni(e.st[RRS_KMIN]);
+  const int fc = awvrr::first_col(al, kminA);
+  const int lane = threadIdx.x & 63, rmask = e.kp.ring - 1;
+  typename RrEnv<OffT>::MetaStored* const meta = e.ring_meta + (size_t)dirc * NCOMP * e.kp.ring;
+  auto put_row = [&](int comp, int score, int apass, int arow) {
+    const int w = e.load(al.meta_off() + al.meta_index(dirc, score, C_M) * 4);
+    const RowMeta m{(int)(short)(w & 0xffff), (int)(short)(w >> 16)};
+    if (m.lo > m.hi) return;
+    if (m.lo - kminC < 256 + 1 || m.hi - kminC + 256 + 4 + 2 > e.wcols) {
+      e.sh->error = ST_CAPACITY;
+      return;
+    }
+    const __attribute__((address_space(1))) short* src = (const __attribute__((address_space(1))) short*)(e.arch + al.row_off(dirc, apass, arow));
+    garch_t dst = e.ring_row(dirc, comp, score);
+    const int c_hi = (m.hi - kminC) | 3;
+    for (int c = ((m.lo - kminC) & ~3) + 4 * lane; c <= c_hi; c += 256) {
+      unsigned short v[4];
+#pragma unroll
+      for (int j = 0; j < 4; ++j) {
+        const int k = c + j + kminC;
+        v[j] = (k >= m.lo && k <= m.hi) ? (unsigned short)src[k - kminA - fc] : (unsigned short)NULL16;
+      }
+      typedef unsigned int u32x2r __attribute__((ext_vector_type(2)));
+      u32x2r w2;
+      w2[0] = (unsigned)v[0] | ((unsigned)v[1] << 16);
+      w2[1] = (unsigned)v[2] | ((unsigned)v[3] << 16);
+      *(__attribute__((address_space(1))) u32x2r*)(dst + (size_t)c * 2) = w2;
+    }
+  };
+  if (sc > 0) {
+    const int lastp = sc / al.T - 1;
+    for (int s = max(1, sc + 1 - (e.kp.pen.scope - 1)); s <= sc; ++s) {
+      if (lane < NCOMP)
+        *reinterpret_cast<int*>(&meta[lane * e.kp.ring + (s & rmask)]) = __hip_atomic_load((int*)e.word(al.meta_off() + al.meta_index(dirc, s, lane) * 4), __ATOMIC_RELAXED, __HIP_MEMORY_SCOPE_AGENT);
+      put_row(C_M, s, awvrr::pass_of(al, s), awvrr::row_of(al, s));
+    }
+    for (int q = 0; q < NID; ++q) {
+      int qc, qs;
+      multi_source<P2, E1, E2>(e.kp.pen, sc, q, qc, qs);
+      if (qs >= 1) put_row(qc, qs, lastp, awvrr::id_row(al, E1, E2, qc, sc - qs));
+    }
+  }
+  if (threadIdx.x == 0) {
+    e.st[RRS_COV] = -1;
+    e.st[RRS_SKIP] = -1;
+  }
+  __syncthreads();
+}
+
+template <bool P2, typename OffT, int E1, int E2>
+__device__ __attribute__((noinline)) void rr_before_pass(unsigned sh_addr, unsigned dyn_addr, int sc_v, int T_v) {
+  const RrEnv<OffT> e = rr_env<P2, OffT>(sh_addr, dyn_addr);
+  const int sc = uni(sc_v), T = uni(T_v), cov = uni(e.st[RRS_COV]);
+  if (cov < 0) return;
+  int take = awvrr::pass_for(e.al, uni(e.st[RRS_N]), sc, T);
+  if (take >= 0) {
+    const size_t tb = e.al.table_off() + e.al.table_index(cov, take) * 4;
+    if (!awvrr::box_ok(e.load(tb + awvrr::P_BOXH * 4), e.load(tb + awvrr::P_BOXV * 4), e.plen, e.tlen)) take = -1;
+    else {
+      const int maxak = e.load(tb + awvrr::P_MAXAK * 4), nc = e.load(tb + awvrr::P_CELLS * 4);
+      if (threadIdx.x == 0) {
+        e.st[RRS_SKIP] = cov;
+        e.st[RRS_MAXAK] = maxak;
+        e.st[RRS_CELLS] = nc;
+        __attribute__((address_space(1))) unsigned long long* const rc = (__attribute__((address_space(1))) unsigned long long*)(e.arch + awvrr::H_RCELLS * 4);
+        *rc = __hip_atomic_load((unsigned long long*)rc, __ATOMIC_RELAXED, __HIP_MEMORY_SCOPE_AGENT) + (unsigned long long)nc;
+        if (take == 0) *e.word(awvrr::H_RSEARCH * 4) = __hip_atomic_load((int*)e.word(awvrr::H_RSEARCH * 4), __ATOMIC_RELAXED, __HIP_MEMORY_SCOPE_AGENT) + 1;
+      }
+      __syncthreads();
+    }
+  }
+  if (take < 0) rr_hand_over<P2, OffT, E1, E2>(e, cov, sc);
+}
+
+template <bool P2, typename OffT, int E1, int E2>
+__device__ __attribute__((noinline)) void rr_end(unsigned sh_addr, unsigned dyn_addr, int sc_v) {
+  const RrEnv<OffT> e = rr_env<P2, OffT>(sh_addr, dyn_addr);
+  const int cov = uni(e.st[RRS_COV]);
+  if (cov >= 0) rr_hand_over<P2, OffT, E1, E2>(e, cov, uni(sc_v));
+}
+
+template <bool P2, typename OffT, int E1, int E2>
+__device__ __attribute__((noinline)) void rr_after_pass(unsigned sh_addr, unsigned dyn_addr, int sc_v, int T_v, int P0_v, int P1_v, int nc0_v, int nc1_v,
+                                                        int arun0_v, int arun1_v) {
+  constexpr int NID = 2 * E1 + (P2 ? 2 * E2 : 0);
+  const RrEnv<OffT> e = rr_env<P2, OffT>(sh_addr, dyn_addr);
+  if (uni(e.st[RRS_PART]) == 0) return;
+  const awvrr::Layout& al = e.al;
+  const int sc = uni(sc_v), T = uni(T_v), n = uni(e.st[RRS_N]);
+  const int lane = threadIdx.x & 63, rmask = e.kp.ring - 1;
+  bool ok = n < al.passes && T == al.T && sc == n * al.T;
+  int hmax[2] = {-K_BIG, -K_BIG}, lmin[2] = {K_BIG, K_BIG};
+#pragma unroll
+  for (int d = 0; d < 2; ++d) {
+    typename RrEnv<OffT>::MetaStored* const meta = e.ring_meta + (size_t)d * NCOMP * e.kp.ring;
+    for (int t = 0; t < T && ok; ++t) {
+      const RowMeta m = uni(meta_load(&meta[C_M * e.kp.ring + ((sc + 1 + t) & rmask)]));
+      if (!awvrr::hull_fits(al, m.lo, m.hi)) ok = false;
+      if (m.lo <= m.hi) { hmax[d] = max(hmax[d], m.hi); lmin[d] = min(lmin[d], m.lo); }
+    }
+  }
+  if (!ok) {
+    if (threadIdx.x == 0) e.st[RRS_PART] = 0;
+    __syncthreads();
+    return;
+  }
+#pragma unroll
+  for (int d = 0; d < 2; ++d) {
+    typename RrEnv<OffT>::MetaStored* const meta = e.ring_meta + (size_t)d * NCOMP * e.kp.ring;
+    const int kminD = d ? e.kmin[1] : e.kmin[0];
+    const int fc = awvrr::first_col(al, kminD);
+    for (int r = 0; r < T + NID; ++r) {
+      int comp = C_M, score = sc + 1 + r;
+      if (r >= T) multi_source<P2, E1, E2>(e.kp.pen, sc + T, r - T, comp, score);
+      if (score < 1) continue;
+      if (r < T && lane < NCOMP)
+        *e.word(al.meta_off() + al.meta_index(d, score, lane) * 4) = *reinterpret_cast<const int*>(&meta[lane * e.kp.ring + (score & rmask)]);
+      const RowMeta m = uni(meta_load(&meta[C_M * e.kp.ring + (score & rmask)]));
+      if (m.lo > m.hi) continue;
+      typedef unsigned int u32x2r __attribute__((ext_vector_type(2)));
+      const garch_t src = e.ring_row(d, comp, score);
+      garch_t dst = e.arch + al.row_off(d, n, r);
+      const int c_hi = (m.hi - kminD) | 3;
+      for (int c = ((m.lo - kminD) & ~3) + 4 * lane; c <= c_hi; c += 256)
+        *(__attribute__((address_space(1))) u32x2r*)(dst + (size_t)(c - fc) * 2) = *(const __attribute__((address_space(1))) u32x2r*)(src + (size_t)c * 2);
+    }
+    const int ar = uni(d ? arun1_v : arun0_v);
+    int boxh = uni(e.st[RRS_BOX + 2 * d]), boxv = uni(e.st[RRS_BOX + 2 * d + 1]);
+    if (hmax[d] >= lmin[d]) {
+      boxh = max(boxh, ar + hmax[d]);
+      boxv = max(boxv, ar - lmin[d]);
+    }
+    if (lane == 0) {
+      e.st[RRS_BOX + 2 * d] = boxh;
+      e.st[RRS_BOX + 2 * d + 1] = boxv;
+      const size_t tb = al.table_off() + al.table_index(d, n) * 4;
+      *e.word(tb + awvrr::P_MAXAK * 4) = uni(d ? P1_v : P0_v);
+      *e.word(tb + awvrr::P_CELLS * 4) = uni(d ? nc1_v : nc0_v);
+      *e.word(tb + awvrr::P_BOXH * 4) = boxh;
+      *e.word(tb + awvrr::P_BOXV * 4) = boxv;
+    }
+  }
+  if (lane == 0) {
+    e.st[RRS_N] = n + 1;
+    *e.word(awvrr::H_NPASS * 4) = n + 1;
+  }
+  __syncthreads();
+}
+
+template <bool P2, typename OffT, int E1, int E2, bool CHAIN>
+__device__ __attribute__((noinline)) void multi_phase_reuse(unsigned sh_addr, unsigned dyn_addr, int s0_v, int fmax_v, int rmax_v, int Tn_v, int pass_v, int deep_v) {
+  Shared& sh = *(Shared*)__builtin_assume_aligned((Shared*)(lds_shared_ptr)(uintptr_t)uni((int)sh_addr), 8);
+  unsigned char* dyn_smem = (unsigned char*)__builtin_assume_aligned((unsigned char*)(lds_bytes_ptr)(uintptr_t)uni((int)dyn_addr), 16);
+  const int Tn = uni(Tn_v);
+  int sc = uni(s0_v);
+  int fmax = uni(fmax_v), rmax = uni(rmax_v), pass = uni(pass_v);
+  const PassCtx& pc = sh.pctx;
+  KParams kp{};
+  kp.ring = uni(pc.ring);
+  kp.wcap = uni(pc.wcap);
+  kp.pen.x = uni(pc.x);
+  kp.pen.o1 = uni(pc.o1);
+  kp.pen.e1 = uni(pc.e1);
+  kp.pen.o2 = uni(pc.o2);
+  kp.pen.e2 = uni(pc.e2);
+  kp.pen.two_piece = P2 ? 1 : 0;
+  kp.pen.scope = max(kp.pen.x, max(kp.pen.o1 + kp.pen.e1, P2 ? kp.pen.o2 + kp.pen.e2 : 0)) + 1;
+  kp.lds_meta_bytes = uni(pc.lds_meta_bytes);
+  auto uni64 = [](unsigned long long v) { return ((unsigned long long)(unsigned)uni((int)(v >> 32)) << 32) | (unsigned)uni((int)v); };
+  SubCtx cx;
+  cx.plen = uni(pc.plen);
+  cx.tlen = uni(pc.tlen);
+  cx.kmin[0] = uni(pc.kmin[0]);
+  cx.kmin[1] = uni(pc.kmin[1]);
+  cx.wcols = uni(pc.wcols);
+  cx.seq_mode = uni(pc.seq_mode);
+  cx.p_w0 = uni(pc.p_w0);
+  cx.t_w0 = uni(pc.t_w0);
+  cx.p_bit = uni(pc.p_bit);
+  cx.t_bit = uni(pc.t_bit);
+  cx.P[0] = (gseq_t)(uintptr_t)uni64(pc.P[0]);
+  cx.P[1] = (gseq_t)(uintptr_t)uni64(pc.P[1]);
+  cx.T[0] = (gseq_t)(uintptr_t)uni64(pc.T[0]);
+  cx.T[1] = (gseq_t)(uintptr_t)uni64(pc.T[1]);
+  cx.Pw = nullptr;
+  cx.Tw = nullptr;
+  cx.pb_abs = cx.tb_abs = 0;
+  Lds<OffT> lds;
+  typedef typename MetaTraits<OffT>::Stored MetaStored;
+  lds.ring_meta = reinterpret_cast<MetaStored*>(dyn_smem);
+  lds.bi_A = reinterpret_cast<int*>(lds.ring_meta + 2 * NCOMP * kp.ring);
+  lds.bi_oob = lds.bi_A + 2 * kp.ring;
+  lds.firstk = lds.bi_oob + 2 * kp.ring;
+  lds.seq = reinterpret_cast<uint32_t*>(dyn_smem + kp.lds_meta_bytes);
+  lds.meta_log = nullptr;
+  const rsrc_t rs = make_rsrc((void*)(uintptr_t)uni64(pc.ring_mem), (size_t)uni64(pc.ring_bytes));
+  const int rmask = kp.ring - 1;
+  const int max_antidiagonal = cx.plen + cx.tlen - 1;
+  const int arun_start = fmax + rmax;
+  int arun0 = fmax, arun1 = rmax;
+  int nsteps = 0, npass = 0, why = MP_MARGIN;
+  unsigned long long cells = 0;
+  unsigned ext_iters = 0;
+  const bool lds_chain = CHAIN && sizeof(OffT) == 4 && cx.seq_mode != 1 &&
+                         uni(pc.lds_seq_bytes) >= (WG / 64) * TMAX32 * 64 * 16;
+  const int margin_shift = (uni(deep_v) >> 8) & 3;
+  const bool long_reads = (uni(deep_v) & 0x400) != 0;
+  const int chain_cap = CHAIN ? min(max(uni(pc.chain_max), 1), sizeof(OffT) == 2 ? CHAIN_MAX : (lds_chain ? 3 : CHAIN_MAX32)) : 1;
+  int* const rrs = lds.firstk;
+  rr_begin<P2, OffT, E1, E2>(sh_addr, dyn_addr, sc, chain_cap > 1 ? TMAX * chain_cap : Tn);
+  for (;;) {
+    if (sc >= uni(pc.score_cap)) { why = MP_BOUND; break; }
+    const int grow = nsteps > 0 ? (arun0 + arun1 - arun_start) / nsteps : 0;
+    int nh = 0;
+    for (int c = chain_cap; c >= 1; --c) {
+      const int T = c > 1 ? TMAX * c : Tn;
+      const int mul4 = (sizeof(OffT) == 2 && !long_reads) ? MARGIN_MUL4 : MARGIN_MUL4 + 2;
+      if (arun0 + arun1 < max_antidiagonal - ((MARGIN_BASE + mul4 * (kp.pen.scope + T) * max(grow, 8) / 4) << margin_shift)) { nh = c; break; }
+    }
+    if (nh == 0) { why = MP_MARGIN; break; }
+    const int T = nh > 1 ? TMAX * nh : Tn;
+    const int aslot = pass % 3;
+    int nc0 = 0, nc1 = 0;
+    if (uni(rrs[RRS_COV]) >= 0) rr_before_pass<P2, OffT, E1, E2>(sh_addr, dyn_addr, sc, T);
+#pragma nounroll
+    for (int dir = 0; dir < 2; ++dir) {
+      if (uni(rrs[RRS_SKIP]) == dir) continue;
+      MultiPlan mp;
+      const unsigned long long tpl = PROF_NOW();
+      plan_multi<P2, OffT, E1, E2, false>(kp, lds, cx, dir, sc, T, nh, mp);
+      mp.lds_chain = lds_chain ? 1 : 0;
+      PROF_ADD_L(STAT_T_CR_REDUCE, tpl);
+      Acc& acc = dir ? sh.acc[aslot][1] : sh.acc[aslot][0];
+      const int nc = compute_rows_multi<P2, OffT, E1, E2, false, CHAIN>(kp, sh, lds, cx, rs, dir, sc, mp, acc, dir ? sh.chain_maxak[1] : sh.chain_maxak[0], ext_iters);
+      if (dir) nc1 = nc; else nc0 = nc;
+    }
+    __syncthreads();
+    if (uni(sh.error)) { why = MP_ERROR; break; }
+    if (uni(sh.acc[aslot][0].oob) != 0 || uni(sh.acc[aslot][1].oob) != 0) { why = MP_DISCARD; break; }
+    const int rr_skip = uni(rrs[RRS_SKIP]);
+    if (rr_skip == 0) nc0 = uni(rrs[RRS_CELLS]);
+    if (rr_skip == 1) nc1 = uni(rrs[RRS_CELLS]);
+    cells += (unsigned long long)(nc0 + nc1);
+    const int P0 = rr_skip == 0 ? uni(rrs[RRS_MAXAK]) : uni(sh.chain_maxak[0][0]), P1 = rr_skip == 1 ? uni(rrs[RRS_MAXAK]) : uni(sh.chain_maxak[1][0]);
+    arun0 = max(arun0, P0);
+    arun1 = max(arun1, P1);
+    fmax = max(fmax, P0);
+    rmax = max(rmax, P1);
+    const bool met = fmax + rmax >= max_antidiagonal;
+    if (uni(rrs[RRS_PART]) != 0) rr_after_pass<P2, OffT, E1, E2>(sh_addr, dyn_addr, sc, T, P0, P1, nc0, nc1, arun0, arun1);
+    __syncthreads();
+    if (threadIdx.x < 16) sh.chain_maxak[threadIdx.x >> 3][threadIdx.x & 7] = 0;
+    if (threadIdx.x == 0) { acc_reset(sh.acc[(pass + 2) % 3][0]); acc_reset(sh.acc[(pass + 2) % 3][1]); }
+    __syncthreads();
+    ++pass;
+    ++npass;
+    nsteps += T;
+    sc += T;
+    if (met) { why = MP_MET; break; }
+  }
+  if (uni(rrs[RRS_COV]) >= 0) rr_end<P2, OffT, E1, E2>(sh_addr, dyn_addr, sc);
+  __syncthreads();
+  if (threadIdx.x == 0) {
+    PhaseResult& pr = sh.pres;
+    pr.why = why;
+    pr.sc = sc;
+    pr.sf = pr.sr = sc;
+    pr.last_fwd = 0;
+    pr.deep_from = sc;
+    pr.fmax = fmax;
+    pr.rmax = rmax;
+    pr.npass = npass;
+    pr.cells = cells;
+    pr.deep_cells = 0;
+#pragma unroll
+    for (int i = 0; i < 3; ++i) { acc_reset(sh.acc[i][0]); acc_reset(sh.acc[i][1]); }
+  }
+  if (threadIdx.x < 16) sh.chain_maxak[threadIdx.x >> 3][threadIdx.x & 7] = 0;
+  atomicAdd(&sh.ext_multi, (unsigned long long)ext_iters);
+  __syncthreads();
+  if ((uni(deep_v) & 1) != 0 && why == MP_MARGIN)
+    deep_phase<P2, OffT, E1, E2>(sh_addr, dyn_addr, sc, fmax, rmax, Tn, pass, npass, (unsigned)cells, (unsigned)(cells >> 32));
+}
+
 template <bool P2, typename OffT, int E1, int E2>
 __device__ __attribute__((noinline)) void deep_phase(unsigned sh_addr, unsigned dyn_addr, int s0_v, int fmax_v, int rmax_v, int Tn_v, int pass_v,
                                                      int far_npass_v, unsigned far_cells_lo, unsigned far_cells_hi) {
@@ -3171,6 +3551,233 @@
 }
 
 template <bool P2, typename OffT>
+__device__ __forceinline__ int find_breakpoint_reuse(const KParams& kp, Shared& sh, const Lds<OffT>& lds, SubCtx cx, void* ring_mem, rsrc_t ring_rs, int cb, int ce,
+                               int score_remaining, int known_score, int attempt, Breakpoint& bp, unsigned long long* lstats) {
+  const DevPenalties& pn = kp.pen;
+  const int tid = cold_tid();
+  const int plen = cx.plen, tlen = cx.tlen;
+  const int rmask = kp.ring - 1;
+  {
+    long long bound = (long long)score_remaining + 2LL * pn.scope + 16;
+    const long long half = (kp.wcap - 2 * COL_PAD - 9 - 256) / 2;
+    bound = min(bound, half);
+    const int blo = (int)min((long long)plen, bound), bhi = (int)min((long long)tlen, bound);
+    const int need = -blo - 4 - COL_PAD;
+    cx.kmin[0] = need;
+    const int D = tlen - plen;
+    const int c0 = D - need - need;
+    const int adj = ((255 - c0) % 256 + 256) % 256;
+    cx.kmin[1] = need - adj;
+    cx.wcols = blo + bhi + 9 + adj + 2 * COL_PAD;
+    if (cx.wcols > kp.wcap) return ST_CAPACITY;
+  }
+  const unsigned sh_addr = (unsigned)(uintptr_t)&sh, dyn_addr = (unsigned)(uintptr_t)lds.ring_meta;
+  if (tid == 0) {
+    PassCtx& pc = sh.pctx;
+    pc.ring_mem = (unsigned long long)(uintptr_t)ring_mem;
+    pc.ring_bytes = (unsigned long long)kp.ring_slot_stride;
+    pc.P[0] = (unsigned long long)(uintptr_t)cx.P[0];
+    pc.P[1] = (unsigned long long)(uintptr_t)cx.P[1];
+    pc.T[0] = (unsigned long long)(uintptr_t)cx.T[0];
+    pc.T[1] = (unsigned long long)(uintptr_t)cx.T[1];
+    pc.ring = kp.ring;
+    pc.wcap = kp.wcap;
+    pc.x = pn.x; pc.o1 = pn.o1; pc.e1 = pn.e1; pc.o2 = pn.o2; pc.e2 = pn.e2;
+    pc.lds_meta_bytes = kp.lds_meta_bytes;
+    pc.chain_max = kp.chain_max;
+    pc.plen = plen; pc.tlen = tlen;
+    pc.kmin[0] = cx.kmin[0]; pc.kmin[1] = cx.kmin[1];
+    pc.wcols = cx.wcols;
+    pc.seq_mode = cx.seq_mode; pc.p_w0 = cx.p_w0; pc.t_w0 = cx.t_w0; pc.p_bit = cx.p_bit; pc.t_bit = cx.t_bit;
+    const long long gap_open_max = P2 ? max(pn.o1, pn.o2) : pn.o1;
+    pc.score_cap = kp.max_penalty == INT_MAX ? INT_MAX : (int)min((long long)INT_MAX, ((long long)kp.max_penalty + pn.scope - 1 + gap_open_max) / 2 + 1);
+    sh.ext_multi = 0;
+  }
+  for (int i = tid; i < 2 * NCOMP; i += WG) {
+    const int dir = i / NCOMP, c = i % NCOMP;
+    const int begin = dir == 0 ? cb : ce;
+    meta_store(&lds.ring_meta[(dir * NCOMP + c) * kp.ring + 0], (c == begin) ? RowMeta{0, 0} : ROW_EMPTY);
+  }
+  if (tid == 0 || tid == (WG > 64 ? 64 : 1)) {
+    const int dir = tid ? 1 : 0;
+    const int begin = dir == 0 ? cb : ce;
+    unsigned it = 0;
+    int v0 = 0;
+    if (begin == C_M)
+      v0 = cx.seq_mode == 2 ? (dir ? extend_lcp_gw<1>(cx, 0, 0, it) : extend_lcp_gw<0>(cx, 0, 0, it))
+                            : extend_lcp(dir ? cx.P[1] : cx.P[0], dir ? cx.T[1] : cx.T[0], 0, 0, plen, tlen, it);
+    {
+      const int col = 0 - (dir ? cx.kmin[1] : cx.kmin[0]);
+      OffT* row = row_ptr<false, OffT>(kp, ring_mem, dir, begin, 0);
+      for (int j = 0; j < 4; ++j) row[(col & ~3) + j] = (OffT)(sizeof(OffT) == 2 ? NULL16 : OFF_NULL);
+      row[col] = (OffT)v0;
+    }
+    sh.ext0[dir] = v0;
+    lds.bi_A[(dir) * kp.ring + (0)] = (begin == C_M) ? 2 * v0 : 0;
+    lds.bi_oob[(dir) * kp.ring + (0)] = 0;
+    acc_reset(sh.acc[0][dir]);
+    acc_reset(sh.acc[1][dir]);
+    acc_reset(sh.acc[2][dir]);
+  }
+  __syncthreads();
+  if (cb == C_M && ce == C_M && plen == tlen && (uni(sh.ext0[0]) >= tlen || uni(sh.ext0[1]) >= tlen)) return BP_END_REACHED;
+  const int max_antidiagonal = plen + tlen - 1;
+  int sc[2] = {0, 0};
+  int comp[2] = {0, 0};
+  int fmax = uni(lds.bi_A[(0) * kp.ring + (0)]), rmax = uni(lds.bi_A[(1) * kp.ring + (0)]);
+  bp.score = INT_MAX;
+  unsigned ext_iters = 0;
+  unsigned long long cells = 0, multi_cells = 0, deep_cells = 0;
+  int pass = 0;
+  const long long max_steps = ((long long)pn.o1 + pn.o2 + 2LL * (pn.e1 + pn.e2) + pn.x) * ((long long)plen + tlen + 4) + 1024;
+  long long steps = 0;
+  int rc = BP_OK;
+  if (kp.max_penalty != INT_MAX) bp.score = kp.max_penalty + 1;
+  const int gap_opening = P2 ? max(pn.o1, pn.o2) : pn.o1;
+  bool last_fwd = false;
+  const bool known_optimum = known_score != INT_MAX;
+  bool dirty[2] = {false, false};
+  const bool force_single = (attempt & 0xff) >= AWV_RESTART_ATTEMPTS - 1;
+  const int deep_arg = kp.deep_passes | ((attempt & 0xff) == 1 && !force_single ? 0x200 : 0) | ((attempt & 0x100) ? 0x400 : 0);
+  const int multi_T = (!force_single && plen + tlen > AWV_MIN_PASS_LEN) ? kp.multi_T : 0;
+  bool deep_on = multi_T == 0;
+  int deep_since[2] = {deep_on ? 0 : INT_MAX, deep_on ? 0 : INT_MAX};
+  auto deep_ok = [&](int d0, int s0, int d1, int s1) {
+    const int lo_need = max(s1 - (pn.scope - 1), 1);
+    return (s0 == 0 || deep_since[d0] <= s0) && (s1 == 0 || deep_since[d1] <= lo_need);
+  };
+  int phase = 1;
+  for (;;) {
+    if (phase == 1 && fmax + rmax >= max_antidiagonal) phase = 2;
+    {
+      Acc* a = sh.acc[pass % 3];
+      int plo[2] = {1, 1}, phi[2] = {0, 0};
+      bool need[2];
+      const unsigned long long tp0 = PROF_NOW();
+      if (!deep_on && (dirty[0] || dirty[1])) {
+        deep_on = true;
+        deep_since[0] = comp[0] + 1;
+        deep_since[1] = comp[1] + 1;
+      }
+      if (!deep_on && phase == 1 && comp[0] == sc[0] && comp[1] == sc[1] && sc[0] == sc[1]) {
+        if (P2) multi_phase_reuse<P2, OffT, 2, 1, P2>(sh_addr, dyn_addr, sc[0], fmax, rmax, multi_T, pass, deep_arg);
+        else if (pn.e1 == 1) multi_phase_reuse<P2, OffT, 1, 1, false>(sh_addr, dyn_addr, sc[0], fmax, rmax, multi_T, pass, deep_arg);
+        else multi_phase_reuse<P2, OffT, 2, 1, false>(sh_addr, dyn_addr, sc[0], fmax, rmax, multi_T, pass, deep_arg);
+        PROF_ADD(STAT_T_BI_COMPUTE, tp0);
+        const int why = uni(sh.pres.why);
+        if (why == MP_ERROR) { rc = uni(sh.error); break; }
+        if (why == MP_MET) { rc = BP_RESTART; break; }
+        steps += (long long)(uni(sh.pres.sc) - sc[0]);
+        comp[0] = comp[1] = uni(sh.pres.sc);
+        sc[0] = uni(sh.pres.sf);
+        sc[1] = uni(sh.pres.sr);
+        last_fwd = uni(sh.pres.last_fwd) != 0;
+        fmax = uni(sh.pres.fmax);
+        rmax = uni(sh.pres.rmax);
+        pass += uni(sh.pres.npass);
+        {
+          const unsigned long long c = ((unsigned long long)(unsigned)uni((int)(sh.pres.cells >> 32)) << 32) | (unsigned)uni((int)sh.pres.cells);
+          const unsigned long long dc = ((unsigned long long)(unsigned)uni((int)(sh.pres.deep_cells >> 32)) << 32) | (unsigned)uni((int)sh.pres.deep_cells);
+          cells += c;
+          multi_cells += c;
+          deep_cells += dc;
+        }
+        deep_on = true;
+        deep_since[0] = deep_since[1] = uni(sh.pres.deep_from) + 1;
+        __syncthreads();
+        continue;
+      } else {
+#pragma unroll
+      for (int dir = 0; dir < 2; ++dir) {
+        need[dir] = comp[dir] == sc[dir];
+        if (need[dir]) {
+          StepPlan pl;
+          plan_step<P2, false, OffT>(kp, lds, dir, sc[dir] + 1, pl);
+          cells += compute_row<P2, false, OffT>(kp, sh, lds, cx, ring_rs, dir, sc[dir] + 1, pl, dirty[dir], a[dir], ext_iters);
+          plo[dir] = pl.lo;
+          phi[dir] = pl.hi;
+        }
+      }
+#ifdef AWV_DIAG
+      if (tid == 0) {
+        const int zone = (dirty[0] || dirty[1]) ? 4 : multi_T == 0 ? 0 : phase == 2 ? 3 : (sc[0] + 1 - (pn.scope - 1) >= 1) ? 2 : 1;
+        unsigned nw = 0;
+        if (need[0] && plo[0] <= phi[0]) nw += (unsigned)((phi[0] - plo[0] + 4) / 248 + 1);
+        if (need[1] && plo[1] <= phi[1]) nw += (unsigned)((phi[1] - plo[1] + 4) / 248 + 1);
+        lstats[STAT_T_CR_LOAD + zone] += nw;
+      }
+#endif
+      if (need[0] || need[1]) {
+        PROF_ADD(STAT_T_BI_COMPUTE, tp0);
+        PROF_INC(STAT_N_PASSES);
+        const unsigned long long tp1 = PROF_NOW();
+        __syncthreads();
+        PROF_ADD(STAT_T_BI_BARRIER, tp1);
+        const unsigned long long tp2 = PROF_NOW();
+        if (uni(sh.error)) { rc = uni(sh.error); break; }
+        const bool trim0 = need[0] && uni(a[0].oob) != 0, trim1 = need[1] && uni(a[1].oob) != 0;
+        dirty[0] = dirty[0] || trim0;
+        dirty[1] = dirty[1] || trim1;
+        if (trim0 || trim1) {
+          if (trim0) trim_pass_fn<P2, false, OffT>(sh_addr, 0, sc[0] + 1, plo[0], phi[0], pass % 3);
+          if (trim1) trim_pass_fn<P2, false, OffT>(sh_addr, 1, sc[1] + 1, plo[1], phi[1], pass % 3);
+          __syncthreads();
+        }
+        if (need[0]) { finalize_row<false, OffT>(kp, lds, cx, 0, sc[0] + 1, a[0], trim0); comp[0] = sc[0] + 1; }
+        if (need[1]) { finalize_row<false, OffT>(kp, lds, cx, 1, sc[1] + 1, a[1], trim1); comp[1] = sc[1] + 1; }
+        if (tid == 0) { acc_reset(sh.acc[(pass + 2) % 3][0]); acc_reset(sh.acc[(pass + 2) % 3][1]); }
+        ++pass;
+        PROF_ADD(STAT_T_BI_FINALIZE, tp2);
+      }
+      }
+    }
+    if (phase == 1) {
+      ++sc[0];
+      fmax = max(fmax, uni(lds.bi_A[0 * kp.ring + (sc[0] & rmask)]));
+      last_fwd = true;
+      if (fmax + rmax >= max_antidiagonal) { phase = 2; continue; }
+      ++sc[1];
+      rmax = max(rmax, uni(lds.bi_A[1 * kp.ring + (sc[1] & rmask)]));
+      last_fwd = false;
+      if (sc[1] >= uni(sh.pctx.score_cap)) { rc = BP_ABOVE_BOUND; break; }
+    } else {
+      if (last_fwd) {
+        const int min_sr = (sc[1] > pn.scope - 1) ? sc[1] - (pn.scope - 1) : 0;
+        if (sc[0] + min_sr - gap_opening >= bp.score) break;
+        if (!deep_ok(0, sc[0], 1, sc[1])) { rc = BP_RESTART; break; }
+        const unsigned long long to0 = PROF_NOW();
+        bialign_overlap<P2, OffT>(kp, sh, lds, cx, ring_mem, ring_rs, 0, sc[0], sc[1], true, bp, lstats);
+        PROF_ADD(STAT_T_OVERLAP, to0);
+        if (known_optimum && bp.score == known_score) break;
+        ++sc[1];
+      }
+      const int min_sf = (sc[0] > pn.scope - 1) ? sc[0] - (pn.scope - 1) : 0;
+      if (min_sf + sc[1] - gap_opening >= bp.score) break;
+      if (!deep_ok(1, sc[1], 0, sc[0])) { rc = BP_RESTART; break; }
+      const unsigned long long to1 = PROF_NOW();
+      bialign_overlap<P2, OffT>(kp, sh, lds, cx, ring_mem, ring_rs, 1, sc[1], sc[0], false, bp, lstats);
+      PROF_ADD(STAT_T_OVERLAP, to1);
+      if (known_optimum && bp.score == known_score) break;
+      ++sc[0];
+      last_fwd = true;
+    }
+    if (++steps > max_steps) { rc = ST_MAX_STEPS; break; }
+  }
+  if (tid == 0) {
+    lstats[STAT_CELLS] += cells;
+    lstats[STAT_MULTI_CELLS] += multi_cells;
+    lstats[STAT_DEEP_CELLS] += deep_cells;
+    lstats[STAT_BREAKPOINTS] += 1;
+  }
+  atomicAdd(&lstats[STAT_EXTEND], (unsigned long long)ext_iters);
+  if (tid == 0) lstats[STAT_EXTEND] += sh.ext_multi;
+  if (rc == BP_OK && bp.score > uni(sh.pctx.max_penalty)) rc = BP_ABOVE_BOUND;
+  __syncthreads();
+  if (rc == BP_OK && bp.score == INT_MAX) rc = ST_INTERNAL;
+  return rc;
+}
+
+template <bool P2, typename OffT>
 __device__ __attribute__((noinline)) int find_breakpoint_fn(unsigned sh_addr, unsigned dyn_addr, unsigned lstats_addr, int cb_v, int ce_v,
                                                             int score_remaining_v, int known_v, int attempt_v) {
   Shared& sh = *(Shared*)__builtin_assume_aligned((Shared*)(__attribute__((address_space(3))) Shared*)(uintptr_t)uni((int)sh_addr), 8);
@@ -3233,6 +3840,70 @@
   return rc;
 }
 
+
+template <bool P2, typename OffT>
+__device__ __attribute__((noinline)) int find_breakpoint_fn_reuse(unsigned sh_addr, unsigned dyn_addr, unsigned lstats_addr, int cb_v, int ce_v,
+                                                            int score_remaining_v, int known_v, int attempt_v) {
+  Shared& sh = *(Shared*)__builtin_assume_aligned((Shared*)(__attribute__((address_space(3))) Shared*)(uintptr_t)uni((int)sh_addr), 8);
+  unsigned char* dyn_smem = (unsigned char*)__builtin_assume_aligned((unsigned char*)(__attribute__((address_space(3))) unsigned char*)(uintptr_t)uni((int)dyn_addr), 16);
+  unsigned long long* lstats = (unsigned long long*)__builtin_assume_aligned((unsigned long long*)(__attribute__((address_space(3))) unsigned long long*)(uintptr_t)uni((int)lstats_addr), 8);
+  const int cb = uni(cb_v), ce = uni(ce_v), score_remaining = uni(score_remaining_v), known = uni(known_v);
+  const int attempt = uni(attempt_v);
+  const PassCtx& pc = sh.pctx;
+  auto uni64 = [](unsigned long long v) { return ((unsigned long long)(unsigned)uni((int)(v >> 32)) << 32) | (unsigned)uni((int)v); };
+  KParams kp{};
+  kp.ring = uni(pc.ring);
+  kp.wcap = uni(pc.wcap);
+  kp.pen.x = uni(pc.x);
+  kp.pen.o1 = uni(pc.o1);
+  kp.pen.e1 = uni(pc.e1);
+  kp.pen.o2 = uni(pc.o2);
+  kp.pen.e2 = uni(pc.e2);
+  kp.pen.two_piece = P2 ? 1 : 0;
+  kp.pen.scope = max(kp.pen.x, max(kp.pen.o1 + kp.pen.e1, P2 ? kp.pen.o2 + kp.pen.e2 : 0)) + 1;
+  kp.lds_meta_bytes = uni(pc.lds_meta_bytes);
+  kp.lds_seq_bytes = uni(pc.lds_seq_bytes);
+  kp.chain_max = uni(pc.chain_max);
+  kp.multi_T = uni(pc.multi_T);
+  kp.deep_passes = uni(pc.deep_passes);
+  kp.max_penalty = score_remaining == INT_MAX ? uni(pc.max_penalty) : INT_MAX;
+  kp.ring_slot_stride = (size_t)uni64(pc.ring_bytes);
+  SubCtx cx;
+  cx.plen = uni(pc.plen);
+  cx.tlen = uni(pc.tlen);
+  cx.kmin[0] = cx.kmin[1] = 0;
+  cx.wcols = 0;
+  cx.seq_mode = uni(pc.seq_mode);
+  cx.p_w0 = uni(pc.p_w0);
+  cx.t_w0 = uni(pc.t_w0);
+  cx.p_bit = uni(pc.p_bit);
+  cx.t_bit = uni(pc.t_bit);
+  cx.P[0] = (gseq_t)(uintptr_t)uni64(pc.P[0]);
+  cx.P[1] = (gseq_t)(uintptr_t)uni64(pc.P[1]);
+  cx.T[0] = (gseq_t)(uintptr_t)uni64(pc.T[0]);
+  cx.T[1] = (gseq_t)(uintptr_t)uni64(pc.T[1]);
+  cx.Pw = (gwords_t)(uintptr_t)uni64(pc.Pw);
+  cx.Tw = (gwords_t)(uintptr_t)uni64(pc.Tw);
+  cx.pb_abs = uni(pc.pb_abs);
+  cx.tb_abs = uni(pc.tb_abs);
+  Lds<OffT> lds;
+  typedef typename MetaTraits<OffT>::Stored MetaStored;
+  lds.ring_meta = reinterpret_cast<MetaStored*>(dyn_smem);
+  lds.bi_A = reinterpret_cast<int*>(lds.ring_meta + 2 * NCOMP * kp.ring);
+  lds.bi_oob = lds.bi_A + 2 * kp.ring;
+  lds.firstk = lds.bi_oob + 2 * kp.ring;
+  lds.seq = reinterpret_cast<uint32_t*>(dyn_smem + kp.lds_meta_bytes);
+  lds.meta_log = nullptr;
+  void* ring_mem = (void*)(__attribute__((address_space(1))) char*)(uintptr_t)uni64(pc.ring_mem);
+  const rsrc_t ring_rs = make_rsrc(ring_mem, kp.ring_slot_stride);
+  __syncthreads();
+  Breakpoint bp;
+  const int rc = find_breakpoint_reuse<P2, OffT>(kp, sh, lds, cx, ring_mem, ring_rs, cb, ce, score_remaining, known, attempt, bp, lstats);
+  if (threadIdx.x == 0) sh.bp_out = bp;
+  __syncthreads();
+  return rc;
+}
+
 template <bool P2, typename OffT, typename... PairSpan>
 __global__ __launch_bounds__(WG, WAVES_PER_SIMD) void biwfa_align_kernel(KParams kp, PairSpan... pair_span_arg) {
   constexpr bool RANGES = sizeof...(PairSpan) > 0;
@@ -3265,6 +3936,10 @@
   __syncthreads();
   constexpr bool TWINS = TWIN_BUILD && !RANGES && sizeof(OffT) == 2;
   if constexpr (TWINS) {
+  const unsigned long long rr_mem = kp.stats[STAT_N_DEV], rr_stride = kp.stats[STAT_N_DEV + 1], rr_pt = kp.stats[STAT_N_DEV + 2];
+  const int rr_passes = uni((int)(unsigned)rr_pt), rr_T = uni((int)(rr_pt >> 32)), rr_nid = uni((int)kp.stats[STAT_N_DEV + 3]);
+  int* const rr_hdr = rr_mem != 0 && rr_passes > 0 && pn.scope * NCOMP >= RRS_WORDS ? (int*)((char*)(uintptr_t)rr_mem + (size_t)blockIdx.x * (size_t)rr_stride) : nullptr;
+  if (rr_hdr != nullptr && tid < awvrr::H_WORDS) rr_hdr[tid] = 0;
   for (;;) {
     if (tid == 0) {
       sh.cur_pair = (long long)atomicAdd(kp.work_counter, 1ULL);
@@ -3321,6 +3996,7 @@
       { const bool x = top; top = top_o; top_o = x; }
     };
     if (TWINS && run_mode == TM_B) face(TM_B);
+    int rr_bv = -1, rr_bh = -1, rr_comp = 0, rr_mode = TM_A;
     int sp = 0;
     if constexpr (RANGES) {
       if (tid == 0) {
@@ -3418,6 +4094,26 @@
             else
               rc = uni(find_breakpoint_fn<P2, OffT>((unsigned)(uintptr_t)&sh, (unsigned)(uintptr_t)lds.ring_meta, (unsigned)(uintptr_t)lstats,
                                                     t.cb, t.ce, t.score_remaining, t.known, attempt));
+          } else if (rr_hdr != nullptr) {
+            int part = 0;
+            if (t.score_remaining == INT_MAX) part = RR_RECORD;
+            else if (rr_bv >= 0 && (mode == rr_mode || (rr_mode == TM_SHARED && mode == TM_A))) {
+              if (t.pb == 0 && t.tb == 0 && t.pe == rr_bv && t.te == rr_bh && t.cb == C_M && t.ce == rr_comp) part = RR_FWD;
+              else if (t.pb == rr_bv && t.tb == rr_bh && t.pe == plenT && t.te == tlenT && t.cb == rr_comp && t.ce == C_M) part = RR_REV;
+            }
+            if (tid == 0) {
+              const unsigned long long ra = (unsigned long long)(uintptr_t)rr_hdr;
+              lds.firstk[RRS_ARCH_LO] = (int)(unsigned)ra;
+              lds.firstk[RRS_ARCH_HI] = (int)(unsigned)(ra >> 32);
+              lds.firstk[RRS_PASSES] = rr_passes;
+              lds.firstk[RRS_T] = rr_T;
+              lds.firstk[RRS_NID] = rr_nid;
+              lds.firstk[RRS_PART] = part;
+              if (part == RR_RECORD) rr_hdr[awvrr::H_NPASS] = 0;
+            }
+            __syncthreads();
+            rc = uni(find_breakpoint_fn_reuse<P2, OffT>((unsigned)(uintptr_t)&sh, (unsigned)(uintptr_t)lds.ring_meta, (unsigned)(uintptr_t)lstats,
+                                                        t.cb, t.ce, t.score_remaining, t.known, attempt));
           } else {
             rc = uni(find_breakpoint_fn<P2, OffT>((unsigned)(uintptr_t)&sh, (unsigned)(uintptr_t)lds.ring_meta, (unsigned)(uintptr_t)lstats,
                                                   t.cb, t.ce, t.score_remaining, t.known, attempt));
@@ -3504,6 +4200,7 @@
         break;
       }
       const int bh = bp.off_f, bv = bp.off_f - bp.kf;
+      if (rr_hdr != nullptr && t.score_remaining == INT_MAX) { rr_bv = bv; rr_bh = bh; rr_comp = bp.comp; rr_mode = mode; }
       if (mode != TM_SHARED) {
         if (bh < 0 || bh > tlen || bv < 0 || bv > plen || sp + 2 > STACK_CAP) { status = ST_INTERNAL; break; }
         if (tid == 0) {
@@ -3599,6 +4296,12 @@
       atomicAdd(&kp.stats[STAT_TWIN_SOLO], (unsigned long long)tw_solo);
       atomicAdd(&kp.stats[STAT_TWIN_NONMIRROR], (unsigned long long)tw_nonmirror);
     }
+  }
+  if (rr_hdr != nullptr && tid == 0) {
+    const unsigned long long rcells = __hip_atomic_load((unsigned long long*)(rr_hdr + awvrr::H_RCELLS), __ATOMIC_RELAXED, __HIP_MEMORY_SCOPE_AGENT);
+    const int rsearch = __hip_atomic_load(rr_hdr + awvrr::H_RSEARCH, __ATOMIC_RELAXED, __HIP_MEMORY_SCOPE_AGENT);
+    if (rcells) atomicAdd(&kp.stats[STAT_REUSE_CELLS], rcells);
+    if (rsearch) atomicAdd(&kp.stats[STAT_REUSE_SEARCHES], (unsigned long long)rsearch);
   }
   } else {
   for (;;) {
diff --git a/allwave_amd/csrc/engine.hip b/allwave_amd/csrc/engine.hip
--- a/allwave_amd/csrc/engine.hip
+++ b/allwave_amd/csrc/engine.hip
@@ -48,6 +48,7 @@
 
 #include "batch_plan.hpp"
 #include "twin_plan.hpp"
+#include "row_reuse.hpp"
 
 namespace {
 const awvb::Limits LIMITS = {awv::TMAX, awv::TMAX32, awv::CHAIN_MAX, awv::MAX_RING, awv::MAX_SCOPE, awv::NCOMP, awv::COL_PAD,
@@ -142,6 +143,7 @@
   SeqSet seqs;
   DevBuf<uint8_t> ring_mem, hist_mem;
   DevBuf<uint32_t> ev_mem;
+  DevBuf<uint8_t> reuse_mem;
   DevBuf<int32_t> d_pair_q, d_pair_t, d_pair_rc;
   DevBuf<int32_t> d_pair_bound;
   DevBuf<int32_t> d_unit_first, d_unit_twin;
@@ -157,6 +159,7 @@
     std::vector<uint64_t> hoff;
     std::vector<awvr::Span> hspan;
     std::vector<awv_result> tres;
+    unsigned long long hreuse[4] = {0, 0, 0, 0};
   } stage;
   awv_stats stats{};
   awp::PlanState* plan = nullptr;
@@ -339,6 +342,7 @@
   double kernel_ms = 0, h2d_ms = 0, d2h_ms = 0;
   unsigned long long stat_tot[awv::STAT_N_DEV] = {0};
   uint64_t launches = 0;
+  awvrr::Layout reuse{0, 0, 0, 0};
   SinkRunner runner;
   bool want_cigar() const { return rq.sink && !rq.score_only && !(e->cfg.flags & AWV_F_KEEP_ON_DEVICE); }
   void lap(const char* what) const {
@@ -402,7 +406,7 @@
   if (int rc = e->d_cigar_off.reserve(n)) return rc;
   if (int rc = e->d_results.reserve(n)) return rc;
   if (int rc = e->d_cigar.reserve((size_t)c.arena + 64)) return rc;
-  if (int rc = e->d_counters.reserve(1 + awv::STAT_N_DEV)) return rc;
+  if (int rc = e->d_counters.reserve(1 + awv::STAT_N_DEV + awv::RR_DESC_WORDS)) return rc;
   static_assert(sizeof(awv_result) == sizeof(awv::DevResult), "result layout");
   c.hres.assign(n, awv_result{});
   return AWV_OK;
@@ -480,6 +484,34 @@
   return AWV_OK;
 }
 
+void plan_row_archives(AlignCall& c, const std::vector<awvb::Entry>& ge, const awvb::RowPlan& rp, int wc, int nslots) {
+  awv_engine* e = c.e;
+  c.reuse = awvrr::Layout{0, 0, 0, 0};
+  const AlignRequest& rq = c.rq;
+  if (rp.waves != 1 || rp.width != 0 || (e->cfg.flags & AWV_F_NO_ROW_REUSE) || rq.spans || rq.score_only || rq.pair_bound ||
+      rq.max_penalty != INT_MAX || c.pp.multi_T <= 0)
+    return;
+  int maxsum = 0;
+  for (const awvb::Entry& p : ge) maxsum = std::max(maxsum, p.ql + p.tl);
+  const int chain = std::min(std::max(c.pp.chain_max, 1), awv::CHAIN_MAX);
+  const int T = chain > 1 ? awv::TMAX * chain : c.pp.multi_T;
+  const int nid = 2 * c.pp.e1 + (c.pp.two_piece ? 2 * c.pp.e2 : 0);
+  const size_t used = rp.per_slot(wc) * (size_t)nslots;
+  const int passes = awvrr::plan_passes(maxsum, T, nid, nslots, rp.budget > used ? rp.budget - used : 0);
+  if (passes == 0) {
+    c.lap("row archives: none (no room, or pairs too short)");
+    return;
+  }
+  const awvrr::Layout l = awvrr::make_layout(passes, T, nid);
+  if (e->reuse_mem.reserve(l.bytes() * (size_t)nslots) != AWV_OK) {
+    (void)hipGetLastError();
+    c.lap("row archives: none (allocation failed)");
+    return;
+  }
+  c.reuse = l;
+  if (c.timing) fprintf(stderr, "[awv] row archives: %d passes of %d scores, %zu MiB for %d workgroups\n", passes, T, (l.bytes() * (size_t)nslots) >> 20, nslots);
+}
+
 int upload_twin_units(AlignCall& c, const std::vector<awvb::Entry>& ge, int64_t& nunits) {
   awv_engine* e = c.e;
   awv_engine::HostStage& st = e->stage;
@@ -535,7 +567,14 @@
   nunits = (int64_t)m;
   if (rp.twin_here)
     if (int rc = upload_twin_units(c, ge, nunits)) return rc;
-  AWV_TRY(hipMemsetAsync(e->d_counters.p, 0, (1 + awv::STAT_N_DEV) * sizeof(unsigned long long), e->stream));
+  AWV_TRY(hipMemsetAsync(e->d_counters.p, 0, (1 + awv::STAT_N_DEV + awv::RR_DESC_WORDS) * sizeof(unsigned long long), e->stream));
+  if (c.reuse.passes > 0) {
+    st.hreuse[0] = (unsigned long long)(uintptr_t)e->reuse_mem.p;
+    st.hreuse[1] = (unsigned long long)c.reuse.bytes();
+    st.hreuse[2] = (unsigned long long)(unsigned)c.reuse.passes | ((unsigned long long)(unsigned)c.reuse.T << 32);
+    st.hreuse[3] = (unsigned long long)c.reuse.nid;
+    AWV_TRY(hipMemcpyAsync(e->d_counters.p + 1 + awv::STAT_N_DEV, st.hreuse, sizeof(st.hreuse), hipMemcpyHostToDevice, e->stream));
+  }
   return timer_stop(c, c.h2d_ms);
 }
 
@@ -677,6 +716,7 @@
   for (int wc = rp.wcap; !ge.empty(); wc = rp.next_wc(wc)) {
     const int nslots = rp.slots(wc, (int64_t)ge.size());
     if (int rc = ensure_arenas(c, rp, wc, nslots)) return rc;
+    plan_row_archives(c, ge, rp, wc, nslots);
     c.lap("arenas reserved");
     if (c.timing) fprintf(stderr, "[awv] ring arena %p (%zu MiB), hist %p, cigar %p\n", (void*)c.e->ring_mem.p, c.e->ring_mem.bytes() >> 20, (void*)c.e->hist_mem.p, (void*)c.e->d_cigar.p);
     int64_t nunits = 0;
@@ -792,7 +832,7 @@
   e->stats.overlap_scans = stat_tot[STAT_OVERLAP];
   e->stats.aligned_bp = stat_tot[STAT_ALIGNED_BP];
   e->stats.pairs_completed = stat_tot[STAT_PAIRS];
-  e->stats.scratch_bytes = e->ring_mem.bytes() + e->hist_mem.bytes() + e->ev_mem.bytes();
+  e->stats.scratch_bytes = e->ring_mem.bytes() + e->hist_mem.bytes() + e->ev_mem.bytes() + e->reuse_mem.bytes();
   for (int i = 0; i < 14; ++i) e->stats.prof[i] = stat_tot[STAT_T_TOTAL + i];
   e->stats.restarts = stat_tot[STAT_RESTARTS];
   e->stats.multi_cell_steps = stat_tot[STAT_MULTI_CELLS];
@@ -805,6 +845,10 @@
   e->stats.clock_tick_khz = (uint64_t)e->wall_clock_khz;
   e->stats.deep_cell_steps = stat_tot[STAT_DEEP_CELLS];
   for (int i = 0; i < 4; ++i) e->twin_stats[i] = stat_tot[STAT_TWIN_UNITS + i];
+#if !defined(AWV_PROF) && !defined(AWV_DIAG)
+  e->stats.prof[12] = stat_tot[STAT_REUSE_CELLS];
+  e->stats.prof[13] = stat_tot[STAT_REUSE_SEARCHES];
+#endif
 }
 
 int align_core(awv_engine* e, SeqSet& s, const awv_penalties* pen, const AlignRequest& rq) {
@@ -924,6 +968,7 @@
   e->ring_mem.release();
   e->hist_mem.release();
   e->ev_mem.release();
+  e->reuse_mem.release();
   e->d_pair_q.release();
   e->d_pair_t.release();
   e->d_pair_rc.release();
diff --git a/allwave_amd/csrc/row_reuse.hpp b/allwave_amd/csrc/row_reuse.hpp
--- /dev/null
+++ b/allwave_amd/csrc/row_reuse.hpp
@@ -0,0 +1,69 @@
+#pragma once
+#include <stddef.h>
+#include <stdint.h>
+
+#if defined(__HIPCC__) || defined(__CUDACC__)
+#define AWVRR_HD __host__ __device__ inline
+#else
+#define AWVRR_HD inline
+#endif
+
+namespace awvrr {
+
+constexpr int NCOMP = 5;
+enum { H_NPASS = 0,
+       H_KMIN0 = 1,
+       H_KMIN1 = 2,
+       H_RCELLS = 4,
+       H_RSEARCH = 6,
+       H_WORDS = 16 };
+enum { P_MAXAK = 0,
+       P_CELLS = 1,
+       P_BOXH = 2,
+       P_BOXV = 3,
+       P_WORDS = 4 };
+
+struct Layout {
+  int passes, T, nid, cols;
+  AWVRR_HD int rows_per_pass() const { return T + nid; }
+  AWVRR_HD int scores() const { return passes * T; }
+  AWVRR_HD int reach() const { return scores(); }
+  AWVRR_HD size_t table_off() const { return (size_t)H_WORDS * 4; }
+  AWVRR_HD size_t table_index(int dir, int pass) const { return ((size_t)dir * passes + pass) * P_WORDS; }
+  AWVRR_HD size_t meta_off() const { return table_off() + (size_t)2 * passes * P_WORDS * 4; }
+  AWVRR_HD size_t meta_index(int dir, int s, int c) const { return ((size_t)dir * scores() + (s - 1)) * NCOMP + c; }
+  AWVRR_HD size_t rows_off() const { return (meta_off() + (size_t)2 * scores() * NCOMP * 4 + 15) & ~(size_t)15; }
+  AWVRR_HD size_t row_index(int dir, int pass, int r) const { return ((size_t)dir * passes + pass) * rows_per_pass() + r; }
+  AWVRR_HD size_t row_off(int dir, int pass, int r) const { return rows_off() + row_index(dir, pass, r) * cols * 2; }
+  AWVRR_HD size_t bytes() const { return (rows_off() + (size_t)2 * passes * rows_per_pass() * cols * 2 + 255) & ~(size_t)255; }
+};
+
+AWVRR_HD int cols_for(int scores) { return (2 * (scores + 8) + 8 + 3) & ~3; }
+AWVRR_HD Layout make_layout(int passes, int T, int nid) { return Layout{passes, T, nid, cols_for(passes * T)}; }
+
+AWVRR_HD int first_col(const Layout& l, int kmin) { return (-(l.reach() + 8) - kmin) & ~3; }
+AWVRR_HD bool hull_fits(const Layout& l, int lo, int hi) { return lo > hi || (lo >= -l.reach() && hi <= l.reach()); }
+AWVRR_HD int pass_of(const Layout& l, int s) { return (s - 1) / l.T; }
+AWVRR_HD int row_of(const Layout& l, int s) { return (s - 1) % l.T; }
+AWVRR_HD int id_row(const Layout& l, int e1, int e2, int comp, int j) {
+  const int base = comp == 1 ? 0 : comp == 3 ? e1 : comp == 2 ? 2 * e1 : 2 * e1 + e2;
+  const int e = (comp == 1 || comp == 3) ? e1 : e2;
+  return l.T + base + (e - 1 - j);
+}
+
+AWVRR_HD bool box_ok(int boxh, int boxv, int plen, int tlen) { return boxh <= 2 * tlen && boxv <= 2 * plen; }
+
+AWVRR_HD int pass_for(const Layout& l, int npass, int sc, int Tc) {
+  if (Tc != l.T || sc < 0 || sc % l.T != 0) return -1;
+  const int p = sc / l.T;
+  return p < npass && p < l.passes ? p : -1;
+}
+
+inline int plan_passes(int maxsum, int T, int nid, long long nslots, unsigned long long avail) {
+  if (T < 2 || nslots <= 0) return 0;
+  int passes = (maxsum / 28 < 4096 ? maxsum / 28 : 4096) / T;
+  while (passes >= 4 && (unsigned long long)make_layout(passes, T, nid).bytes() * (unsigned long long)nslots > avail) passes = passes * 3 / 4;
+  return passes >= 4 ? passes : 0;
+}
+
+}
diff --git a/allwave_amd/ffi.py b/allwave_amd/ffi.py
--- a/allwave_amd/ffi.py
+++ b/allwave_amd/ffi.py
@@ -28,6 +28,7 @@
 AWV_F_NO_TWIN = 2048
 AWV_F_TWIN_TOP_ONLY = 4096
 AWV_F_NO_TWIN_BASE = 8192
+AWV_F_NO_ROW_REUSE = 16384
 AWV_ORIENT_FORWARD = 0
 AWV_ORIENT_REVERSE = 1
 AWV_ORIENT_UNDECIDED = 2
diff --git a/include/allwave_hip.h b/include/allwave_hip.h
--- a/include/allwave_hip.h
+++ b/include/allwave_hip.h
@@ -51,6 +51,7 @@
 #define AWV_F_NO_TWIN 2048
 #define AWV_F_TWIN_TOP_ONLY 4096
 #define AWV_F_NO_TWIN_BASE 8192
+#define AWV_F_NO_ROW_REUSE 16384
 
 typedef struct {
   int32_t match;
diff --git a/scratch/asm_identity.py b/scratch/asm_identity.py
--- /dev/null
+++ b/scratch/asm_identity.py
@@ -0,0 +1,39 @@
+import re
+import sys
+
+
+def functions(path):
+    out, name, body = {}, None, []
+    for line in open(path):
+        m = re.match(r"^(_Z\w+):\s", line)
+        if m:
+            if name:
+                out[name] = body
+            name, body = m.group(1), []
+            continue
+        if name is None:
+            continue
+        if line.startswith(".Lfunc_end"):
+            out[name] = body
+            name = None
+            continue
+        s = line.split(";")[0].strip()
+        if not s or s.startswith(".") and not s.startswith(".LBB") or s.endswith(":"):
+            continue
+        body.append(re.sub(r"\.LBB\d+_", ".LBB_", s))
+    if name:
+        out[name] = body
+    return out
+
+
+a, b = functions(sys.argv[1]), functions(sys.argv[2])
+same = [n for n in a if n in b and a[n] == b[n]]
+diff = [n for n in a if n in b and a[n] != b[n]]
+print("%d functions at the parent, %d in this build; %d identical, %d differ, %d only at the parent, %d only in this build" %
+      (len(a), len(b), len(same), len(diff), len(set(a) - set(b)), len(set(b) - set(a))))
+for n in diff:
+    print("  differs  %-100s instructions %d -> %d" % (n, len(a[n]), len(b[n])))
+for n in sorted(set(a) - set(b)):
+    print("  only at the parent  %s (%d)" % (n, len(a[n])))
+for n in sorted(set(b) - set(a)):
+    print("  only in this build  %s (%d)" % (n, len(b[n])))
```
